# dbdexter-dev/sdrpp_radiosonde

Hardware: AMD Instinct MI355X
Metric: IQ Msamples/s through demod+FEC @ 48 kS/s/ch (higher is better)
Workload: dtype f32; 1 GPU; RS41-SG x 1024 channels/GPU x 196608 samples per step (4800 Bd GFSK, 48 kS/s, Eb/N0 14.0 dB); 5 consecutive blocks of a continuous signal resident in HBM, cycled; channels_per_gpu=1024, samples_per_channel=196608, flags=0, launch_units=1, join=one launch on the caller's stream, channel_stride_samples=262144, ingest=rank-local

## Files before the change

### include/sonde_abi.h

```cpp
#ifndef SONDE_ABI_H
#define SONDE_ABI_H

#include <stddef.h>
#include <stdint.h>
#include <time.h>

#ifdef __cplusplus
extern "C" {
#endif


typedef enum { PROCEED = 0, PARSED = 1 } ParserStatus;

#define DATA_SEQ      (1 << 0)
#define DATA_POS      (1 << 1)
#define DATA_SPEED    (1 << 2)
#define DATA_TIME     (1 << 3)
#define DATA_PTU      (1 << 4)
#define DATA_SERIAL   (1 << 5)
#define DATA_SHUTDOWN (1 << 6)
#define DATA_OZONE    (1 << 7)

typedef struct {
	int    fields;
	int    seq;
	float  lat, lon, alt;
	float  speed, heading, climb;
	time_t time;
	float  calib_percent;
	float  temp, rh, pressure;
	char   serial[32];
	int    shutdown;
	float  o3_mpa;
} SondeData;

typedef struct SondeB1Decoder RS41Decoder;
typedef struct SondeB1Decoder DFM09Decoder;
typedef struct SondeB1Decoder IMS100Decoder;
typedef struct SondeB1Decoder M10Decoder;
typedef struct SondeB1Decoder IMET4Decoder;
typedef struct SondeB1Decoder C50Decoder;
typedef struct SondeB1Decoder MRZN1Decoder;

#define SONDE_B1_DECL(T, x) \
	T *x##_decoder_init(int samplerate); \
	void x##_decoder_deinit(T *d); \
	ParserStatus x##_decode(T *d, SondeData *dst, const float *src, size_t len);

SONDE_B1_DECL(RS41Decoder,   rs41)
SONDE_B1_DECL(DFM09Decoder,  dfm09)
SONDE_B1_DECL(IMS100Decoder, ims100)
SONDE_B1_DECL(M10Decoder,    m10)
SONDE_B1_DECL(IMET4Decoder,  imet4)
SONDE_B1_DECL(C50Decoder,    c50)
SONDE_B1_DECL(MRZN1Decoder,  mrzn1)


enum { SONDE_RS41 = 0, SONDE_DFM09 = 1, SONDE_IMS100 = 2, SONDE_M10 = 3, SONDE_IMET4 = 4, SONDE_C50 = 5, SONDE_MRZN1 = 6, SONDE_NTYPES = 7 };

enum { SONDE_INPUT_IQ = 0,
       SONDE_INPUT_REAL = 1,
       SONDE_INPUT_IQ8 = 3,
       SONDE_INPUT_IQ16 = 2 };

#define SONDE_TILE       2048
#define SONDE_FRAME_MAX  528

typedef struct {
	uint32_t channel;
	uint32_t type;
	int32_t  len;
	int32_t  nerr[2];
	uint32_t flags;
	uint64_t bitpos;
	uint8_t  data[SONDE_FRAME_MAX];
} SondeFrame;

typedef struct {
	uint32_t       n_channels;
	const uint8_t *types;
	uint32_t       max_samples;
	int32_t        input_kind;
	int32_t        device;
	uint32_t       flags;
	uint32_t       launch_units;
	uint32_t       struct_size;
	uint32_t       time_slices;
} SondeBatchConfig;
#define SONDE_BATCH_CONFIG_INIT { 0, NULL, 0, 0, 0, 0, 0, (uint32_t)sizeof(SondeBatchConfig), 0 }

#define SONDE_FLAG_WIDE      1u
#define SONDE_FLAG_RS41_WIDE SONDE_FLAG_WIDE
#define SONDE_FLAG_SPLIT_FEC 2u
#define SONDE_FLAG_PIPELINE  4u
#define SONDE_FLAG_WIDE_AUTO 8u
#define SONDE_FLAG_JOIN      16u
#define SONDE_FLAG_LATE_JOIN 32u

typedef struct SondeBatch SondeBatch;

int  sonde_batch_create(const SondeBatchConfig *cfg, SondeBatch **out);
void sonde_batch_destroy(SondeBatch *b);

size_t sonde_row_stride(size_t n_samples, int input_kind);
size_t sonde_sample_bytes(int input_kind);
int  sonde_batch_submit(SondeBatch *b, const void *samples, size_t n_samples, size_t channel_stride, void *stream);
int  sonde_batch_submit_host(SondeBatch *b, const void *samples, size_t n_samples, size_t channel_stride);
int  sonde_batch_wait_input(SondeBatch *b, void *stream);
long sonde_batch_sync(SondeBatch *b);
long sonde_batch_frames(SondeBatch *b, SondeFrame *out, size_t cap);
uint64_t sonde_batch_ticket(SondeBatch *b);
long sonde_batch_frames_of(SondeBatch *b, uint64_t ticket, SondeFrame *out, size_t cap);
long sonde_batch_overflow(SondeBatch *b);
long sonde_batch_poll(SondeBatch *b, SondeData *out, uint32_t *channel, size_t cap);
int  sonde_batch_kernel_ms(SondeBatch *b, float *demod_ms, float *framer_ms);
int  sonde_batch_set_timing(SondeBatch *b, int every_n);
int  sonde_batch_launch_info(const SondeBatch *b, uint32_t *n_units, int32_t *join_mode);
int  sonde_batch_class_ms(SondeBatch *b, float out[4]);

int      sonde_batch_read_bits(SondeBatch *b, uint32_t channel, uint64_t from, size_t count, uint8_t *out );
int      sonde_batch_test_rs255(SondeBatch *b, uint8_t *cw_pairs, size_t n_pairs, int n, int32_t *status);
uint64_t sonde_batch_nbits(SondeBatch *b, uint32_t channel);
int      sonde_batch_read_state(SondeBatch *b, uint32_t channel, int64_t *t_next, int32_t *period, float *bias, float *amp,
                                float *afc_u );
int      sonde_get_taps(int type, float *out );
int      sonde_get_afsk_table(float *out );

int  sonde_parse_frame(const SondeFrame *f, SondeData *out, int cap);

typedef struct SondeParserHandle SondeParserHandle;
SondeParserHandle *sonde_parser_create(int sonde_type);
int  sonde_parser_feed(SondeParserHandle *p, const SondeFrame *f, SondeData *out, int cap);
void sonde_parser_destroy(SondeParserHandle *p);

float sonde_rs41_temp(uint32_t f, uint32_t f1, uint32_t f2, float rf1, float rf2, const float co[3], const float cal[3]);
float sonde_rs41_rh(uint32_t f, uint32_t f1, uint32_t f2, float calh0, float temp);
float sonde_dfm_temp(float f, float f1, float f2);
float sonde_rs41_pressure(uint32_t f, uint32_t f1, uint32_t f2, float tpress, const float *cfP );
float sonde_ozone_mpa(float cell_ua, float tpump_c);
float sonde_m10_temp(unsigned scale, unsigned adc);
float sonde_m10_rh(uint32_t cap_sensor, uint32_t cap_ref, float temp);
float sonde_m20_temp(unsigned adc);
float sonde_ims100_temp(uint32_t f, float c0, float c1, float c2);

typedef struct SondeChannelizer SondeChannelizer;
int         sonde_chan_create(const uint8_t *types , uint32_t blocks_per_submit ,
                              int device, SondeChannelizer **out);
int         sonde_chan_create_multi(const uint8_t *types, uint32_t blocks_per_submit, uint32_t n_streams, int device, SondeChannelizer **out);
int         sonde_chan_create_dual(const uint8_t *types, uint32_t blocks_per_submit, uint32_t n_streams, int device, SondeChannelizer **out);
uint32_t    sonde_chan_streams(const SondeChannelizer *c);
uint32_t    sonde_chan_channels(const SondeChannelizer *c);
int         sonde_chan_set_fused(SondeChannelizer *c, int on);
int         sonde_chan_set_input(SondeChannelizer *c, int input_kind);
int         sonde_chan_set_overlap(SondeChannelizer *c, int on);
void        sonde_chan_destroy(SondeChannelizer *c);
uint32_t    sonde_chan_samples_per_submit(const SondeChannelizer *c);
int         sonde_chan_submit(SondeChannelizer *c, const void *iq_dev, size_t n_samples, void *stream);
SondeBatch *sonde_chan_batch(SondeChannelizer *c);
int         sonde_chan_read(SondeChannelizer *c, float *bins, float *out48);
int         sonde_chan_kernel_ms(SondeChannelizer *c, float *pfb_ms, float *disc_resamp_ms, float *demod_ms, float *framer_ms);
int         sonde_chan_tables(float *h, float *tw, float *g);

typedef struct SondeVfo SondeVfo;
int    sonde_vfo_create(uint32_t n_channels, int rate_in, size_t max_in, int device, SondeVfo **out);
void   sonde_vfo_destroy(SondeVfo *v);
int    sonde_vfo_ratio(int rate_in, int *up, int *down);
size_t sonde_vfo_out_samples(const SondeVfo *v, size_t n_in);
int    sonde_vfo_process(SondeVfo *v, const void *iq_dev, size_t n_in, size_t channel_stride ,
                         float *out48_dev, size_t out_stride , void *stream);
int    sonde_vfo_process_host(SondeVfo *v, const void *iq_host, size_t n_in, size_t channel_stride,
                              const float **out48_dev, size_t *out_stride);
int    sonde_vfo_taps(int rate_in, float *g );

typedef struct SondeDetector SondeDetector;
typedef struct {
	int32_t  type;
	uint32_t inverted;
	double   best[SONDE_NTYPES];
	uint64_t pos[SONDE_NTYPES];
} SondeDetection;
int  sonde_detect_create(uint32_t n_channels, uint32_t max_samples, int input_kind, const uint8_t *type_mask, int device, SondeDetector **out);
void sonde_detect_destroy(SondeDetector *d);
int  sonde_detect_submit(SondeDetector *d, const void *samples, size_t n_samples, size_t channel_stride, void *stream);
int  sonde_detect_results(SondeDetector *d, SondeDetection *out, size_t cap);
int  sonde_detect_reset(SondeDetector *d);
int  sonde_detect_thresholds(float out[SONDE_NTYPES]);
int  sonde_detect_read(SondeDetector *d, uint32_t channel, int32_t *D , int32_t *a_imet , int32_t *a_c50 );
int  sonde_detect_templates(int type, int8_t *s, int cap);

typedef struct { int32_t offset_hz; uint32_t bandwidth_hz;  } SondeTunerVfo;
typedef struct SondeTuner SondeTuner;
int    sonde_tuner_ratio(uint32_t rate_in, uint32_t rate_out, int *up, int *down);
int    sonde_tuner_taps(uint32_t rate_in, uint32_t rate_out, uint32_t bandwidth_hz, float *g, size_t cap);
int    sonde_tuner_create(uint32_t rate_in, uint32_t rate_out, uint32_t n_vfos, const SondeTunerVfo *vfos,
                          size_t max_in, int input_kind, int device, SondeTuner **out);
void   sonde_tuner_destroy(SondeTuner *t);
size_t sonde_tuner_out_samples(const SondeTuner *t, size_t n_in);
int    sonde_tuner_retune(SondeTuner *t, uint32_t vfo, int32_t offset_hz);
int    sonde_tuner_process(SondeTuner *t, const void *wide_dev, size_t n_in,
                           void *out_dev , size_t out_stride , void *stream);

typedef struct SondeScanner SondeScanner;
typedef struct {
	uint32_t struct_size;
	uint32_t smooth_hz;
	uint32_t min_sep_hz;
	uint32_t centroid_hz;
	float    threshold;
} SondeScanParams;
typedef struct {
	int32_t  offset_hz;
	uint32_t bandwidth_hz;
	float    cn0_dbhz;
	float    excess_db;
	uint32_t bin;
} SondeScanCandidate;
int  sonde_scan_create(uint32_t rate_in, uint32_t fft_size , size_t max_in, int input_kind, int device, SondeScanner **out);
void sonde_scan_destroy(SondeScanner *s);
int  sonde_scan_fft_size(const SondeScanner *s);
int  sonde_scan_submit(SondeScanner *s, const void *wide_dev, size_t n_in, void *stream);
int  sonde_scan_reset(SondeScanner *s);
long long sonde_scan_segments(SondeScanner *s);
int  sonde_scan_spectrum(SondeScanner *s, float *P, size_t cap);
int  sonde_scan_candidates(SondeScanner *s, const SondeScanParams *p, SondeScanCandidate *out, size_t cap);
int  sonde_scan_search(const float *P, uint32_t n, uint32_t rate_in, const SondeScanParams *p, SondeScanCandidate *out, size_t cap);
int  sonde_scan_window(uint32_t n, float *w, size_t cap);
int  sonde_scan_auto_fft_size(uint32_t rate_in);

float sonde_dewpt(float temp, float rh);
float sonde_altitude_to_pressure(float alt);

void *sonde_gpx_open(const char *path);
void  sonde_gpx_close(void *g);
void  sonde_gpx_start_track(void *g, const char *name);
void  sonde_gpx_stop_track(void *g);
void  sonde_gpx_add_point(void *g, long t, float lat, float lon, float alt, float spd, float hdg);
void *sonde_ptu_open(const char *path);
void  sonde_ptu_close(void *p);
void  sonde_ptu_add_point(void *p, long t, float temp, float rh, float dewpt, float pressure, float lat, float lon,
                          float alt, float spd, float hdg, float climb, const char *aux);

int sonde_hbm_read_probe(const void *d_buf, size_t bytes, int reps, float *gbs_out);

const char *sonde_last_error(void);
const char *sonde_version(void);

#ifdef __cplusplus
}
#endif
#endif
```

### sdrpp_radiosonde_amd/_lib.py

```python
from __future__ import annotations

import ctypes as C
import os

import numpy as np

PKG_DIR = os.path.dirname(os.path.abspath(__file__))
LIB_PATH = os.environ.get("SONDE_MI355_LIB") or os.path.join(PKG_DIR, "libsonde_mi355.so")

TILE = 2048
FRAME_MAX = 528
(RS41, DFM09, IMS100, M10, IMET4, C50, MRZN1) = range(7)
INPUT_IQ, INPUT_REAL, INPUT_IQ16, INPUT_IQ8 = 0, 1, 2, 3
PROCEED, PARSED = 0, 1
DATA_SEQ, DATA_POS, DATA_SPEED, DATA_TIME, DATA_PTU, DATA_SERIAL, DATA_SHUTDOWN, DATA_OZONE = (1 << i for i in range(8))


class SondeFrame(C.Structure):
    _fields_ = [("channel", C.c_uint32), ("type", C.c_uint32), ("len", C.c_int32), ("nerr", C.c_int32 * 2),
                ("flags", C.c_uint32), ("bitpos", C.c_uint64), ("data", C.c_uint8 * FRAME_MAX)]


FRAME_DTYPE = np.dtype([("channel", "<u4"), ("type", "<u4"), ("len", "<i4"), ("nerr", "<i4", (2,)),
                        ("flags", "<u4"), ("bitpos", "<u8"), ("data", "u1", (FRAME_MAX,))])
assert FRAME_DTYPE.itemsize == C.sizeof(SondeFrame)


class SondeData(C.Structure):
    _fields_ = [("fields", C.c_int), ("seq", C.c_int), ("lat", C.c_float), ("lon", C.c_float), ("alt", C.c_float),
                ("speed", C.c_float), ("heading", C.c_float), ("climb", C.c_float), ("time", C.c_int64),
                ("calib_percent", C.c_float), ("temp", C.c_float), ("rh", C.c_float), ("pressure", C.c_float),
                ("serial", C.c_char * 32), ("shutdown", C.c_int), ("o3_mpa", C.c_float)]


class SondeDetection(C.Structure):
    _fields_ = [("type", C.c_int32), ("inverted", C.c_uint32), ("best", C.c_double * 7), ("pos", C.c_uint64 * 7)]


DETECTION_DTYPE = np.dtype([("type", "<i4"), ("inverted", "<u4"), ("best", "<f8", (7,)), ("pos", "<u8", (7,))])
assert DETECTION_DTYPE.itemsize == C.sizeof(SondeDetection)


class SondeTunerVfo(C.Structure):
    _fields_ = [("offset_hz", C.c_int32), ("bandwidth_hz", C.c_uint32)]


class SondeScanParams(C.Structure):
    _fields_ = [("struct_size", C.c_uint32), ("smooth_hz", C.c_uint32), ("min_sep_hz", C.c_uint32), ("centroid_hz", C.c_uint32),
                ("threshold", C.c_float)]


class SondeScanCandidate(C.Structure):
    _fields_ = [("offset_hz", C.c_int32), ("bandwidth_hz", C.c_uint32), ("cn0_dbhz", C.c_float), ("excess_db", C.c_float),
                ("bin", C.c_uint32)]


CANDIDATE_DTYPE = np.dtype([("offset_hz", "<i4"), ("bandwidth_hz", "<u4"), ("cn0_dbhz", "<f4"), ("excess_db", "<f4"), ("bin", "<u4")])
assert CANDIDATE_DTYPE.itemsize == C.sizeof(SondeScanCandidate)


class SondeBatchConfig(C.Structure):
    _fields_ = [("n_channels", C.c_uint32), ("types", C.POINTER(C.c_uint8)), ("max_samples", C.c_uint32),
                ("input_kind", C.c_int32), ("device", C.c_int32), ("flags", C.c_uint32), ("launch_units", C.c_uint32),
                ("struct_size", C.c_uint32), ("time_slices", C.c_uint32)]

    def __init__(self, *a, **k):
        super().__init__(*a, **k)
        self.struct_size = C.sizeof(SondeBatchConfig)


FLAG_WIDE = 1
FLAG_RS41_WIDE = FLAG_WIDE
FLAG_SPLIT_FEC = 2
FLAG_PIPELINE = 4
FLAG_JOIN = 16
FLAG_LATE_JOIN = 32
FLAG_WIDE_AUTO = 8


ABI_SYMBOLS = [
    "sonde_batch_create", "sonde_batch_destroy", "sonde_batch_submit", "sonde_batch_submit_host",
    "sonde_row_stride", "sonde_sample_bytes", "sonde_batch_wait_input", "sonde_batch_sync", "sonde_batch_frames", "sonde_batch_frames_of", "sonde_batch_ticket", "sonde_batch_overflow", "sonde_batch_kernel_ms", "sonde_batch_set_timing", "sonde_batch_class_ms", "sonde_batch_read_bits",
    "sonde_batch_launch_info", "sonde_batch_nbits", "sonde_batch_read_state", "sonde_batch_test_rs255", "sonde_batch_poll", "sonde_get_taps", "sonde_get_afsk_table", "sonde_parse_frame",
    "sonde_parser_create", "sonde_parser_feed", "sonde_parser_destroy", "sonde_rs41_temp", "sonde_rs41_rh", "sonde_dfm_temp", "sonde_rs41_pressure", "sonde_ozone_mpa",
    "sonde_m10_temp", "sonde_m10_rh", "sonde_m20_temp", "sonde_ims100_temp",
    "sonde_last_error", "sonde_version", "sonde_hbm_read_probe", "sonde_dewpt", "sonde_altitude_to_pressure",
    "sonde_gpx_open", "sonde_gpx_close", "sonde_gpx_start_track", "sonde_gpx_stop_track", "sonde_gpx_add_point",
    "sonde_ptu_open", "sonde_ptu_close", "sonde_ptu_add_point",
    "sonde_chan_create", "sonde_chan_create_multi", "sonde_chan_create_dual", "sonde_chan_streams", "sonde_chan_channels", "sonde_chan_set_fused", "sonde_chan_set_input", "sonde_chan_set_overlap", "sonde_chan_destroy", "sonde_chan_samples_per_submit", "sonde_chan_submit", "sonde_chan_batch",
    "sonde_chan_read", "sonde_chan_tables", "sonde_chan_kernel_ms",
    "sonde_vfo_create", "sonde_vfo_destroy", "sonde_vfo_ratio", "sonde_vfo_out_samples", "sonde_vfo_process", "sonde_vfo_process_host", "sonde_vfo_taps",
    "sonde_detect_create", "sonde_detect_destroy", "sonde_detect_submit", "sonde_detect_results", "sonde_detect_reset", "sonde_detect_thresholds",
    "sonde_detect_read", "sonde_detect_templates",
    "sonde_tuner_ratio", "sonde_tuner_taps", "sonde_tuner_create", "sonde_tuner_destroy", "sonde_tuner_out_samples", "sonde_tuner_retune",
    "sonde_tuner_process",
    "sonde_scan_create", "sonde_scan_destroy", "sonde_scan_fft_size", "sonde_scan_submit", "sonde_scan_reset", "sonde_scan_segments",
    "sonde_scan_spectrum", "sonde_scan_candidates", "sonde_scan_search", "sonde_scan_window", "sonde_scan_auto_fft_size",
] + [f"{x}_{fn}" for x in ("rs41", "dfm09", "ims100", "m10", "imet4", "c50", "mrzn1")
     for fn in ("decoder_init", "decoder_deinit", "decode")]

_lib = None


def load() -> C.CDLL:
    global _lib
    if _lib is not None:
        return _lib
    if not os.path.exists(LIB_PATH):
        import subprocess
        csrc = os.path.join(os.path.dirname(LIB_PATH), "csrc")
        try:
            subprocess.check_call(["make", "-s", "-C", csrc])
        except (OSError, subprocess.CalledProcessError) as e:
            raise RuntimeError(f"{LIB_PATH} is missing and `make -C {csrc}` failed ({e}); there is no CPU fallback") from e
    L = C.CDLL(LIB_PATH)
    vp = C.c_void_p
    L.sonde_hbm_read_probe.argtypes = [C.c_void_p, C.c_size_t, C.c_int, C.POINTER(C.c_float)]
    L.sonde_hbm_read_probe.restype = C.c_int
    L.sonde_last_error.restype = C.c_char_p
    L.sonde_version.restype = C.c_char_p
    L.sonde_batch_create.argtypes = [C.POINTER(SondeBatchConfig), C.POINTER(vp)]
    L.sonde_batch_destroy.argtypes = [vp]
    L.sonde_batch_destroy.restype = None
    L.sonde_batch_submit.argtypes = [vp, vp, C.c_size_t, C.c_size_t, vp]
    L.sonde_batch_submit_host.argtypes = [vp, vp, C.c_size_t, C.c_size_t]
    L.sonde_batch_sync.argtypes = [vp]
    L.sonde_batch_sync.restype = C.c_long
    if hasattr(L, "sonde_batch_wait_input"):
        L.sonde_batch_wait_input.argtypes = [vp, vp]
    L.sonde_batch_frames.argtypes = [vp, vp, C.c_size_t]
    L.sonde_batch_frames.restype = C.c_long
    if hasattr(L, "sonde_batch_frames_of"):
        L.sonde_batch_frames_of.argtypes = [vp, C.c_uint64, vp, C.c_size_t]
        L.sonde_batch_frames_of.restype = C.c_long
        L.sonde_batch_ticket.argtypes = [vp]
        L.sonde_batch_ticket.restype = C.c_uint64
        L.sonde_batch_overflow.argtypes = [vp]
        L.sonde_batch_overflow.restype = C.c_long
    L.sonde_batch_kernel_ms.argtypes = [vp, C.POINTER(C.c_float), C.POINTER(C.c_float)]
    if hasattr(L, "sonde_batch_set_timing"):
        L.sonde_batch_set_timing.argtypes = [vp, C.c_int]
    L.sonde_batch_read_bits.argtypes = [vp, C.c_uint32, C.c_uint64, C.c_size_t, vp]
    L.sonde_batch_nbits.argtypes = [vp, C.c_uint32]
    L.sonde_batch_nbits.restype = C.c_uint64
    L.sonde_batch_read_state.argtypes = [vp, C.c_uint32, C.POINTER(C.c_int64), C.POINTER(C.c_int32),
                                         C.POINTER(C.c_float), C.POINTER(C.c_float), C.POINTER(C.c_float)]
    if hasattr(L, "sonde_batch_test_rs255"):
        L.sonde_batch_test_rs255.argtypes = [vp, vp, C.c_size_t, C.c_int, vp]
    L.sonde_get_taps.argtypes = [C.c_int, vp]
    L.sonde_parse_frame.argtypes = [vp, C.POINTER(SondeData), C.c_int]
    L.sonde_batch_poll.argtypes = [vp, C.POINTER(SondeData), C.POINTER(C.c_uint32), C.c_size_t]
    L.sonde_batch_poll.restype = C.c_long
    L.sonde_parser_create.argtypes = [C.c_int]
    L.sonde_parser_create.restype = vp
    L.sonde_parser_feed.argtypes = [vp, vp, C.POINTER(SondeData), C.c_int]
    L.sonde_parser_feed.restype = C.c_int
    L.sonde_parser_destroy.argtypes = [vp]
    L.sonde_parser_destroy.restype = None
    L.sonde_rs41_pressure.argtypes = [C.c_uint32, C.c_uint32, C.c_uint32, C.c_float, C.POINTER(C.c_float)]
    L.sonde_rs41_pressure.restype = C.c_float
    L.sonde_ozone_mpa.argtypes = [C.c_float, C.c_float]
    L.sonde_ozone_mpa.restype = C.c_float
    L.sonde_m10_temp.argtypes = [C.c_uint, C.c_uint]
    L.sonde_m10_temp.restype = C.c_float
    L.sonde_m10_rh.argtypes = [C.c_uint32, C.c_uint32, C.c_float]
    L.sonde_m10_rh.restype = C.c_float
    L.sonde_m20_temp.argtypes = [C.c_uint]
    L.sonde_m20_temp.restype = C.c_float
    L.sonde_ims100_temp.argtypes = [C.c_uint32, C.c_float, C.c_float, C.c_float]
    L.sonde_ims100_temp.restype = C.c_float
    L.sonde_rs41_temp.argtypes = [C.c_uint32, C.c_uint32, C.c_uint32, C.c_float, C.c_float, C.POINTER(C.c_float), C.POINTER(C.c_float)]
    L.sonde_rs41_temp.restype = C.c_float
    L.sonde_rs41_rh.argtypes = [C.c_uint32, C.c_uint32, C.c_uint32, C.c_float, C.c_float]
    L.sonde_rs41_rh.restype = C.c_float
    L.sonde_dfm_temp.argtypes = [C.c_float, C.c_float, C.c_float]
    L.sonde_dfm_temp.restype = C.c_float
    L.sonde_dewpt.restype = C.c_float
    L.sonde_dewpt.argtypes = [C.c_float, C.c_float]
    L.sonde_altitude_to_pressure.restype = C.c_float
    L.sonde_altitude_to_pressure.argtypes = [C.c_float]
    L.sonde_chan_create.argtypes = [vp, C.c_uint32, C.c_int, C.POINTER(vp)]
    L.sonde_chan_create_multi.argtypes = [vp, C.c_uint32, C.c_uint32, C.c_int, C.POINTER(vp)]
    L.sonde_chan_set_fused.argtypes = [vp, C.c_int]
    L.sonde_chan_set_overlap.argtypes = [vp, C.c_int]
    L.sonde_row_stride.argtypes = [C.c_size_t, C.c_int]
    L.sonde_row_stride.restype = C.c_size_t
    L.sonde_sample_bytes.argtypes = [C.c_int]
    L.sonde_sample_bytes.restype = C.c_size_t
    L.sonde_chan_streams.argtypes = [vp]
    L.sonde_chan_streams.restype = C.c_uint32
    L.sonde_chan_destroy.argtypes = [vp]
    L.sonde_chan_destroy.restype = None
    L.sonde_chan_samples_per_submit.argtypes = [vp]
    L.sonde_chan_samples_per_submit.restype = C.c_uint32
    L.sonde_chan_submit.argtypes = [vp, vp, C.c_size_t, vp]
    L.sonde_chan_kernel_ms.argtypes = [vp] + [C.POINTER(C.c_float)] * 4
    L.sonde_chan_batch.argtypes = [vp]
    L.sonde_chan_batch.restype = vp
    L.sonde_chan_read.argtypes = [vp, vp, vp]
    L.sonde_chan_tables.argtypes = [vp, vp, vp]
    if hasattr(L, "sonde_vfo_create"):
        L.sonde_vfo_create.argtypes = [C.c_uint32, C.c_int, C.c_size_t, C.c_int, C.POINTER(vp)]
        L.sonde_vfo_destroy.argtypes = [vp]
        L.sonde_vfo_destroy.restype = None
        L.sonde_vfo_ratio.argtypes = [C.c_int, C.POINTER(C.c_int), C.POINTER(C.c_int)]
        L.sonde_vfo_out_samples.argtypes = [vp, C.c_size_t]
        L.sonde_vfo_out_samples.restype = C.c_size_t
        L.sonde_vfo_process.argtypes = [vp, vp, C.c_size_t, C.c_size_t, vp, C.c_size_t, vp]
        L.sonde_vfo_process_host.argtypes = [vp, vp, C.c_size_t, C.c_size_t, C.POINTER(vp), C.POINTER(C.c_size_t)]
        L.sonde_vfo_taps.argtypes = [C.c_int, vp]
    if hasattr(L, "sonde_detect_create"):
        L.sonde_detect_create.argtypes = [C.c_uint32, C.c_uint32, C.c_int, vp, C.c_int, C.POINTER(vp)]
        L.sonde_detect_destroy.argtypes = [vp]
        L.sonde_detect_destroy.restype = None
        L.sonde_detect_submit.argtypes = [vp, vp, C.c_size_t, C.c_size_t, vp]
        L.sonde_detect_results.argtypes = [vp, vp, C.c_size_t]
        L.sonde_detect_reset.argtypes = [vp]
        L.sonde_detect_thresholds.argtypes = [vp]
        L.sonde_detect_read.argtypes = [vp, C.c_uint32, vp, vp, vp]
        L.sonde_detect_templates.argtypes = [C.c_int, vp, C.c_int]
    if hasattr(L, "sonde_tuner_create"):
        L.sonde_tuner_ratio.argtypes = [C.c_uint32, C.c_uint32, C.POINTER(C.c_int), C.POINTER(C.c_int)]
        L.sonde_tuner_taps.argtypes = [C.c_uint32, C.c_uint32, C.c_uint32, vp, C.c_size_t]
        L.sonde_tuner_create.argtypes = [C.c_uint32, C.c_uint32, C.c_uint32, C.POINTER(SondeTunerVfo), C.c_size_t, C.c_int, C.c_int, C.POINTER(vp)]
        L.sonde_tuner_destroy.argtypes = [vp]
        L.sonde_tuner_destroy.restype = None
        L.sonde_tuner_out_samples.argtypes = [vp, C.c_size_t]
        L.sonde_tuner_out_samples.restype = C.c_size_t
        L.sonde_tuner_retune.argtypes = [vp, C.c_uint32, C.c_int32]
        L.sonde_tuner_process.argtypes = [vp, vp, C.c_size_t, vp, C.c_size_t, vp]
    if hasattr(L, "sonde_scan_create"):
        L.sonde_scan_create.argtypes = [C.c_uint32, C.c_uint32, C.c_size_t, C.c_int, C.c_int, C.POINTER(vp)]
        L.sonde_scan_destroy.argtypes = [vp]
        L.sonde_scan_destroy.restype = None
        L.sonde_scan_fft_size.argtypes = [vp]
        L.sonde_scan_submit.argtypes = [vp, vp, C.c_size_t, vp]
        L.sonde_scan_reset.argtypes = [vp]
        L.sonde_scan_segments.argtypes = [vp]
        L.sonde_scan_segments.restype = C.c_longlong
        L.sonde_scan_spectrum.argtypes = [vp, vp, C.c_size_t]
        L.sonde_scan_candidates.argtypes = [vp, C.POINTER(SondeScanParams), vp, C.c_size_t]
        L.sonde_scan_search.argtypes = [vp, C.c_uint32, C.c_uint32, C.POINTER(SondeScanParams), vp, C.c_size_t]
        L.sonde_scan_window.argtypes = [C.c_uint32, vp, C.c_size_t]
        L.sonde_scan_auto_fft_size.argtypes = [C.c_uint32]
    f = C.c_float
    L.sonde_gpx_open.restype = vp
    L.sonde_gpx_open.argtypes = [C.c_char_p]
    L.sonde_gpx_close.argtypes = [vp]
    L.sonde_gpx_start_track.argtypes = [vp, C.c_char_p]
    L.sonde_gpx_stop_track.argtypes = [vp]
    L.sonde_gpx_add_point.argtypes = [vp, C.c_long, f, f, f, f, f]
    L.sonde_ptu_open.restype = vp
    L.sonde_ptu_open.argtypes = [C.c_char_p]
    L.sonde_ptu_close.argtypes = [vp]
    L.sonde_ptu_add_point.argtypes = [vp, C.c_long, f, f, f, f, f, f, f, f, f, f, C.c_char_p]
    for x in ("rs41", "dfm09", "ims100", "m10", "imet4", "c50", "mrzn1"):
        getattr(L, f"{x}_decoder_init").argtypes = [C.c_int]
        getattr(L, f"{x}_decoder_init").restype = vp
        getattr(L, f"{x}_decoder_deinit").argtypes = [vp]
        getattr(L, f"{x}_decoder_deinit").restype = None
        getattr(L, f"{x}_decode").argtypes = [vp, C.POINTER(SondeData), vp, C.c_size_t]
        getattr(L, f"{x}_decode").restype = C.c_int
    _lib = L
    return L


def last_error() -> str:
    return load().sonde_last_error().decode()
```

### sdrpp_radiosonde_amd/batch.py

```python
from __future__ import annotations

import ctypes as C

import numpy as np

from . import _lib
from ._lib import FRAME_DTYPE, INPUT_IQ, INPUT_IQ8, INPUT_IQ16, INPUT_REAL, TILE


class SondeError(RuntimeError):
    pass


class SondeBatch:

    def __init__(self, n_channels: int, max_samples: int, *, types=None, input_kind: int = INPUT_IQ, device: int = 0, flags: int = 0, time_slices: int = 0):
        self.L = _lib.load()
        self.n_channels = int(n_channels)
        self.max_samples = int(max_samples)
        self.input_kind = input_kind
        self.device = int(device)
        cfg = _lib.SondeBatchConfig()
        cfg.n_channels = self.n_channels
        self._types = None
        if types is not None:
            self._types = np.ascontiguousarray(types, dtype=np.uint8)
            assert self._types.shape == (self.n_channels,)
            cfg.types = self._types.ctypes.data_as(C.POINTER(C.c_uint8))
        cfg.max_samples = self.max_samples
        cfg.flags = flags
        cfg.time_slices = time_slices
        cfg.input_kind = input_kind
        cfg.device = device
        h = C.c_void_p()
        if self.L.sonde_batch_create(C.byref(cfg), C.byref(h)) != 0:
            raise SondeError(_lib.last_error())
        self.h = h

    def close(self):
        if getattr(self, "h", None):
            self.L.sonde_batch_destroy(self.h)
            self.h = None

    __del__ = close

    def _chk(self, rc):
        if rc < 0:
            raise SondeError(_lib.last_error())
        return rc

    def submit(self, samples, stream: int | None = None):
        shape = tuple(samples.shape)
        n = shape[1]
        if shape[0] != self.n_channels:
            raise SondeError("first dimension must be n_channels")
        is_iq = self.input_kind in (INPUT_IQ, INPUT_IQ16, INPUT_IQ8)
        if is_iq and (len(shape) != 3 or shape[2] != 2):
            raise SondeError("IQ input must be [C, n, 2] (float32; int16 for INPUT_IQ16, int8 for INPUT_IQ8)")
        if not is_iq and len(shape) != 2:
            raise SondeError("real input must be [C, n] float32")
        dt = str(getattr(samples, "dtype", ""))
        want = {INPUT_IQ16: "int16", INPUT_IQ8: "int8"}.get(self.input_kind, "float32")
        if not dt.endswith(want) or dt.endswith("u" + want):
            raise SondeError(f"samples must be {want}, got {dt}")
        dev = getattr(samples, "device", None)
        if dev is None or getattr(dev, "type", "") != "cuda":
            raise SondeError("samples must be a device (HIP) tensor; use submit_host() for host memory")
        if dev.index is not None and dev.index != self.device:
            raise SondeError(f"samples live on device {dev.index}, the batch on device {self.device}")
        st = tuple(samples.stride())
        if (is_iq and st[1:] != (2, 1)) or (not is_iq and st[1] != 1):
            raise SondeError("samples must be contiguous inside a channel (only the channel stride may be padded)")
        stride = samples.stride(0) // (2 if is_iq else 1)
        self._keep = (samples, getattr(self, "_keep", (None, None))[0])
        self._chk(self.L.sonde_batch_submit(self.h, C.c_void_p(samples.data_ptr()), n, stride, C.c_void_p(stream or 0)))

    def submit_host(self, samples: np.ndarray):
        want = {INPUT_IQ16: np.int16, INPUT_IQ8: np.int8}.get(self.input_kind, np.float32)
        if want is not np.float32 and np.asarray(samples).dtype != want:
            raise SondeError(f"samples must be {np.dtype(want).name} for this input kind, got {np.asarray(samples).dtype} (no silent conversion)")
        samples = np.ascontiguousarray(samples, dtype=want)
        n = samples.shape[1]
        self._chk(self.L.sonde_batch_submit_host(self.h, samples.ctypes.data_as(C.c_void_p), n, n))

    def wait_input(self, stream: int | None = None):
        self._chk(self.L.sonde_batch_wait_input(self.h, C.c_void_p(stream or 0)))

    def sync(self) -> int:
        return self._chk(self.L.sonde_batch_sync(self.h))

    def frames(self) -> np.ndarray:
        n = self.sync()
        out = np.zeros(n, dtype=FRAME_DTYPE)
        if n:
            got = self._chk(self.L.sonde_batch_frames(self.h, out.ctypes.data_as(C.c_void_p), n))
            out = out[:got]
        return out

    def ticket(self) -> int:
        return int(self.L.sonde_batch_ticket(self.h))

    def frames_of(self, ticket: int) -> np.ndarray:
        n = self._chk(self.L.sonde_batch_frames_of(self.h, ticket, None, 0))
        out = np.zeros(n, dtype=FRAME_DTYPE)
        if n:
            out = out[:self._chk(self.L.sonde_batch_frames_of(self.h, ticket, out.ctypes.data_as(C.c_void_p), n))]
        return out

    def overflow(self) -> int:
        return self._chk(self.L.sonde_batch_overflow(self.h))

    def poll(self, cap: int = 4096):
        out = (_lib.SondeData * cap)()
        chan = (C.c_uint32 * cap)()
        res = []
        while True:
            n = self._chk(self.L.sonde_batch_poll(self.h, out, chan, cap))
            if n == 0:
                return res
            for i in range(n):
                d = _lib.SondeData()
                C.memmove(C.byref(d), C.byref(out[i]), C.sizeof(d))
                res.append((int(chan[i]), d))

    def kernel_ms(self):
        a, b = C.c_float(), C.c_float()
        self._chk(self.L.sonde_batch_kernel_ms(self.h, C.byref(a), C.byref(b)))
        return a.value, b.value

    def class_ms(self) -> dict:
        v = (C.c_float * 4)()
        self.L.sonde_batch_class_ms.argtypes = [C.c_void_p, C.POINTER(C.c_float)]
        n = self._chk(self.L.sonde_batch_class_ms(self.h, v))
        return {k: float(v[k]) for k in range(4) if n > 0 and v[k] >= 0.0}

    def launch_info(self) -> dict:
        u, j = C.c_uint32(), C.c_int32()
        self.L.sonde_batch_launch_info.argtypes = [C.c_void_p, C.POINTER(C.c_uint32), C.POINTER(C.c_int32)]
        self._chk(self.L.sonde_batch_launch_info(self.h, C.byref(u), C.byref(j)))
        return {"units": int(u.value), "join": int(j.value)}

    def set_timing(self, every_n: int):
        self._chk(self.L.sonde_batch_set_timing(self.h, int(every_n)))

    def nbits(self, channel: int) -> int:
        return int(self.L.sonde_batch_nbits(self.h, channel))

    def read_bits(self, channel: int, start: int, count: int) -> np.ndarray:
        out = np.zeros(count, dtype=np.uint8)
        self._chk(self.L.sonde_batch_read_bits(self.h, channel, start, count, out.ctypes.data_as(C.c_void_p)))
        return out

    def state(self, channel: int) -> dict:
        t, p = C.c_int64(), C.c_int32()
        b, a, y = C.c_float(), C.c_float(), C.c_float()
        self._chk(self.L.sonde_batch_read_state(self.h, channel, C.byref(t), C.byref(p), C.byref(b), C.byref(a), C.byref(y)))
        return dict(t_next=t.value, period=p.value, bias=b.value, amp=a.value, afc_u=y.value, yprev=y.value)


def row_stride(n_samples: int, iq: bool = True, kind: int | None = None) -> int:
    if kind is None:
        kind = INPUT_IQ if iq else INPUT_REAL
    return int(_lib.load().sonde_row_stride(int(n_samples), kind))


def strided_rows(x, stride: int | None = None):
    import torch
    n = x.shape[1]
    st = stride or row_stride(n, kind={torch.int16: INPUT_IQ16, torch.int8: INPUT_IQ8}.get(x.dtype, INPUT_IQ) if x.dim() == 3 else INPUT_REAL)
    if st == n:
        return x
    buf = torch.empty((x.shape[0], st) + tuple(x.shape[2:]), dtype=x.dtype, device=x.device)
    buf[:, :n] = x
    return buf[:, :n]


class SondeChannelizer:

    def __init__(self, types=None, blocks_per_submit: int = 1, device: int = 0, n_streams: int = 1, fused: bool | None = None, overlap: bool | None = None,
                 dual: bool = False, input_kind: int = INPUT_IQ):
        self.L = _lib.load()
        self._types = None
        self.n_streams = int(n_streams)
        self.dual = bool(dual)
        self.n_channels = (1024 if dual else 512) * self.n_streams
        tp = None
        if types is not None:
            self._types = np.ascontiguousarray(types, dtype=np.uint8)
            assert self._types.shape == (self.n_channels,)
            tp = self._types.ctypes.data_as(C.c_void_p)
        h = C.c_void_p()
        create = self.L.sonde_chan_create_dual if dual else self.L.sonde_chan_create_multi
        if create(tp, blocks_per_submit, self.n_streams, device, C.byref(h)) != 0:
            raise SondeError(_lib.last_error() or "sonde_chan_create failed")
        self.h = h
        self.fused = bool(self.L.sonde_chan_set_fused(self.h, 1 if fused else 0)) if fused is not None else bool(self.L.sonde_chan_set_fused(self.h, -1))
        self.overlap = bool(self.L.sonde_chan_set_overlap(self.h, 1)) if overlap else False
        self.input_kind = int(self.L.sonde_chan_set_input(self.h, input_kind))
        if self.input_kind != input_kind:
            raise SondeError("sonde_chan_set_input: input kind not accepted")
        self.samples_per_submit = int(self.L.sonde_chan_samples_per_submit(self.h))
        self.n_steps = self.samples_per_submit // 500
        self.batch = SondeBatch.__new__(SondeBatch)
        self.batch.L = self.L
        self.batch.h = C.c_void_p(self.L.sonde_chan_batch(self.h))
        self.batch.n_channels = self.n_channels
        self.batch.close = lambda: None

    def submit(self, iq, stream: int | None = None):
        assert tuple(iq.shape) in ((self.samples_per_submit, 2), (self.n_streams, self.samples_per_submit, 2)) and iq.is_contiguous()
        assert self.n_streams == 1 or iq.dim() == 3
        want = {INPUT_IQ16: "int16", INPUT_IQ8: "int8"}.get(self.input_kind, "float32")
        if not str(iq.dtype).endswith(want) or str(iq.dtype).endswith("u" + want):
            raise SondeError(f"wideband block must be {want}, got {iq.dtype}")
        self._keep = iq
        if self.L.sonde_chan_submit(self.h, C.c_void_p(iq.data_ptr()), self.samples_per_submit, C.c_void_p(stream or 0)) != 0:
            raise SondeError(_lib.last_error() or "sonde_chan_submit failed")

    def frames(self) -> np.ndarray:
        return SondeBatch.frames(self.batch)

    def kernel_ms(self):
        v = [C.c_float() for _ in range(4)]
        if self.L.sonde_chan_kernel_ms(self.h, *[C.byref(x) for x in v]) != 0:
            raise SondeError(_lib.last_error() or "sonde_chan_kernel_ms failed")
        return tuple(x.value for x in v)

    def read(self):
        bins = np.zeros((self.n_channels, self.n_steps), dtype=np.float32)
        out48 = None if self.fused else np.zeros((self.n_channels, self.n_steps * 12 // 5), dtype=np.float32)
        if self.L.sonde_chan_read(self.h, bins.ctypes.data_as(C.c_void_p), out48.ctypes.data_as(C.c_void_p) if out48 is not None else None) != 0:
            raise SondeError("sonde_chan_read failed")
        return bins, out48

    def close(self):
        if getattr(self, "h", None):
            self.batch.h = None
            self.L.sonde_chan_destroy(self.h)
            self.h = None

    __del__ = close


def get_taps(sonde_type: int) -> np.ndarray:
    out = np.zeros((32, 32), dtype=np.float32)
    if _lib.load().sonde_get_taps(sonde_type, out.ctypes.data_as(C.c_void_p)) != 0:
        raise SondeError(_lib.last_error())
    return out


VFO_RATE = {0: 10000, 1: 15000, 2: 20000, 3: 50000, 4: 20000, 5: 20000, 6: 20000}


class SondeVfo:

    def __init__(self, n_channels: int, rate_in: int, max_in: int, device: int = 0):
        self.L = _lib.load()
        h = C.c_void_p()
        if self.L.sonde_vfo_create(n_channels, rate_in, max_in, device, C.byref(h)) != 0:
            raise SondeError(_lib.last_error() or "sonde_vfo_create failed")
        self.h = h
        self.n_channels, self.rate_in, self.max_in = n_channels, rate_in, max_in
        up, down = C.c_int(), C.c_int()
        self.L.sonde_vfo_ratio(rate_in, C.byref(up), C.byref(down))
        self.up, self.down = up.value, down.value

    def out_samples(self, n_in: int) -> int:
        return int(self.L.sonde_vfo_out_samples(self.h, n_in))

    def process(self, iq, out=None, stream: int | None = None):
        import torch
        assert iq.is_cuda and iq.dtype == torch.float32 and iq.shape[0] == self.n_channels and iq.shape[2] == 2 and iq.stride(1) == 2
        n_in = iq.shape[1]
        n_out = self.out_samples(n_in)
        if out is None:
            out = torch.empty((self.n_channels, n_out), dtype=torch.float32, device=iq.device)
        if stream is None:
            stream = torch.cuda.current_stream(iq.device).cuda_stream
        if self.L.sonde_vfo_process(self.h, C.c_void_p(iq.data_ptr()), n_in, iq.stride(0) // 2, C.c_void_p(out.data_ptr()), out.stride(0),
                                    C.c_void_p(stream)) != 0:
            raise SondeError(_lib.last_error() or "sonde_vfo_process failed")
        return out

    def taps(self) -> np.ndarray:
        g = np.zeros((self.up, 16), dtype=np.float32)
        if self.L.sonde_vfo_taps(self.rate_in, g.ctypes.data_as(C.c_void_p)) != 0:
            raise SondeError(_lib.last_error() or "sonde_vfo_taps failed")
        return g

    def close(self):
        if getattr(self, "h", None):
            self.L.sonde_vfo_destroy(self.h)
            self.h = None

    def __del__(self):
        try:
            self.close()
        except Exception:
            pass
```

### sdrpp_radiosonde_amd/csrc/batch.hip

```cpp
#include <hip/hip_runtime.h>
#include <math.h>
#include <stdio.h>
#include <stdlib.h>
#include <string.h>
#include <algorithm>
#include <string>
#include <vector>
#include "sonde_dev.h"
#include "sd_input.h"
#include "../../include/sonde_abi.h"

#include "launch.h"
#include "parse.h"
#include <deque>
#include <memory>

#ifndef SD_EV_FLAGS
#define SD_EV_FLAGS hipEventDisableSystemFence
#endif
#define SD_EV_TIMING (SD_EV_FLAGS)
#define SD_EV_ORDER  (hipEventDisableTiming | SD_EV_FLAGS)
static thread_local std::string g_err;
static int fail(const char *what, hipError_t e = hipSuccess)
{
	g_err = what;
	if (e != hipSuccess) { g_err += ": "; g_err += hipGetErrorString(e); }
	return -1;
}
#define HIPCHK(x) do { hipError_t e_ = (x); if (e_ != hipSuccess) return fail(#x, e_); } while (0)

extern "C" const char *sonde_last_error(void) { return g_err.c_str(); }
int sd_fail(const char *what, hipError_t e) { return fail(what, e); }
extern "C" const char *sonde_version(void) { return "sonde_mi355 0.1 (gfx950)"; }

struct ModemDef { double baud; float cutoff; int decim; int pre; };
static const ModemDef k_modems[SONDE_NTYPES] = {
	{ 4800.0, 0.65f, 4, 1 },
	{ 5000.0, 0.65f, 4, 1 },
	{ 4800.0, 0.65f, 4, 1 },
	{ 9600.0, 0.65f, 2, 1 },
	{ 1200.0, 0.65f, 1, 8 },
	{ 2400.0, 0.65f, 1, 8 },
	{ 4800.0, 0.65f, 4, 1 },
};

static int modem_div(const ModemDef *md, int type) { return md[type].decim * md[type].pre; }
static int32_t modem_period0(const ModemDef *md, int type) { return (int32_t)llrint(65536.0 * ((double)SD_FS / modem_div(md, type)) / md[type].baud); }
static int modem_nt(const ModemDef *md, int type) { return SD_NT_OF(modem_period0(md, type), md[type].pre); }
static const int k_cls_decim[4] = { 1, 2, 4, 2 }, k_cls_nt[4] = { 16, 16, 8, 8 };
static int modem_class(const ModemDef *md, int type)
{
	const int d = md[type].decim, nt = modem_nt(md, type);
	for (int k = 0; k < 4; k++) if (k_cls_decim[k] == d && k_cls_nt[k] == nt) return k;
	return -1;
}

static void make_taps(const ModemDef *md, int type, float *out )
{
	const double PI = 3.14159265358979323846;
	const double fc = (double)md[type].cutoff * md[type].baud / ((double)SD_FS / modem_div(md, type));
	const int nt = modem_nt(md, type);
	memset(out, 0, sizeof(float) * SD_NPHASE * SD_NTAPS);
	for (int p = 0; p < SD_NPHASE; p++) {
		double h[SD_NTAPS], sum = 0.0;
		for (int j = 0; j < nt; j++) {
			const double t = (double)j - (double)(nt / 2) + (double)p / (double)SD_NPHASE;
			const double x = (t + (double)(nt / 2)) / (double)nt;
			const double w = 0.42 - 0.5 * cos(2.0 * PI * x) + 0.08 * cos(4.0 * PI * x);
			const double s = (t == 0.0) ? 2.0 * fc : sin(2.0 * PI * fc * t) / (PI * t);
			h[j] = s * w;
			sum += h[j];
		}
		for (int j = 0; j < nt; j++) out[p * SD_NTAPS + j] = (float)(h[j] / sum);
	}
}

void make_mixer(float *out, int cycles, int per)
{
	const double PI = 3.14159265358979323846;
	for (int k = 0; k < per; k++) {
		const double a = 2.0 * PI * (double)cycles * (double)k / (double)per;
		out[2 * k] = (float)cos(a);
		out[2 * k + 1] = (float)(-sin(a));
	}
}
extern "C" int sonde_get_afsk_table(float *out )
{
	if (!out) return fail("sonde_get_afsk_table: null argument");
	make_mixer(out, 17, SD_AF_PER);
	return 0;
}

extern "C" int sonde_get_taps(int type, float *out)
{
	if (type < 0 || type >= SONDE_NTYPES || !out) return fail("sonde_get_taps: bad argument");
	make_taps(k_modems, type, out);
	return 0;
}

struct SondeBatch {
	uint32_t n_channels = 0, max_samples = 0;
	int input_kind = 0, device = 0;
	uint32_t ring_words = 0, max_frames = 0;
	uint32_t type_frames[SONDE_NTYPES] = {};
	std::vector<uint8_t> types;
	std::vector<uint32_t> chlist[SONDE_NTYPES];
	ModemDef md[SONDE_NTYPES];

	SdChanState *d_states = nullptr;
	SdFramerState *d_fstates = nullptr;
	float *d_hist = nullptr;
	uint32_t *d_bitring = nullptr;
	SondeFrame *d_frames2[2] = {};
	uint32_t *d_counts2[2] = {};
	hipEvent_t ev_done[2] = {};
	bool ev_valid[2] = { false, false };
	bool ticketing = false;
	hipEvent_t ev_xs = nullptr;
	uint64_t tickets = 0;
	float *d_taps = nullptr;
	SdModem *d_modems = nullptr;
	uint8_t *d_gfexp = nullptr, *d_gflog = nullptr, *d_g64 = nullptr;
	uint16_t *d_m10tab = nullptr;
	uint32_t fuse_fec = 1;
	uint32_t fixed_epi = 1;
	SdFramerOut *d_fo2[2] = {};
	SdFramerOut h_fo2[2] = {};
	SdModem h_modems[SONDE_NTYPES] = {};
	uint32_t *d_gfswar = nullptr;
	void *d_descs = nullptr;
	uint32_t *d_chlist[SONDE_NTYPES] = {};
	void *d_stage = nullptr;
	size_t stage_bytes = 0;
	SdAfskState *d_astates = nullptr;
	float *d_wtab = nullptr, *d_wtab_c50 = nullptr, *d_afq = nullptr;
	uint32_t n_cls[4] = {};
	int cls_type[4] = { -1, -1, -1, -1 };
	int n_classes = 0, only_class = 0;
	struct Unit { int type, cls; uint32_t off, n; size_t row0; hipStream_t st; hipEvent_t ev_join[2]; };
	std::vector<Unit> units;
	uint32_t *d_cls[4] = {};
	int n_chunks = 1;
	hipEvent_t ev_fork = nullptr;
	int join_mode = 0;
	bool pipeline = false;
	hipStream_t done_stream = nullptr;
	uint32_t granule = SONDE_TILE;
	uint32_t *d_prog = nullptr;
	uint32_t seg_base = 0;
	uint32_t residency = 1024;
	int seg_force = 0;
	bool sliced_once = false;
	bool mixed_one = false;

	static const int kEvSlots = 128;
	hipEvent_t ev[3 * kEvSlots] = {};
	int ev_used = 0;
	hipEvent_t *evc = nullptr;
	int evc_used = 0;
	int timing_every = 8;
	unsigned long n_submits = 0;
	bool ev_has_framer[kEvSlots] = {};
	hipStream_t last_stream = nullptr;
	bool pending = false;
	bool have_counts2[2] = { false, false };
	std::vector<uint32_t> h_counts2[2];
	long n_frames2[2] = { 0, 0 }, n_overflow2[2] = { 0, 0 };
	std::vector<SondeFrame> h_slots;
	std::vector<std::unique_ptr<SondeParser>> parsers;
	std::deque<std::pair<uint32_t, SondeData>> frags;
	uint64_t polled_ticket = 0;
};

static uint32_t pow2ceil(uint32_t v) { uint32_t p = 1; while (p < v) p <<= 1; return p; }

extern "C" void sonde_batch_destroy(SondeBatch *b)
{
	if (!b) return;
	(void)hipSetDevice(b->device);
	if (b->pending) (void)hipStreamSynchronize(b->last_stream);
	(void)hipFree(b->d_states); (void)hipFree(b->d_fstates); (void)hipFree(b->d_hist); (void)hipFree(b->d_bitring);
	for (int k = 0; k < 2; k++) { (void)hipFree(b->d_frames2[k]); (void)hipFree(b->d_counts2[k]); (void)hipFree(b->d_fo2[k]); if (b->ev_done[k]) (void)hipEventDestroy(b->ev_done[k]); }
	if (b->ev_xs) (void)hipEventDestroy(b->ev_xs);
	(void)hipFree(b->d_taps); (void)hipFree(b->d_modems); (void)hipFree(b->d_prog);
	(void)hipFree(b->d_astates); (void)hipFree(b->d_wtab); (void)hipFree(b->d_wtab_c50); (void)hipFree(b->d_afq);
	for (auto &u : b->units) { if (u.st) (void)hipStreamDestroy(u.st); for (int k = 0; k < 2; k++) if (u.ev_join[k]) (void)hipEventDestroy(u.ev_join[k]); }
	for (int k = 0; k < 4; k++) (void)hipFree(b->d_cls[k]);
	if (b->done_stream) (void)hipStreamDestroy(b->done_stream);
	if (b->ev_fork) (void)hipEventDestroy(b->ev_fork);
	(void)hipFree(b->d_gfexp); (void)hipFree(b->d_gflog); (void)hipFree(b->d_gfswar); (void)hipFree(b->d_g64); (void)hipFree(b->d_m10tab); (void)hipFree(b->d_descs); (void)hipFree(b->d_stage);
	for (int t = 0; t < SONDE_NTYPES; t++) (void)hipFree(b->d_chlist[t]);
	for (int i = 0; i < 3 * SondeBatch::kEvSlots; i++) if (b->ev[i]) (void)hipEventDestroy(b->ev[i]);
	if (b->evc) { for (size_t i = 0; i < 2 * b->units.size() * SondeBatch::kEvSlots; i++) if (b->evc[i]) (void)hipEventDestroy(b->evc[i]); delete[] b->evc; }
	delete b;
}

extern "C" int sonde_batch_create(const SondeBatchConfig *cfg, SondeBatch **out)
{
	if (!cfg || !out) return fail("sonde_batch_create: null argument");
	*out = nullptr;
	if (cfg->struct_size != sizeof(SondeBatchConfig))
		return fail("sonde_batch_create: SondeBatchConfig.struct_size != sizeof(SondeBatchConfig) -- initialise with SONDE_BATCH_CONFIG_INIT (a host built against an older sonde_abi.h must be recompiled)");
	if (cfg->launch_units > 16) return fail("sonde_batch_create: launch_units must be 0 (the library's choice) or 1..16");
	if (cfg->time_slices > 16) return fail("sonde_batch_create: time_slices must be 0 (the library's choice) or 1..16");
	if (cfg->n_channels == 0) return fail("sonde_batch_create: n_channels == 0");
	if (cfg->max_samples == 0 || cfg->max_samples % SONDE_TILE) return fail("sonde_batch_create: max_samples must be a positive multiple of SONDE_TILE");
	if (!sd_input_known(cfg->input_kind)) return fail("sonde_batch_create: bad input_kind");
	int ndev = 0;
	HIPCHK(hipGetDeviceCount(&ndev));
	if (cfg->device < 0 || cfg->device >= ndev) return fail("sonde_batch_create: no such HIP device");
	HIPCHK(hipSetDevice(cfg->device));

	SondeBatch *b = new SondeBatch;
	b->n_channels = cfg->n_channels;
	b->max_samples = cfg->max_samples;
	b->input_kind = cfg->input_kind;
	b->device = cfg->device;
	for (int t = 0; t < SONDE_NTYPES; t++) b->md[t] = k_modems[t];
	if ((cfg->flags & (SONDE_FLAG_WIDE | SONDE_FLAG_WIDE_AUTO)) && cfg->input_kind != SONDE_INPUT_REAL)
		for (int t = 0; t < SONDE_NTYPES; t++) {
			const bool wide_type = (cfg->flags & SONDE_FLAG_WIDE) || t == SONDE_IMS100 || t == SONDE_MRZN1 || t == SONDE_M10;
			if (b->md[t].pre == 1 && wide_type) b->md[t].decim /= 2;
		}
	const ModemDef *md = b->md;
	b->types.assign(cfg->n_channels, SONDE_RS41);
	if (cfg->types) b->types.assign(cfg->types, cfg->types + cfg->n_channels);
	uint64_t max_bits = 0;
	for (uint32_t c = 0; c < b->n_channels; c++) {
		const int t = b->types[c];
		if (t < 0 || t >= SONDE_NTYPES) { delete b; return fail("sonde_batch_create: bad sonde type"); }
		b->chlist[t].push_back(c);
		const int32_t p = modem_period0(md, t) - (modem_period0(md, t) >> 8);
		max_bits = std::max(max_bits, ((uint64_t)(cfg->max_samples / modem_div(md, t)) << 16) / (uint64_t)p + 2);
	}
	b->ring_words = pow2ceil((uint32_t)((max_bits + 8 * SONDE_FRAME_MAX + 1024 + 31) / 32));
	b->max_frames = 2;
	{
		static const uint32_t min_frame_bits[SONDE_NTYPES] = { 320 * 8, 560, 1152, 1648, 140, 90, 768 };
		for (int t = 0; t < SONDE_NTYPES; t++) {
			if (b->chlist[t].empty()) continue;
			const int32_t p = modem_period0(md, t) - (modem_period0(md, t) >> 8);
			const uint64_t bits_t = ((uint64_t)(cfg->max_samples / modem_div(md, t)) << 16) / (uint64_t)p + 2;
			b->type_frames[t] = (uint32_t)(bits_t / min_frame_bits[t]) + 2;
			b->max_frames = std::max(b->max_frames, b->type_frames[t]);
		}
	}
	if ((size_t)b->ring_words * 4 >= 65536) { delete b; return fail("sonde_batch_create: max_samples too large for the LDS-staged bit ring (< 64 KB)"); }

	const size_t C = b->n_channels;
#define ALLOC(p, bytes) do { hipError_t e_ = hipMalloc((void **)&(p), (bytes)); if (e_ != hipSuccess) { sonde_batch_destroy(b); return fail("hipMalloc " #p, e_); } } while (0)
	ALLOC(b->d_states, C * sizeof(SdChanState));
	ALLOC(b->d_fstates, C * sizeof(SdFramerState));
	ALLOC(b->d_hist, C * SD_HIST * sizeof(float));
	ALLOC(b->d_bitring, C * (size_t)b->ring_words * sizeof(uint32_t));
	for (int k = 0; k < 2; k++) {
		ALLOC(b->d_frames2[k], C * (size_t)b->max_frames * sizeof(SondeFrame));
		ALLOC(b->d_counts2[k], C * sizeof(uint32_t));
		ALLOC(b->d_fo2[k], sizeof(SdFramerOut));
	}
	ALLOC(b->d_taps, (size_t)SONDE_NTYPES * SD_NPHASE * SD_NTAPS * sizeof(float));
	ALLOC(b->d_modems, SONDE_NTYPES * sizeof(SdModem));
	ALLOC(b->d_prog, (C + 1) * sizeof(uint32_t));
	ALLOC(b->d_gfexp, 2304);
	ALLOC(b->d_gflog, 512);
	ALLOC(b->d_gfswar, 24 * 8 * sizeof(uint32_t));
	ALLOC(b->d_g64, 192);
	ALLOC(b->d_m10tab, 99 * 8 * sizeof(uint16_t));
	ALLOC(b->d_descs, C * (size_t)b->max_frames * SD_DESC_BYTES);
	for (int t = 0; t < SONDE_NTYPES; t++)
		if (!b->chlist[t].empty()) ALLOC(b->d_chlist[t], b->chlist[t].size() * sizeof(uint32_t));
	const size_t n_afsk = b->chlist[SONDE_IMET4].size() + b->chlist[SONDE_C50].size();
	std::vector<uint32_t> cls[4];
	for (uint32_t c = 0; c < b->n_channels; c++) {
		if (b->types[c] == SONDE_IMET4 || b->types[c] == SONDE_C50) continue;
		const int k = modem_class(md, b->types[c]);
		if (k < 0) { sonde_batch_destroy(b); return fail("sonde_batch_create: no demodulator class for this sonde type"); }
		cls[k].push_back(c);
	}
	for (int k = 0; k < 4; k++) {
		b->n_cls[k] = (uint32_t)cls[k].size();
		if (b->n_cls[k]) { b->n_classes++; b->only_class = k; }
		for (uint32_t c : cls[k]) {
			if (c == cls[k][0]) b->cls_type[k] = b->types[c];
			else if (b->types[c] != b->cls_type[k]) { b->cls_type[k] = -1; break; }
		}
	}
	b->join_mode = (cfg->flags & SONDE_FLAG_PIPELINE) ? 2 : ((cfg->flags & SONDE_FLAG_LATE_JOIN) ? 1 : 0);
	int one_class_units = 1;
	if (b->join_mode != 0 && n_afsk == 0 && b->n_classes == 1) {
		int n_types = 0;
		for (int t = 0; t < SONDE_NTYPES; t++) n_types += !b->chlist[t].empty();
		hipDeviceProp_t prop0;
		const uint32_t residency = hipGetDeviceProperties(&prop0, cfg->device) == hipSuccess ? 4u * (uint32_t)prop0.multiProcessorCount : 1024u;
		one_class_units = (n_types == 1 && b->n_channels >= 512 && b->n_channels % residency != 0) ? 2 : 1;
		if (cfg->launch_units) one_class_units = std::max(1, std::min(16, (int)cfg->launch_units));
	}
	const bool need_lists = n_afsk != 0 || b->n_classes > 1 || one_class_units > 1;
	if (n_afsk) {
		if (cfg->max_samples % (SONDE_TILE * SD_AF_DEC)) { sonde_batch_destroy(b); return fail("sonde_batch_create: with iMet channels max_samples must be a multiple of 16384"); }
		b->granule = SONDE_TILE * SD_AF_DEC;
		ALLOC(b->d_astates, C * sizeof(SdAfskState));
		ALLOC(b->d_wtab, SD_AF_PER * 2 * sizeof(float));
		ALLOC(b->d_wtab_c50, SD_C50_PER * 2 * sizeof(float));
		ALLOC(b->d_afq, n_afsk * (size_t)(cfg->max_samples / SD_AF_DEC) * sizeof(float));
	}
#undef ALLOC
#define CHK(x) do { hipError_t e_ = (x); if (e_ != hipSuccess) { sonde_batch_destroy(b); return fail(#x, e_); } } while (0)
	std::vector<float> taps((size_t)SONDE_NTYPES * SD_NPHASE * SD_NTAPS);
	SdModem modems[SONDE_NTYPES];
	for (int t = 0; t < SONDE_NTYPES; t++) {
		make_taps(md, t, &taps[(size_t)t * SD_NPHASE * SD_NTAPS]);
		const int32_t p0 = modem_period0(md, t);
		modems[t].period0 = p0;
		modems[t].kp = (float)p0 * 0.159154943f;
		modems[t].ki = modems[t].kp * (1.0f / 4096.0f);
		modems[t].pmin = p0 - (p0 >> 8);
		modems[t].pmax = p0 + (p0 >> 8);
		modems[t].decim = md[t].decim;
		modems[t].itile = SD_TILE / md[t].decim;
		modems[t].nt = modem_nt(md, t);
		const int rmax = SD_ROUND_MAX * SD_ROUND_SPL(modems[t].decim, modems[t].nt);
		modems[t].rounds = (int32_t)(((((int64_t)modems[t].itile << 16) / modems[t].pmin) + 2 + rmax - 1) / rmax);
	}
	CHK(hipMemcpy(b->d_taps, taps.data(), taps.size() * sizeof(float), hipMemcpyHostToDevice));
	CHK(hipMemcpy(b->d_modems, modems, sizeof(modems), hipMemcpyHostToDevice));
	memcpy(b->h_modems, modems, sizeof(modems));
	uint8_t gexp[512], glog[256];
	{
		int x = 1;
		memset(glog, 0, sizeof(glog));
		for (int i = 0; i < 255; i++) { gexp[i] = (uint8_t)x; glog[x] = (uint8_t)i; x <<= 1; if (x & 0x100) x ^= 0x11D; }
		for (int i = 255; i < 512; i++) gexp[i] = gexp[i - 255];
	}
	{
		std::vector<uint8_t> e2(2304, 0);
		for (int i = 0; i < 768; i++) e2[i] = gexp[i % 255];
		uint16_t l2[256];
		for (int v = 0; v < 256; v++) l2[v] = v ? (uint16_t)glog[v] : (uint16_t)768;
		CHK(hipMemcpy(b->d_gfexp, e2.data(), e2.size(), hipMemcpyHostToDevice));
		CHK(hipMemcpy(b->d_gflog, l2, sizeof(l2), hipMemcpyHostToDevice));
	}
	{
		uint32_t sw[24 * 8];
		memset(sw, 0, sizeof(sw));
		auto mul = [&](int c, int v) -> uint32_t { return (c && v) ? gexp[glog[c] + glog[v]] : 0u; };
		for (int j = 0; j < 24; j++) {
			const int c = gexp[(4 * j) % 255];
			for (int x = 0; x < 8; x++) {
				sw[8 * j + 0 + x / 4] |= mul(c, x) << (8 * (x % 4));
				sw[8 * j + 2 + x / 4] |= mul(c, x << 3) << (8 * (x % 4));
				if (x < 4) sw[8 * j + 4] |= mul(c, x << 6) << (8 * x);
			}
		}
		CHK(hipMemcpy(b->d_gfswar, sw, sizeof(sw), hipMemcpyHostToDevice));
	}
	{
		uint8_t g64[192];
		memset(g64, 0, sizeof(g64));
		int x = 1;
		for (int i = 0; i < 63; i++) { g64[i] = (uint8_t)x; g64[128 + x] = (uint8_t)i; x <<= 1; if (x & 0x40) x ^= 0x43; }
		for (int i = 63; i < 128; i++) g64[i] = g64[i - 63];
		CHK(hipMemcpy(b->d_g64, g64, sizeof(g64), hipMemcpyHostToDevice));
	}
	{
		auto step = [](unsigned c, unsigned bb) {
			const unsigned c1 = c & 0xFF;
			bb = ((bb >> 1) | ((bb & 1) << 7)) & 0xFF;
			bb ^= (bb >> 2) & 0xFF;
			const unsigned t6 = (c & 1) ^ ((c >> 2) & 1) ^ ((c >> 4) & 1);
			const unsigned t7 = ((c >> 1) & 1) ^ ((c >> 3) & 1) ^ ((c >> 5) & 1);
			const unsigned t = (c & 0x3F) | (t6 << 6) | (t7 << 7);
			unsigned sft = (c >> 7) & 0xFF;
			sft ^= (sft >> 2) & 0xFF;
			return ((c1 << 8) | (bb ^ t ^ sft)) & 0xFFFFu;
		};
		uint16_t tab[99 * 8];
		for (int j = 0; j < 8; j++) {
			unsigned c = step(0, 1u << j);
			for (int k = 0; k < 99; k++) { tab[8 * k + j] = (uint16_t)c; c = step(c, 0); }
		}
		CHK(hipMemcpy(b->d_m10tab, tab, sizeof(tab), hipMemcpyHostToDevice));
	}
	{
		b->fuse_fec = (cfg->flags & SONDE_FLAG_SPLIT_FEC) ? 0u : 1u;
		for (int k = 0; k < 2; k++) {
			hipDeviceProp_t prop;
			CHK(hipGetDeviceProperties(&prop, cfg->device));
			const uint32_t loop_wg = 4u * (uint32_t)prop.multiProcessorCount;
			if (!b->fuse_fec) b->fixed_epi = 0;
			const SdFramerOut fo = { b->d_fstates, b->d_descs, b->d_counts2[k], b->max_frames, b->fuse_fec, loop_wg, b->d_gfexp, b->d_gflog, b->d_gfswar, b->d_g64, b->d_frames2[k],
			                         b->d_m10tab, b->fixed_epi };
			CHK(hipMemcpy(b->d_fo2[k], &fo, sizeof(fo), hipMemcpyHostToDevice));
			b->h_fo2[k] = fo;
			CHK(hipEventCreateWithFlags(&b->ev_done[k], hipEventDisableTiming));
		}
		CHK(hipEventCreateWithFlags(&b->ev_xs, SD_EV_ORDER));
	}
	std::vector<SdChanState> st(C);
	for (size_t c = 0; c < C; c++) {
		memset(&st[c], 0, sizeof(SdChanState));
		const int t = b->types[c];
		st[c].type = t;
		st[c].period = modems[t].period0;
		st[c].t_next = ((int64_t)SD_NTAPS << 16) + modems[t].period0;
		st[c].amp = 0.25f;
	}
	CHK(hipMemcpy(b->d_states, st.data(), C * sizeof(SdChanState), hipMemcpyHostToDevice));
	CHK(hipMemset(b->d_fstates, 0, C * sizeof(SdFramerState)));
	CHK(hipMemset(b->d_prog, 0, (C + 1) * sizeof(uint32_t)));
	{
		hipDeviceProp_t pr;
		if (hipGetDeviceProperties(&pr, cfg->device) == hipSuccess && pr.multiProcessorCount > 0) b->residency = 4u * (uint32_t)pr.multiProcessorCount;
		b->seg_force = (int)cfg->time_slices;
	}
	CHK(hipMemset(b->d_hist, 0, C * SD_HIST * sizeof(float)));
	CHK(hipMemset(b->d_bitring, 0, C * (size_t)b->ring_words * sizeof(uint32_t)));
	for (int k = 0; k < 2; k++) CHK(hipMemset(b->d_counts2[k], 0, C * sizeof(uint32_t)));
	if (n_afsk) {
		float wtab[2 * SD_AF_PER];
		sonde_get_afsk_table(wtab);
		CHK(hipMemcpy(b->d_wtab, wtab, sizeof(wtab), hipMemcpyHostToDevice));
		float wc[2 * SD_C50_PER];
		make_mixer(wc, 19, SD_C50_PER);
		CHK(hipMemcpy(b->d_wtab_c50, wc, sizeof(wc), hipMemcpyHostToDevice));
		CHK(hipMemset(b->d_astates, 0, C * sizeof(SdAfskState)));
	}
	for (int t = 0; t < SONDE_NTYPES; t++)
		if (!b->chlist[t].empty())
			CHK(hipMemcpy(b->d_chlist[t], b->chlist[t].data(), b->chlist[t].size() * sizeof(uint32_t), hipMemcpyHostToDevice));
	for (int i = 0; i < 3 * SondeBatch::kEvSlots; i++) CHK(hipEventCreateWithFlags(&b->ev[i], SD_EV_TIMING));
	if (need_lists) {
		CHK(hipEventCreateWithFlags(&b->ev_fork, SD_EV_ORDER));
		const bool pipelined = b->join_mode != 0;
		int R = 1;
		if (one_class_units > 1) R = one_class_units;
		b->n_chunks = pipelined ? R : 1;
		static const int order[] = { SONDE_M10, SONDE_RS41, SONDE_DFM09, SONDE_IMS100, SONDE_MRZN1 };
		if (pipelined) {
			for (int j = 0; j < R; j++)
				for (int t : order) {
					const size_t nt = b->chlist[t].size();
					const size_t lo = nt * (size_t)j / (size_t)R, hi = nt * (size_t)(j + 1) / (size_t)R;
					if (hi > lo) b->units.push_back({ t, modem_class(md, t), (uint32_t)lo, (uint32_t)(hi - lo), 0, nullptr, { nullptr, nullptr } });
				}
		} else {
			for (int k : { 3, 0, 2, 1 }) {
				if (!b->n_cls[k]) continue;
				hipError_t e_ = hipMalloc((void **)&b->d_cls[k], cls[k].size() * sizeof(uint32_t));
				if (e_ == hipSuccess) e_ = hipMemcpy(b->d_cls[k], cls[k].data(), cls[k].size() * sizeof(uint32_t), hipMemcpyHostToDevice);
				if (e_ != hipSuccess) { sonde_batch_destroy(b); return fail("hipMalloc d_cls", e_); }
				b->units.push_back({ -1, k, 0, b->n_cls[k], 0, nullptr, { nullptr, nullptr } });
			}
		}
		size_t row0 = 0;
		for (int t : { SONDE_IMET4, SONDE_C50 }) {
			if (b->chlist[t].empty()) continue;
			b->units.push_back({ t, 0, 0, (uint32_t)b->chlist[t].size(), row0, nullptr, { nullptr, nullptr } });
			row0 += b->chlist[t].size();
		}
		{
			if (b->join_mode == 0 && n_afsk == 0 && b->n_classes == 2 && b->n_cls[2] && b->n_cls[3] && b->fuse_fec && b->fixed_epi) {
				b->mixed_one = true;
				b->units.clear();
			}
		}
		for (auto &u : b->units) {
			CHK(hipStreamCreateWithFlags(&u.st, hipStreamNonBlocking));
			for (int k = 0; k < 2; k++) CHK(hipEventCreateWithFlags(&u.ev_join[k], SD_EV_ORDER));
		}
		const size_t nev = 2 * b->units.size() * SondeBatch::kEvSlots;
		b->evc = new hipEvent_t[nev]();
		for (size_t i = 0; i < nev; i++) CHK(hipEventCreateWithFlags(&b->evc[i], SD_EV_TIMING));
		if (b->join_mode != 0) {
			b->pipeline = true;
			CHK(hipStreamCreateWithFlags(&b->done_stream, hipStreamNonBlocking));
		}
	}
#undef CHK
	for (int k = 0; k < 2; k++) b->h_counts2[k].assign(C, 0);
	*out = b;
	return 0;
}

static int submit_impl(SondeBatch *b, const void *samples, size_t n_samples, size_t channel_stride, void *stream_, const SdBinsArgs *bins_in);

extern "C" int sonde_batch_submit(SondeBatch *b, const void *samples, size_t n_samples, size_t channel_stride, void *stream_)
{
	if (!b || !samples) return fail("sonde_batch_submit: null argument");
	if (n_samples == 0 || n_samples % b->granule || n_samples > b->max_samples) return fail("sonde_batch_submit: n_samples must be a multiple of SONDE_TILE (16384 with iMet channels) and <= max_samples");
	if (channel_stride < n_samples) return fail("sonde_batch_submit: channel_stride < n_samples");
	if (((uintptr_t)samples & 15u) || channel_stride % (16 / sd_sample_bytes(b->input_kind)))
		return fail("sonde_batch_submit: samples must be 16-byte aligned and channel_stride a multiple of 2 (IQ) / 4 (real, 16-bit IQ) / 8 (8-bit IQ) samples");
	return submit_impl(b, samples, n_samples, channel_stride, stream_, nullptr);
}

int sd_batch_bins_capable(const SondeBatch *b)
{
	if (!b || b->input_kind != SONDE_INPUT_REAL) return 0;
	for (int t = 0; t < SONDE_NTYPES; t++) {
		if (b->chlist[t].empty()) continue;
		if (t == SONDE_IMET4 || t == SONDE_C50) return 0;
		const int k = modem_class(b->md, t);
		if (!(k_cls_nt[k] == 8 && k_cls_decim[k] == 4)) return 0;
	}
	return 1;
}
int sd_batch_submit_bins(SondeBatch *b, const SdBinsArgs *ba, size_t n_steps, void *stream_)
{
	if (!b || !ba || !ba->phases || !ba->carry_rows || !ba->g_comp || !sd_batch_bins_capable(b)) return fail("sd_batch_submit_bins: bad argument");
	if (!b->units.empty()) return fail("sd_batch_submit_bins: the decoder batch behind a channelizer must be one plain launch (no launch units)");
	const size_t n_out = n_steps / 5 * 12;
	if (n_steps == 0 || n_steps % 2560 || n_out > b->max_samples || ba->row_stride < n_steps + 16)
		return fail("sd_batch_submit_bins: n_steps must be a multiple of 2560 within max_samples");
	if ((ba->row_stride & 7) || (ba->carry_stride & 7) || ((uintptr_t)ba->phases & 15u) || ((uintptr_t)ba->carry_rows & 15u))
		return fail("sd_batch_submit_bins: phase rows and carry rows must be 16-byte aligned with strides that are multiples of 8 phases");
	return submit_impl(b, ba->phases, n_out, ba->row_stride, stream_, ba);
}

static int choose_segments(const SondeBatch *b, uint32_t n_wg, uint32_t total_wg, int n_tiles)
{
	(void)n_wg;
	if (b->seg_force > 0) return (b->seg_force <= n_tiles && total_wg > 0) ? b->seg_force : 1;
	if (b->join_mode != 0 || total_wg <= b->residency) return 1;
	static const int cand[] = { 1, 2, 4, 8 };
	int best = 1;
	double best_cost = 1e30;
	for (int S : cand) {
		const int st = (n_tiles + S - 1) / S;
		if (S > 1 && (st < 12 || n_tiles % S)) continue;
		double cost = 0.0;
		for (uint64_t left = (uint64_t)total_wg * (uint64_t)S; left > 0;) {
			const uint64_t g = left < b->residency ? left : b->residency;
			const double occ = (double)g / (double)b->residency;
			cost += (double)st * (occ < 0.67 ? 0.67 : occ) + 2.6;
			left -= g;
		}
		if (cost < best_cost * 0.98) { best_cost = cost; best = S; }
	}
	return best;
}

static int submit_impl(SondeBatch *b, const void *samples, size_t n_samples, size_t channel_stride, void *stream_, const SdBinsArgs *bins_in)
{
	HIPCHK(hipSetDevice(b->device));
	hipStream_t stream = (hipStream_t)stream_;
	const int n_tiles = (int)(n_samples / SONDE_TILE);
	const bool timed = b->timing_every > 0 && (b->n_submits % (unsigned long)b->timing_every == (unsigned long)b->timing_every - 1 || b->tickets == 0);
	b->n_submits++;
	hipEvent_t *ev = b->ev + 3 * (b->ev_used % SondeBatch::kEvSlots);
	if (timed) HIPCHK(hipEventRecord(ev[0], stream));
	const int slot = (int)(b->tickets & 1);
	SondeFrame *const d_frames = b->d_frames2[slot];
	uint32_t *const d_counts = b->d_counts2[slot];
	const SdFramerOut *fo = b->d_fo2[slot];
	const bool pipe = b->pipeline;
	if (!pipe && b->tickets && stream != b->last_stream) {
		HIPCHK(hipEventRecord(b->ev_xs, b->last_stream));
		HIPCHK(hipStreamWaitEvent(stream, b->ev_xs, 0));
	}
	bool framer_launched = false;
	auto launch_framers = [&](int t, hipStream_t sk, uint32_t off = 0, uint32_t nch = 0) -> int {
		if (b->chlist[t].empty()) return 0;
		if (!nch) nch = (uint32_t)b->chlist[t].size();
		const uint32_t *list = b->d_chlist[t] + off;
		if (t == SONDE_RS41) {
			if (b->fuse_fec) return 0;
			sd_launch_framer_rs41(nch, sk, b->d_bitring, b->ring_words, b->d_gfexp, b->d_gflog, b->d_gfswar, b->d_descs,
				d_frames, d_counts, b->max_frames, b->type_frames[SONDE_RS41], list);
		} else if (t == SONDE_C50) {
			sd_launch_framer_c50(nch, sk, b->d_states, b->d_fstates, b->d_bitring, b->ring_words, d_frames, d_counts, b->max_frames, list);
		} else if (t == SONDE_IMET4) {
			sd_launch_framer_imet(nch, sk, b->d_states, b->d_fstates, b->d_bitring, b->ring_words, d_frames, d_counts, b->max_frames, list);
		} else {
			if (b->fixed_epi && !bins_in) return 0;
			sd_launch_framer_other(t, nch, sk, b->d_states, b->d_fstates, b->d_bitring, b->ring_words,
				t == SONDE_M10 ? (const uint8_t *)b->d_m10tab : b->d_g64, b->d_descs, d_frames, d_counts, b->max_frames, b->type_frames[t], list,
				 !b->fuse_fec);
		}
		HIPCHK(hipGetLastError());
		framer_launched = true;
		return 0;
	};
	const bool one_launch = b->units.empty();
	uint32_t total_wg = b->n_channels;
	if (!one_launch) { total_wg = 0; for (const SondeBatch::Unit &u : b->units) total_wg += u.n; }
	int max_seg = 1;
	auto slice_of = [&](uint32_t n_wg, int tiles, SdSlice &sl, int decim, int nt) -> const SdSlice * {
		if (!sd_slices_supported(b->input_kind, decim, nt)) return nullptr;
		if (!one_launch && b->seg_force <= 0) return nullptr;
		const int S = choose_segments(b, n_wg, total_wg, tiles);
		if (S <= 1) return nullptr;
		sl.seg_tiles = (tiles + S - 1) / S; sl.n_wg = n_wg; sl.seg_base = b->seg_base; sl.prog = b->d_prog; sl.err_index = b->n_channels;
		sl.n_seg = (tiles + sl.seg_tiles - 1) / sl.seg_tiles;
		max_seg = std::max(max_seg, (int)sl.n_seg);
		b->sliced_once = true;
		return &sl;
	};
	if (b->mixed_one && !bins_in) {
		sd_launch_demod_mixed(b->input_kind, b->n_cls[2], b->d_cls[2], b->cls_type[2], b->n_cls[3], b->d_cls[3], b->cls_type[3], stream, (const float *)samples, channel_stride,
			n_tiles, b->d_states, b->d_hist, b->d_bitring, b->ring_words, b->d_taps, b->d_modems, fo);
		HIPCHK(hipGetLastError());
		if (timed) HIPCHK(hipEventRecord(ev[1], stream));
	} else if (one_launch) {
		if (bins_in)
			sd_launch_bins(b->n_channels, stream, bins_in->phases, bins_in->row_stride, n_tiles / 3, bins_in->carry_rows, bins_in->carry_stride,
				b->d_states, b->d_hist, b->d_bitring, b->ring_words, b->d_taps, b->h_modems, &b->h_fo2[slot], bins_in->g_comp, b->cls_type[b->only_class]);
		else {
			SdSlice sl;
			sd_launch_demod(b->input_kind, k_cls_decim[b->only_class], k_cls_nt[b->only_class], b->n_channels, stream, (const float *)samples, channel_stride, n_tiles,
				b->d_states, b->d_hist, b->d_bitring, b->ring_words, b->d_taps, b->d_modems, nullptr, false, fo, b->cls_type[b->only_class],
				slice_of(b->n_channels, n_tiles, sl, k_cls_decim[b->only_class], k_cls_nt[b->only_class]));
		}
		HIPCHK(hipGetLastError());
		if (timed) HIPCHK(hipEventRecord(ev[1], stream));
		for (int t = 0; t < SONDE_NTYPES; t++) if (launch_framers(t, stream)) return -1;
	} else {
		HIPCHK(hipEventRecord(b->ev_fork, stream));
		const size_t nq = n_samples / SD_AF_DEC;
		hipStream_t join_to = pipe ? b->done_stream : stream;
		for (size_t ui = 0; ui < b->units.size(); ui++) {
			const SondeBatch::Unit &u = b->units[ui];
			HIPCHK(hipStreamWaitEvent(u.st, b->ev_fork, 0));
			hipEvent_t *ec = b->evc + 2 * (b->units.size() * (size_t)(b->evc_used % SondeBatch::kEvSlots) + ui);
			if (timed) HIPCHK(hipEventRecord(ec[0], u.st));
			if (u.type == SONDE_IMET4 || u.type == SONDE_C50) {
				float *rows = b->d_afq + u.row0 * (size_t)(b->max_samples / SD_AF_DEC);
				sd_launch_afsk(u.type, b->input_kind, u.n, u.st, (const float *)samples, channel_stride, n_tiles,
					b->d_chlist[u.type], b->d_astates, u.type == SONDE_C50 ? b->d_wtab_c50 : b->d_wtab, rows, nq);
				sd_launch_demod(SONDE_INPUT_REAL, 1, 16, u.n, u.st, rows, nq, (int)(nq / SONDE_TILE),
					b->d_states, b->d_hist, b->d_bitring, b->ring_words, b->d_taps, b->d_modems, b->d_chlist[u.type], true, fo, u.type);
			} else {
				SdSlice sl;
				sd_launch_demod(b->input_kind, k_cls_decim[u.cls], k_cls_nt[u.cls], u.n, u.st, (const float *)samples, channel_stride, n_tiles,
					b->d_states, b->d_hist, b->d_bitring, b->ring_words, b->d_taps, b->d_modems,
					u.type < 0 ? b->d_cls[u.cls] : b->d_chlist[u.type] + u.off, false, fo, u.type < 0 ? b->cls_type[u.cls] : u.type,
					slice_of(u.n, n_tiles, sl, k_cls_decim[u.cls], k_cls_nt[u.cls]));
			}
			HIPCHK(hipGetLastError());
			if (timed) HIPCHK(hipEventRecord(ec[1], u.st));
			if (u.type >= 0) {
				if (launch_framers(u.type, u.st, u.off, u.n)) return -1;
			} else {
				for (int t = 0; t < SONDE_NTYPES; t++)
					if (t != SONDE_IMET4 && t != SONDE_C50 && modem_class(b->md, t) == u.cls && launch_framers(t, u.st)) return -1;
			}
			HIPCHK(hipEventRecord(u.ev_join[slot], u.st));
			HIPCHK(hipStreamWaitEvent(join_to, u.ev_join[slot], 0));
		}
		if (b->join_mode == 1 && b->tickets)
			for (const SondeBatch::Unit &u : b->units) HIPCHK(hipStreamWaitEvent((hipStream_t)stream_, u.ev_join[slot ^ 1], 0));
		if (timed) b->evc_used++;
		if (pipe) stream = b->done_stream;
		if (timed) HIPCHK(hipEventRecord(ev[1], stream));
		framer_launched = false;
	}
	if (timed) {
		if (framer_launched) HIPCHK(hipEventRecord(ev[2], stream));
		b->ev_has_framer[b->ev_used % SondeBatch::kEvSlots] = framer_launched;
		b->ev_used++;
	}
	if (max_seg > 1) b->seg_base += (uint32_t)max_seg;
	b->ev_valid[slot] = b->ticketing;
	if (b->ticketing) HIPCHK(hipEventRecord(b->ev_done[slot], stream));
	b->tickets++;
	b->last_stream = stream;
	b->pending = true;
	b->have_counts2[slot] = false;
	return 0;
}

extern "C" int sonde_batch_wait_input(SondeBatch *b, void *stream_)
{
	if (!b) return fail("sonde_batch_wait_input: null argument");
	if (b->tickets == 0) return 0;
	HIPCHK(hipSetDevice(b->device));
	hipStream_t stream = (hipStream_t)stream_;
	if (!b->units.empty()) {
		const int slot = (int)((b->tickets - 1) & 1);
		for (const SondeBatch::Unit &u : b->units) HIPCHK(hipStreamWaitEvent(stream, u.ev_join[slot], 0));
		return 0;
	}
	if (stream == b->last_stream) return 0;
	HIPCHK(hipEventRecord(b->ev_xs, b->last_stream));
	HIPCHK(hipStreamWaitEvent(stream, b->ev_xs, 0));
	return 0;
}

extern "C" int sonde_batch_launch_info(const SondeBatch *b, uint32_t *n_units, int32_t *join_mode)
{
	if (!b) return fail("sonde_batch_launch_info: null argument");
	if (n_units) *n_units = b->units.empty() ? 1u : (uint32_t)b->units.size();
	if (join_mode) *join_mode = b->join_mode;
	return 0;
}

extern "C" size_t sonde_sample_bytes(int input_kind)
{
	return sd_sample_bytes(input_kind);
}

extern "C" size_t sonde_row_stride(size_t n_samples, int input_kind)
{
	const size_t elem = sonde_sample_bytes(input_kind);
	const size_t bytes = n_samples * elem;
	if (bytes < 64 * 1024) return n_samples;
	size_t p = 64 * 1024;
	while (p < bytes) p <<= 1;
	if (3 * p <= 4 * bytes) return p / elem;
	size_t units = (bytes + 65535) / 65536;
	units |= 1;
	return std::min(units * 65536, p) / elem;
}

extern "C" int sonde_batch_submit_host(SondeBatch *b, const void *samples, size_t n_samples, size_t channel_stride)
{
	if (!b || !samples) return fail("sonde_batch_submit_host: null argument");
	if (n_samples == 0 || n_samples % b->granule || n_samples > b->max_samples) return fail("sonde_batch_submit_host: bad n_samples");
	HIPCHK(hipSetDevice(b->device));
	const size_t elem = sonde_sample_bytes(b->input_kind);
	const size_t dstride = sonde_row_stride(n_samples, b->input_kind);
	const size_t need = (size_t)b->n_channels * sonde_row_stride(b->max_samples, b->input_kind) * elem;
	if (b->stage_bytes < need) {
		(void)hipFree(b->d_stage);
		b->d_stage = nullptr;
		b->stage_bytes = 0;
		HIPCHK(hipMalloc(&b->d_stage, need));
		b->stage_bytes = need;
	}
	if (b->pending) HIPCHK(hipStreamSynchronize(b->last_stream));
	HIPCHK(hipMemcpy2D(b->d_stage, dstride * elem, samples, channel_stride * elem, n_samples * elem, b->n_channels, hipMemcpyHostToDevice));
	return sonde_batch_submit(b, b->d_stage, n_samples, dstride, nullptr);
}

static long sync_ticket(SondeBatch *b, uint64_t ticket)
{
	if (ticket == 0 || ticket > b->tickets) return fail("sonde_batch: no such submit");
	if (b->tickets - ticket >= 2) return fail("sonde_batch: the frames of that submit have been overwritten (two newer submits)");
	if (hipSetDevice(b->device) != hipSuccess) return fail("hipSetDevice");
	const int slot = (int)((ticket - 1) & 1);
	if (!b->have_counts2[slot]) {
		hipError_t e = b->ev_valid[slot] ? hipEventSynchronize(b->ev_done[slot]) : hipStreamSynchronize(b->last_stream);
		if (e != hipSuccess) return fail("hipEventSynchronize", e);
		if (ticket == b->tickets || !b->ev_valid[slot]) b->pending = false;
		e = hipMemcpy(b->h_counts2[slot].data(), b->d_counts2[slot], b->n_channels * sizeof(uint32_t), hipMemcpyDeviceToHost);
		if (e != hipSuccess) return fail("hipMemcpy counts", e);
		if (b->sliced_once) {
			uint32_t gave_up = 0;
			e = hipMemcpy(&gave_up, b->d_prog + b->n_channels, sizeof(uint32_t), hipMemcpyDeviceToHost);
			if (e != hipSuccess) return fail("hipMemcpy prog", e);
			if (gave_up) return fail("sonde_batch: a time-sliced demod launch found a segment whose predecessor never finished (workgroup dispatch out of order?); the batch's state is undefined -- recreate it");
		}
		long n = 0, over = 0;
		for (uint32_t c = 0; c < b->n_channels; c++) {
			n += std::min(b->h_counts2[slot][c], b->max_frames);
			if (b->h_counts2[slot][c] > b->max_frames) over += b->h_counts2[slot][c] - b->max_frames;
		}
		b->n_frames2[slot] = n;
		b->n_overflow2[slot] = over;
		b->have_counts2[slot] = true;
	}
	return b->n_frames2[slot];
}

extern "C" long sonde_batch_sync(SondeBatch *b)
{
	if (!b) return fail("sonde_batch_sync: null argument");
	if (b->tickets == 0) return 0;
	return sync_ticket(b, b->tickets);
}

extern "C" uint64_t sonde_batch_ticket(SondeBatch *b)
{
	if (!b) return 0;
	b->ticketing = true;
	return b->tickets;
}

extern "C" long sonde_batch_overflow(SondeBatch *b)
{
	if (!b) return fail("sonde_batch_overflow: null argument");
	if (b->tickets == 0) return 0;
	if (sync_ticket(b, b->tickets) < 0) return -1;
	return b->n_overflow2[(b->tickets - 1) & 1];
}

extern "C" long sonde_batch_frames_of(SondeBatch *b, uint64_t ticket, SondeFrame *out, size_t cap)
{
	if (!b) return fail("sonde_batch_frames_of: null argument");
	const long n = sync_ticket(b, ticket);
	if (n < 0) return n;
	if (!out || cap == 0) return n;
	if (n == 0) return 0;
	const int slot = (int)((ticket - 1) & 1);
	const std::vector<uint32_t> &h_counts = b->h_counts2[slot];
	const SondeFrame *d_frames = b->d_frames2[slot];
	size_t k = 0;
	const size_t all = (size_t)b->n_channels * b->max_frames;
	if (all * sizeof(SondeFrame) <= (64u << 20)) {
		b->h_slots.resize(all);
		hipError_t e = hipMemcpy(b->h_slots.data(), d_frames, all * sizeof(SondeFrame), hipMemcpyDeviceToHost);
		if (e != hipSuccess) return fail("hipMemcpy frames", e);
		for (uint32_t c = 0; c < b->n_channels && k < cap; c++) {
			const uint32_t cnt = std::min(h_counts[c], b->max_frames);
			const size_t take = std::min((size_t)cnt, cap - k);
			if (take) memcpy(out + k, b->h_slots.data() + (size_t)c * b->max_frames, take * sizeof(SondeFrame));
			k += take;
		}
		return (long)k;
	}
	for (uint32_t c = 0; c < b->n_channels && k < cap; c++) {
		const uint32_t cnt = std::min(h_counts[c], b->max_frames);
		if (!cnt) continue;
		const size_t take = std::min((size_t)cnt, cap - k);
		hipError_t e = hipMemcpy(out + k, d_frames + (size_t)c * b->max_frames, take * sizeof(SondeFrame), hipMemcpyDeviceToHost);
		if (e != hipSuccess) return fail("hipMemcpy frames", e);
		k += take;
	}
	return (long)k;
}

extern "C" long sonde_batch_frames(SondeBatch *b, SondeFrame *out, size_t cap)
{
	if (!b) return fail("sonde_batch_frames: null argument");
	if (b->tickets == 0) return 0;
	return sonde_batch_frames_of(b, b->tickets, out, cap);
}

extern "C" long sonde_batch_poll(SondeBatch *b, SondeData *out, uint32_t *channel, size_t cap)
{
	if (!b || !out || !channel) return fail("sonde_batch_poll: null argument");
	while (b->polled_ticket < b->tickets) {
		const uint64_t t = b->polled_ticket + 1;
		if (b->tickets - t >= 2) {
			b->polled_ticket = b->tickets - 2;
			return fail("sonde_batch_poll: the frames of an unpolled submit have been overwritten (poll at least every second submit)");
		}
		const long n = sync_ticket(b, t);
		if (n < 0) return n;
		std::vector<SondeFrame> fr((size_t)n);
		const long got = n ? sonde_batch_frames_of(b, t, fr.data(), (size_t)n) : 0;
		if (got < 0) return got;
		if (b->parsers.empty()) b->parsers.resize(b->n_channels);
		std::vector<SondeData> v;
		for (long i = 0; i < got; i++) {
			const uint32_t c = fr[(size_t)i].channel;
			if (c >= b->n_channels) continue;
			if (!b->parsers[c]) b->parsers[c].reset(new SondeParser((int)b->types[c]));
			v.clear();
			b->parsers[c]->feed(fr[(size_t)i], v);
			for (const SondeData &d : v) b->frags.emplace_back(c, d);
		}
		b->polled_ticket = t;
	}
	size_t k = 0;
	while (k < cap && !b->frags.empty()) {
		channel[k] = b->frags.front().first;
		out[k] = b->frags.front().second;
		b->frags.pop_front();
		k++;
	}
	return (long)k;
}

extern "C" int sonde_batch_kernel_ms(SondeBatch *b, float *demod_ms, float *framer_ms)
{
	if (!b) return fail("sonde_batch_kernel_ms: null argument");
	if (sonde_batch_sync(b) < 0) return -1;
	float a = 0.0f, c = 0.0f;
	const int n = std::min(b->ev_used, (int)SondeBatch::kEvSlots);
	if (n == 0) return fail("sonde_batch_kernel_ms: no timed submit since the last query (sonde_batch_set_timing)");
	for (int i = 0; i < n; i++) {
		float x = 0.0f, y = 0.0f;
		HIPCHK(hipEventElapsedTime(&x, b->ev[3 * i], b->ev[3 * i + 1]));
		if (b->ev_has_framer[i]) HIPCHK(hipEventElapsedTime(&y, b->ev[3 * i + 1], b->ev[3 * i + 2]));
		a += x; c += y;
	}
	a /= (float)n; c /= (float)n;
	b->ev_used = 0;
	if (demod_ms) *demod_ms = a;
	if (framer_ms) *framer_ms = c;
	return 0;
}

extern "C" int sonde_batch_set_timing(SondeBatch *b, int every_n)
{
	if (!b || every_n < 0) return fail("sonde_batch_set_timing: bad argument");
	if (sonde_batch_sync(b) < 0) return -1;
	b->timing_every = every_n;
	b->n_submits = 0;
	b->ev_used = 0;
	b->evc_used = 0;
	return 0;
}

extern "C" int sonde_batch_class_ms(SondeBatch *b, float out[4])
{
	if (!b || !out) return fail("sonde_batch_class_ms: null argument");
	for (int k = 0; k < 4; k++) out[k] = -1.0f;
	if (!b->evc) return 0;
	if (sonde_batch_sync(b) < 0) return -1;
	const int n = std::min(b->evc_used, (int)SondeBatch::kEvSlots);
	const size_t nu = b->units.size();
	for (int k = 0; k < 4 && n > 0; k++) {
		float acc = 0.0f;
		int cnt = 0;
		for (size_t ui = 0; ui < nu; ui++) {
			const SondeBatch::Unit &u = b->units[ui];
			if (u.type == SONDE_IMET4 || u.type == SONDE_C50 || u.cls != k) continue;
			for (int i = 0; i < n; i++) {
				float x = 0.0f;
				HIPCHK(hipEventElapsedTime(&x, b->evc[2 * (nu * (size_t)i + ui)], b->evc[2 * (nu * (size_t)i + ui) + 1]));
				acc += x;
				cnt++;
			}
		}
		if (cnt) out[k] = acc / (float)cnt;
	}
	b->evc_used = 0;
	return n;
}

extern "C" int sonde_batch_test_rs255(SondeBatch *b, uint8_t *cw_pairs, size_t n_pairs, int n, int32_t *status)
{
	if (!b || !cw_pairs || !status || !n_pairs || n < 25 || n > 255) return fail("sonde_batch_test_rs255: bad argument");
	HIPCHK(hipSetDevice(b->device));
	uint8_t *d_cw = nullptr;
	int32_t *d_st = nullptr;
	HIPCHK(hipMalloc((void **)&d_cw, n_pairs * 512));
	if (hipMalloc((void **)&d_st, n_pairs * 2 * sizeof(int32_t)) != hipSuccess) { (void)hipFree(d_cw); return fail("hipMalloc"); }
	hipError_t e = hipMemcpy(d_cw, cw_pairs, n_pairs * 512, hipMemcpyHostToDevice);
	if (e == hipSuccess) {
		sd_launch_rs255_unit(d_cw, (uint32_t)n_pairs, n, d_st, b->d_gfexp, (const uint8_t *)b->d_gflog, b->d_gfswar, nullptr);
		e = hipGetLastError();
	}
	if (e == hipSuccess) e = hipMemcpy(cw_pairs, d_cw, n_pairs * 512, hipMemcpyDeviceToHost);
	if (e == hipSuccess) e = hipMemcpy(status, d_st, n_pairs * 2 * sizeof(int32_t), hipMemcpyDeviceToHost);
	(void)hipFree(d_cw); (void)hipFree(d_st);
	return e == hipSuccess ? 0 : fail("sonde_batch_test_rs255", e);
}

extern "C" uint64_t sonde_batch_nbits(SondeBatch *b, uint32_t channel)
{
	if (!b || channel >= b->n_channels) { fail("sonde_batch_nbits: bad argument"); return 0; }
	if (sonde_batch_sync(b) < 0) return 0;
	SdChanState st;
	if (hipMemcpy(&st, b->d_states + channel, sizeof(st), hipMemcpyDeviceToHost) != hipSuccess) { fail("hipMemcpy state"); return 0; }
	return st.wpos;
}

extern "C" int sonde_batch_read_bits(SondeBatch *b, uint32_t channel, uint64_t from, size_t count, uint8_t *out)
{
	if (!b || channel >= b->n_channels || !out) return fail("sonde_batch_read_bits: bad argument");
	if (sonde_batch_sync(b) < 0) return -1;
	SdChanState st;
	HIPCHK(hipMemcpy(&st, b->d_states + channel, sizeof(st), hipMemcpyDeviceToHost));
	const uint64_t ring_bits = (uint64_t)b->ring_words * 32;
	if (from + count > st.wpos || st.wpos - from > ring_bits) return fail("sonde_batch_read_bits: range not in the ring");
	std::vector<uint32_t> ring(b->ring_words);
	HIPCHK(hipMemcpy(ring.data(), b->d_bitring + (size_t)channel * b->ring_words, (size_t)b->ring_words * 4, hipMemcpyDeviceToHost));
	for (size_t i = 0; i < count; i++) {
		const uint64_t p = from + i;
		out[i] = (ring[(p >> 5) & (b->ring_words - 1)] >> (p & 31)) & 1u;
	}
	return 0;
}

extern "C" int sonde_batch_read_state(SondeBatch *b, uint32_t channel, int64_t *t_next, int32_t *period, float *bias, float *amp, float *afc_u)
{
	if (!b || channel >= b->n_channels) return fail("sonde_batch_read_state: bad argument");
	if (sonde_batch_sync(b) < 0) return -1;
	SdChanState st;
	HIPCHK(hipMemcpy(&st, b->d_states + channel, sizeof(st), hipMemcpyDeviceToHost));
	if (t_next) *t_next = st.t_next;
	if (period) *period = st.period;
	if (bias) *bias = st.bias;
	if (amp) *amp = st.amp;
	if (afc_u) *afc_u = st.afc[2];
	return 0;
}

typedef uint32_t sd_u32x4 __attribute__((ext_vector_type(4)));
__global__ __launch_bounds__(256) void sd_read_probe_kernel(const sd_u32x4 *__restrict__ src, size_t n16, uint32_t *sink)
{
	const size_t stride = (size_t)gridDim.x * 256;
	size_t i = (size_t)blockIdx.x * 256 + threadIdx.x;
	uint32_t acc = 0;
	for (; i + 7 * stride < n16; i += 8 * stride) {
		sd_u32x4 v[8];
#pragma unroll
		for (int k = 0; k < 8; k++) v[k] = __builtin_nontemporal_load(src + i + k * stride);
#pragma unroll
		for (int k = 0; k < 8; k++) acc ^= v[k].x ^ v[k].y ^ v[k].z ^ v[k].w;
	}
	for (; i < n16; i += stride) {
		const sd_u32x4 v = src[i];
		acc ^= v.x ^ v.y ^ v.z ^ v.w;
	}
	if (acc == 0x5EEDBEEFu) sink[0] = acc;
}

extern "C" int sonde_hbm_read_probe(const void *d_buf, size_t bytes, int reps, float *gbs_out)
{
	if (!d_buf || bytes < 16 || reps < 1 || !gbs_out) return fail("sonde_hbm_read_probe: bad argument");
	uint32_t *sink = nullptr;
	HIPCHK(hipMalloc(&sink, 4));
	hipEvent_t e0, e1;
	HIPCHK(hipEventCreate(&e0));
	HIPCHK(hipEventCreate(&e1));
	const size_t n16 = bytes / 16;
	float best = 1e30f;
	for (int grid = 256 * 4; grid <= 256 * 32; grid *= 2) {
		sd_read_probe_kernel<<<grid, 256>>>((const sd_u32x4 *)d_buf, n16, sink);
		for (int r = 0; r < reps; r++) {
			(void)hipEventRecord(e0, 0);
			sd_read_probe_kernel<<<grid, 256>>>((const sd_u32x4 *)d_buf, n16, sink);
			(void)hipEventRecord(e1, 0);
			(void)hipEventSynchronize(e1);
			float ms = 0.f;
			(void)hipEventElapsedTime(&ms, e0, e1);
			if (ms < best) best = ms;
		}
	}
	const hipError_t err = hipGetLastError();
	(void)hipEventDestroy(e0);
	(void)hipEventDestroy(e1);
	(void)hipFree(sink);
	if (err != hipSuccess) return fail("sonde_hbm_read_probe", err);
	*gbs_out = (float)((double)(n16 * 16) / ((double)best * 1e-3) / 1e9);
	return 0;
}
```

### sdrpp_radiosonde_amd/csrc/bins_kernel.hip

```cpp
#include <hip/hip_runtime.h>
#include <atomic>
#include "sonde_dev.h"
#include "sd_input.h"
#include "sd_math.h"
#include "sd_wave.h"
#include "sd_rs41.h"
#include "sd_rsdec.h"
#include "sd_fixed.h"
#include "launch.h"

#define BK_WAVES 8
#define BK_IT    (SD_TILE / 4)
#define BK_SPILL 128
#define BK_A     (SD_LH + BK_IT + BK_SPILL + 4)
#define BK_PASS_PH 336
#define BK_NT    8
#define BK_SLOTS 4

struct BinsWaveLds {
	float A[BK_A];
	alignas(16) float d[BK_PASS_PH + 8];
	uint32_t chunk[10];
	uint32_t mirror[SD_MIRROR_WORDS];
	SdFrameDesc k4list[SD_K4_LIST];
};
struct BinsLds {
	BinsWaveLds w[BK_WAVES];
	alignas(16) float taps[BK_SLOTS][SD_NPHASE * SD_TAPS_LD];
	EpiTabs et;
};
static_assert(sizeof(FramerLds) <= sizeof(float) * BK_A, "the FEC work area aliases the tile buffer");
static_assert(sizeof(BinsLds) <= 80 * 1024, "two workgroups per CU: 16 bins in flight per CU, 4096 bins in one generation");

__device__ __forceinline__ int bk_slot(int type) { return type == SONDE_RS41 ? 0 : type == SONDE_DFM09 ? 1 : type == SONDE_IMS100 ? 2 : 3; }

#ifdef BK_TS
__device__ unsigned long long g_bk_ts[64];
extern "C" int sonde_debug_bins_ts(unsigned long long *out) { return hipMemcpyFromSymbol(out, HIP_SYMBOL(g_bk_ts), sizeof(g_bk_ts)) == hipSuccess ? 0 : -1; }
#define BK_STAMP(i) do { if (ch == 1000u && lane == 0) g_bk_ts[i] = __builtin_readcyclecounter(); } while (0)
#else
#define BK_STAMP(i) do { } while (0)
#endif

struct SdBinsParams {
	SdFramerOut fo;
	SdModem modems[SONDE_NTYPES];
	int utype;
};

__global__ __launch_bounds__(64 * BK_WAVES, 4) void sd_bins_kernel(
	const int16_t *__restrict__ phases, size_t row_stride , int n_blocks,
	int16_t *__restrict__ carry_rows, size_t carry_stride ,
	SdChanState *__restrict__ states, float *__restrict__ hist, uint32_t *__restrict__ bitring, uint32_t ring_words,
	const float *__restrict__ taps_all, const float *__restrict__ g_comp , uint32_t n_channels, const SdBinsParams P)
{
	__shared__ __attribute__((aligned(16))) BinsLds s;
	const int tid = threadIdx.x, lane = tid & 63;
	const int wave = __builtin_amdgcn_readfirstlane(tid >> 6);
	const uint32_t ch = blockIdx.x * (blockDim.x >> 6) + (uint32_t)wave;
	if (ch >= n_channels) return;
	BinsWaveLds &w = s.w[wave];
	BK_STAMP(0);

	const uint32_t *row32 = reinterpret_cast<const uint32_t *>(phases + (size_t)ch * row_stride);
	const uint4 *row128 = reinterpret_cast<const uint4 *>(row32);
	uint4 ph[4];
	const int n_pass = 8 * n_blocks;
	auto load_pass = [&](int gp, uint4 &p) {
		p = lane < 42 ? row128[40 * (size_t)gp + lane] : make_uint4(0u, 0u, 0u, 0u);
	};
	load_pass(0, ph[0]); load_pass(1, ph[1]); load_pass(2, ph[2]);
	const uint32_t sv = lane < 16 ? reinterpret_cast<const uint32_t *>(states + ch)[lane] : (lane < 24 ? reinterpret_cast<const uint32_t *>(P.fo.fstates + ch)[lane - 16] : 0u);
	const float hv = lane >= SD_HIST - 16 ? hist[(size_t)ch * SD_HIST + lane] : 0.0f;
	auto svw = [&](int i) { return (uint32_t)__builtin_amdgcn_readlane((int)sv, i); };
	auto sv64 = [&](int i) { return (uint64_t)svw(i) | ((uint64_t)svw(i + 1) << 32); };
	SdChanState st;
	st.t_next = (int64_t)sv64(0); st.n0 = (int64_t)sv64(2); st.wpos = sv64(4); st.period = (int32_t)svw(6); st.nstat = (int32_t)svw(7);
	st.bias = __uint_as_float(svw(8)); st.amp = __uint_as_float(svw(9)); st.iq_last[0] = __uint_as_float(svw(10)); st.iq_last[1] = __uint_as_float(svw(11));
	st.type = (int32_t)svw(12); st.afc[0] = __uint_as_float(svw(13)); st.afc[1] = __uint_as_float(svw(14)); st.afc[2] = __uint_as_float(svw(15));
	SdFramerState f0;
	f0.rpos = sv64(16); f0.fstart = sv64(18); f0.collecting = (int32_t)svw(20); f0.inv = (int32_t)svw(21); f0.flen = (int32_t)svw(22); f0.pad = 0;
	const int stype = P.utype >= 0 ? P.utype : st.type;
	const SdModem md = P.modems[stype];
	const bool is_rs41 = stype == SONDE_RS41, is_dfm = stype == SONDE_DFM09, is_ims = stype == SONDE_IMS100, is_mrz = stype == SONDE_MRZN1;
	const bool fuse = P.fo.fuse_fec != 0;
	const bool framing = is_rs41 || (fuse && (is_dfm || is_ims || is_mrz));
	const bool fec_here = is_rs41 && fuse;
	uint32_t *ring_g = bitring + (size_t)ch * ring_words;
	const uint32_t ring_mask = ring_words - 1;
	const uint32_t wi = (uint32_t)(st.wpos >> 5) - (uint32_t)(63 - lane);
	const uint32_t xw = __hip_atomic_load(ring_g + (wi & ring_mask), __ATOMIC_RELAXED, __HIP_MEMORY_SCOPE_AGENT);
	float *const taps = s.taps[bk_slot(stype)];
	{
		const float4 *taps_g = reinterpret_cast<const float4 *>(taps_all + (size_t)stype * SD_NPHASE * SD_NTAPS);
#pragma unroll
		for (int q = 0; q < 4; q++) {
			const int i = lane + 64 * q, rowi = i >> 3, c4 = i & 7;
			const float4 tv = taps_g[i];
			*reinterpret_cast<float4 *>(&taps[rowi * SD_TAPS_LD + 4 * c4]) = make_float4(tv.y, tv.x, tv.w, tv.z);
		}
	}
	if (lane < 10) w.chunk[lane] = 0u;
	WAVE_SYNC();
	BK_STAMP(1);

	auto pass = [&](const uint4 p, int out0 ) {
		{
			typedef unsigned short u16x2 __attribute__((ext_vector_type(2)));
			const uint32_t below = (uint32_t)__builtin_amdgcn_update_dpp(0, (int)p.w, 0x138, 0xF, 0xF, false);
			const uint32_t x0 = __builtin_amdgcn_alignbit(p.x, below, 16), x1 = __builtin_amdgcn_alignbit(p.y, p.x, 16),
			               x2 = __builtin_amdgcn_alignbit(p.z, p.y, 16), x3 = __builtin_amdgcn_alignbit(p.w, p.z, 16);
			const uint32_t e0 = __builtin_bit_cast(uint32_t, __builtin_bit_cast(u16x2, p.x) - __builtin_bit_cast(u16x2, x0));
			const uint32_t e1 = __builtin_bit_cast(uint32_t, __builtin_bit_cast(u16x2, p.y) - __builtin_bit_cast(u16x2, x1));
			const uint32_t e2 = __builtin_bit_cast(uint32_t, __builtin_bit_cast(u16x2, p.z) - __builtin_bit_cast(u16x2, x2));
			const uint32_t e3 = __builtin_bit_cast(uint32_t, __builtin_bit_cast(u16x2, p.w) - __builtin_bit_cast(u16x2, x3));
			if (lane < 42) {
				float4 *dst = reinterpret_cast<float4 *>(&w.d[8 * lane]);
				dst[0] = sd_cs16_f4(make_uint2(e0, e1));
				dst[1] = sd_cs16_f4(make_uint2(e2, e3));
			}
		}
		WAVE_SYNC();
		typedef const __attribute__((address_space(4))) float *CTab;
		unsigned long long g_addr = (unsigned long long)g_comp;
		asm volatile("" : "+s"(g_addr));
		const CTab g_pass = (CTab)g_addr;
		float dv[20];
		const float *dp = &w.d[5 * lane + 1];
#pragma unroll
		for (int k = 0; k < 20; k++) dv[k] = dp[k];
#pragma unroll
		for (int c = 0; c < 3; c++) {
			constexpr int BO[3] = {1, 2, 4};
			const int bo = BO[c] + 15;
			const CTab gt = g_pass + SD_RS_KT_LD * c;
			float acc = 0.0f;
#pragma unroll
			for (int t = 0; t < SD_RS_KT; t++) acc = __builtin_fmaf(gt[t], dv[bo - t], acc);
			w.A[out0 + 3 * lane + c] = acc;
		}
		WAVE_SYNC();
	};

	int64_t n0 = st.n0;
	uint64_t wpos = st.wpos;
	uint32_t partial = 0;
	SdSyncRun k4;
	auto tile_rounds = [&]() {
		n0 += BK_IT;
		const int64_t limit = (((n0 - 1 - BK_NT / 2 - SD_MARGIN) << 16) | 0xFFFF);
		int K = (st.t_next <= limit) ? (int)((uint32_t)(limit - st.t_next) / (uint32_t)st.period) + 1 : 0;
		if (K > SD_ROUND_MAX) K = SD_ROUND_MAX;
		const int64_t base = (n0 - BK_IT - SD_LH) << 16;
		const uint32_t rel0 = (uint32_t)(st.t_next - base);
		const float bias = st.bias;
		int Ei = 0, S1i = 0, S0i = 0, C1 = 0;
#pragma unroll
		for (int hh = 0; hh < 4; hh += 2) {
			float y[2], m[2];
#pragma unroll
			for (int h = 0; h < 2; h++) {
				const uint32_t rel = rel0 + __umul24((unsigned)(sd_hw_symbol(lane) + 64 * (hh + h)), (unsigned)st.period);
				y[h] = interp<BK_NT>(w.A, taps, rel);
				m[h] = interp<BK_NT>(w.A, taps, rel - ((uint32_t)st.period >> 1));
			}
#pragma unroll
			for (int h = 0; h < 2; h++) {
				const bool act = sd_hw_symbol(lane) + 64 * (hh + h) < K;
				const float yy = act ? y[h] : 0.0f;
				const float yprev = sd_hw_prev(yy, lane);
				float e = (yprev - yy) * (m[h] - bias);
				e = sd_clamp(e * 1024.0f, -1.0e6f, 1.0e6f);
				Ei += (act && lane != 0) ? __float2int_rn(e) : 0;
				const bool bit = act && (yy > bias);
				const int Y = __float2int_rn(sd_clamp(yy, -8.0f, 8.0f) * 4096.0f);
				S1i += bit ? Y : 0;
				S0i += (act && !bit) ? Y : 0;
				const unsigned long long bal = __ballot(sd_hw_unpermute(bit ? 1 : 0, lane) != 0);
				C1 += __popcll(bal);
				if (lane == 0) { w.chunk[1 + 2 * (hh + h)] = (uint32_t)bal; w.chunk[2 + 2 * (hh + h)] = (uint32_t)(bal >> 32); }
			}
		}
		const int E = wave_sum(Ei), S1 = wave_sum(S1i), S0 = wave_sum(S0i);
		WAVE_SYNC();
		if (K <= 0) return;
		if (lane < 9) {
			const uint32_t sh = (uint32_t)wpos & 31u, w0 = (uint32_t)(wpos >> 5);
			uint32_t vv = 0;
			if ((uint32_t)(32 * lane) < sh + (uint32_t)K) {
				const uint32_t lo = w.chunk[lane + 1], pvw = w.chunk[lane];
				vv = sh ? ((lo << sh) | (pvw >> (32u - sh))) : lo;
				if (lane == 0 && sh) vv |= partial & ((1u << sh) - 1u);
				const uint32_t idx = (w0 + (uint32_t)lane) & ring_mask;
				ring_g[idx] = vv;
				w.mirror[idx & (SD_MIRROR_WORDS - 1)] = vv;
			}
			partial = vv;
		}
		partial = (uint32_t)__builtin_amdgcn_readlane((int)partial, (int)((((uint32_t)wpos & 31u) + (uint32_t)K) >> 5));
		wpos += (uint64_t)K;
		const int C0 = K - C1;
		if (C1 > 0 && C0 > 0) {
			const f32x2 cnt = {(float)C1, (float)C0};
			const f32x2 rc = sd_recip2(cnt);
			const float hi = ((float)S1 * rc.x) * (1.0f / 4096.0f);
			const float lo = ((float)S0 * rc.y) * (1.0f / 4096.0f);
			const float c = 0.5f * (hi + lo), a = 0.5f * (hi - lo);
			if (st.nstat == 0) { st.bias = c; st.amp = a; }
			else { st.bias = st.bias + 0.5f * (c - st.bias); st.amp = st.amp + 0.5f * (a - st.amp); }
			if (!(st.amp >= 1.0e-3f)) st.amp = 1.0e-3f;
			st.nstat = 1;
		} else {
			st.bias = ((float)(S1 + S0) * sd_recip((float)K)) * (1.0f / 4096.0f);
		}
		if (n0 <= 3 * (int64_t)BK_IT) st.bias = ((float)(S1 + S0) * sd_recip((float)K)) * (1.0f / 4096.0f);
		const f32x2 den = {(float)K, st.amp * st.amp};
		const f32x2 rd = sd_recip2(den);
		float err = ((float)E * rd.x) * (1.0f / 1024.0f);
		err = err * rd.y;
		err = sd_clamp(err, -1.0f, 1.0f);
		const int dphase = __float2int_rn(err * md.kp), dper = __float2int_rn(err * md.ki);
		st.t_next += (int64_t)K * st.period + dphase;
		st.period += dper;
		if (st.period < md.pmin) st.period = md.pmin;
		if (st.period > md.pmax) st.period = md.pmax;
	};
	auto k4_block = [&]() {
		if (!framing) return;
		WAVE_SYNC();
		SdFrameDesc *dch = (SdFrameDesc *)P.fo.descs + (size_t)ch * P.fo.max_frames;
		const uint32_t mf = P.fo.max_frames;
		if (is_rs41) sd_rs41_sync_step<true>(k4, wpos, w.mirror, lane, dch, mf, w.k4list);
		else if (is_dfm) sd_fixed_sync_step<SONDE_DFM09, true>(k4, wpos, w.mirror, lane, dch, mf, w.k4list);
		else if (is_ims) sd_fixed_sync_step<SONDE_IMS100, true>(k4, wpos, w.mirror, lane, dch, mf, w.k4list);
		else sd_fixed_sync_step<SONDE_MRZN1, true>(k4, wpos, w.mirror, lane, dch, mf, w.k4list);
	};
	auto roll = [&]() {
		const float h0 = w.A[BK_IT + lane], h1 = w.A[BK_IT + 64 + lane], h2 = w.A[BK_IT + 128 + lane];
		WAVE_SYNC();
		w.A[lane] = h0; w.A[64 + lane] = h1; w.A[128 + lane] = h2;
		WAVE_SYNC();
	};

	for (int b = 0; b < n_blocks; b++) {
		const int gp = 8 * b;
		load_pass(gp + 3, ph[3]);                         pass(ph[0], SD_LH + 0);     
		load_pass(gp + 4, ph[0]);                         pass(ph[1], SD_LH + 192);   
		load_pass(gp + 5, ph[1]);                         pass(ph[2], SD_LH + 384);   BK_STAMP(5);
		if (b == 0) {
			w.A[lane] = hv;
			w.mirror[wi & (SD_MIRROR_WORDS - 1)] = xw;
			partial = ((uint32_t)st.wpos & 31u) ? (uint32_t)__builtin_amdgcn_readlane((int)xw, 63) : 0u;
			k4.rpos = f0.rpos; k4.fstart = f0.fstart; k4.collecting = f0.collecting; k4.inv = f0.inv; k4.flen = f0.flen; k4.nout = 0; k4.wp_seen = 0;
			WAVE_SYNC();
			BK_STAMP(2);
		}
		tile_rounds(); BK_STAMP(6); roll(); 
		load_pass(gp + 6, ph[2]);                         pass(ph[3], SD_LH + 64);    
		load_pass(gp + 7, ph[3]);                         pass(ph[0], SD_LH + 256);   
		if (gp + 8 < n_pass) load_pass(gp + 8, ph[0]);    pass(ph[1], SD_LH + 448);   BK_STAMP(10);
		tile_rounds(); BK_STAMP(11); roll();
		if (gp + 9 < n_pass) load_pass(gp + 9, ph[1]);    pass(ph[2], SD_LH + 128);   
		if (gp + 10 < n_pass) load_pass(gp + 10, ph[2]);  pass(ph[3], SD_LH + 320);   BK_STAMP(13);
		tile_rounds(); BK_STAMP(14); roll();
		k4_block();
	}

	if (lane >= SD_HIST - 16) hist[(size_t)ch * SD_HIST + lane] = w.A[lane];
	if (lane < 8) {
		const size_t n_ph = 2560 * (size_t)n_blocks;
		reinterpret_cast<uint32_t *>(carry_rows + (size_t)ch * carry_stride)[lane] = row32[n_ph / 2 + lane];
	}
	if (lane == 0) {
		st.n0 = n0;
		st.wpos = wpos;
		states[ch] = st;
		if (framing) {
			SdFramerState f1;
			f1.rpos = k4.rpos; f1.fstart = k4.fstart; f1.collecting = k4.collecting; f1.inv = k4.inv; f1.flen = k4.flen; f1.pad = 0;
			P.fo.fstates[ch] = f1;
			P.fo.counts[ch] = k4.nout;
		}
	}
	BK_STAMP(15);
	if (fec_here) {
		const uint32_t max_frames = P.fo.max_frames;
		const uint32_t nfr = min((uint32_t)__builtin_amdgcn_readfirstlane((int)k4.nout), max_frames);
		if (nfr) {
			for (int i = lane; i < GF_EXP2 / 16 + 512 / 16 + RS_R * 8 * 4 / 16; i += 64) {
				if (i < GF_EXP2 / 16) reinterpret_cast<uint4 *>(s.et.tabs.exp2)[i] = reinterpret_cast<const uint4 *>(P.fo.gf_exp)[i];
				else if (i < GF_EXP2 / 16 + 512 / 16) reinterpret_cast<uint4 *>(s.et.tabs.log2)[i - GF_EXP2 / 16] = reinterpret_cast<const uint4 *>(P.fo.gf_log)[i - GF_EXP2 / 16];
				else reinterpret_cast<uint4 *>(s.et.swar)[i - (GF_EXP2 / 16 + 512 / 16)] = reinterpret_cast<const uint4 *>(P.fo.gf_swar)[i - (GF_EXP2 / 16 + 512 / 16)];
			}
			WAVE_SYNC();
			FramerLds &wl = *reinterpret_cast<FramerLds *>(&w.A[0]);
			GfSwar swar;
			const uint32_t *sw = s.et.swar + 8 * (lane % RS_R);
			swar.a_lo = sw[0]; swar.a_hi = sw[1]; swar.b_lo = sw[2]; swar.b_hi = sw[3]; swar.c = sw[4];
			const unsigned long long *dg = reinterpret_cast<const unsigned long long *>((const SdFrameDesc *)P.fo.descs + (size_t)ch * max_frames);
			SondeFrame *fout = P.fo.frames + (size_t)ch * max_frames;
			for (uint32_t k = 0; k < nfr; k++) {
				unsigned long long d0, d1;
				if (k < SD_K4_LIST) {
					const unsigned long long *dl = reinterpret_cast<const unsigned long long *>(&w.k4list[k]);
					d0 = dl[0]; d1 = dl[1];
				} else {
					d0 = __hip_atomic_load(dg + 2 * k, __ATOMIC_RELAXED, __HIP_MEMORY_SCOPE_AGENT);
					d1 = __hip_atomic_load(dg + 2 * k + 1, __ATOMIC_RELAXED, __HIP_MEMORY_SCOPE_AGENT);
				}
				SdFrameDesc d;
				d.fstart = sd_uniform64(d0);
				d.flen = __builtin_amdgcn_readfirstlane((int)(uint32_t)d1);
				d.inv = __builtin_amdgcn_readfirstlane((int)(d1 >> 32));
				sd_rs41_decode_frame<true>(s.et.tabs, wl, swar, ring_g, ring_mask, d, fout + k, ch, lane);
			}
		}
	}
	BK_STAMP(16);
}

void sd_launch_bins(uint32_t n_channels, hipStream_t stream, const int16_t *phases, size_t row_stride, int n_blocks,
	int16_t *carry_rows, size_t carry_stride, SdChanState *states, float *hist, uint32_t *bitring, uint32_t ring_words,
	const float *taps_all, const SdModem *modems_host, const SdFramerOut *fo_host, const float *g_comp, int utype)
{
	int wpw = BK_WAVES;
	{
		static std::atomic<int> cus_of[64];
		int dev = 0, cus = 256;
		if (hipGetDevice(&dev) == hipSuccess && dev >= 0 && dev < 64) {
			int known = cus_of[dev].load(std::memory_order_relaxed);
			if (!known && hipDeviceGetAttribute(&known, hipDeviceAttributeMultiprocessorCount, dev) == hipSuccess && known > 0) cus_of[dev].store(known, std::memory_order_relaxed);
			if (known > 0) cus = known;
		}
		while (wpw > 1 && (n_channels + wpw - 1) / wpw < (uint32_t)cus) wpw >>= 1;
	}
	const dim3 g((n_channels + wpw - 1) / wpw), blk(64 * wpw);
	SdBinsParams P;
	P.fo = *fo_host;
	for (int t = 0; t < SONDE_NTYPES; t++) P.modems[t] = modems_host[t];
	P.utype = utype;
	hipLaunchKernelGGL(sd_bins_kernel, g, blk, 0, stream, phases, row_stride, n_blocks, carry_rows, carry_stride, states, hist, bitring,
	                   ring_words, taps_all, g_comp, n_channels, P);
}
```

### sdrpp_radiosonde_amd/csrc/channelizer.hip

```cpp
#include <hip/hip_runtime.h>
#include <math.h>
#include <stdlib.h>
#include <string.h>
#include <type_traits>
#include <string>
#include <vector>
#include "sd_math.h"
#include "sonde_dev.h"
#include "sd_input.h"
#include "../../include/sonde_abi.h"
#include "launch.h"

#define CH_M 512
#define CH_D 500
#define CH_T 16
#define CH_L (CH_M * CH_T)
#define CH_H (CH_L - CH_D)
#define RS_UP 12
#define RS_DN 5
#define RS_TAPS 16
#define PH_HEAD 16

#define P_S    8
#define P_NT   (64 * P_S)
#define P_NS   (CH_T + P_S - 1)
#define P_WIN  (CH_L + (P_S - 1) * CH_D)
#define P_NOWRAP ((CH_M - (P_S - 1) * (CH_M - CH_D)) / 64)
#define PFB_FB (CH_M + CH_M / 8)
#define P_OT   (P_S + 1)
static_assert(P_NT == CH_M, "fold: one thread per window column; FFT: one wave per step");
static_assert(CH_M * P_OT <= 2 * P_S * PFB_FB, "the phase tile aliases the FFT buffers");
static_assert(3 * ((CH_L / 2 + 128) * sizeof(float) + P_S * PFB_FB * sizeof(float2)) <= 160 * 1024, "three workgroups per CU");

#ifdef P_TS
__device__ unsigned long long g_pfb_ts[128];
extern "C" int sonde_debug_pfb_ts(unsigned long long *out) { return hipMemcpyFromSymbol(out, HIP_SYMBOL(g_pfb_ts), sizeof(g_pfb_ts)) == hipSuccess ? 0 : -1; }
#define P_STAMP(i) do { if (blockIdx.x == P_TS_WG && blockIdx.y == 0 && (threadIdx.x & 63) == 0) g_pfb_ts[8 * (i) + (threadIdx.x >> 6)] = __builtin_readcyclecounter(); } while (0)
#ifndef P_TS_WG
#define P_TS_WG 100
#endif
#else
#define P_STAMP(i) do { } while (0)
#endif

__device__ __forceinline__ void pfb_bfly(float2 &a, float2 &b, const float2 w)
{
	const float tr = __builtin_fmaf(-b.y, w.y, b.x * w.x);
	const float ti = __builtin_fmaf(b.x, w.y, b.y * w.x);
	const float2 a0 = a;
	a = make_float2(a0.x + tr, a0.y + ti);
	b = make_float2(a0.x - tr, a0.y - ti);
}

__device__ __forceinline__ void pfb_bfly_one(float2 &a, float2 &b)
{
	const float2 a0 = a, b0 = b;
	a = make_float2(a0.x + b0.x, a0.y + b0.y);
	b = make_float2(a0.x - b0.x, a0.y - b0.y);
}
__device__ __forceinline__ void pfb_bfly_mj(float2 &a, float2 &b)
{
	const float2 a0 = a, b0 = b;
	a = make_float2(a0.x + b0.y, a0.y - b0.x);
	b = make_float2(a0.x - b0.y, a0.y + b0.x);
}
struct PfbTw { float2 a2, b2[2], c2[4], a3, b3[2], c3[4]; };
__device__ __forceinline__ PfbTw pfb_load_tw(const float2 *__restrict__ tw, int lane)
{
	PfbTw t;
	const int lo = lane >> 3;
	t.a2 = tw[lo * 32];
#pragma unroll
	for (int k = 0; k < 2; k++) t.b2[k] = tw[(lo + 8 * k) * 16];
#pragma unroll
	for (int k = 0; k < 4; k++) t.c2[k] = tw[(lo + 8 * k) * 8];
	t.a3 = tw[lane * 4];
#pragma unroll
	for (int k = 0; k < 2; k++) t.b3[k] = tw[(lane + 64 * k) * 2];
#pragma unroll
	for (int k = 0; k < 4; k++) t.c3[k] = tw[lane + 64 * k];
	return t;
}
#define PFB_WSYNC() do { __builtin_amdgcn_fence(__ATOMIC_SEQ_CST, "wavefront"); __builtin_amdgcn_wave_barrier(); } while (0)
__device__ __forceinline__ void pfb_fft512n(float2 *fb, const float2 w64 , const float2 w128 , const float2 w192 ,
                                            const PfbTw &t, int lane, float2 (&e)[8])
{
	constexpr int BR3[8] = {0, 4, 2, 6, 1, 5, 3, 7};
	(void)w128;
#pragma unroll
	for (int j = 0; j < 8; j++) e[j] = fb[lane + 64 * BR3[j]];
#pragma unroll
	for (int j = 0; j < 8; j += 2) pfb_bfly_one(e[j], e[j + 1]);
#pragma unroll
	for (int j = 0; j < 8; j++) if ((j & 2) == 0) { if (j & 1) pfb_bfly_mj(e[j], e[j + 2]); else pfb_bfly_one(e[j], e[j + 2]); }
	pfb_bfly_one(e[0], e[4]); pfb_bfly(e[1], e[5], w64); pfb_bfly_mj(e[2], e[6]); pfb_bfly(e[3], e[7], w192);
	PFB_WSYNC();
#pragma unroll
	for (int j = 0; j < 8; j++) fb[72 * j + lane] = e[j];
	PFB_WSYNC();
	{
		const int lo = lane >> 3, hp = lane & 7;
#pragma unroll
		for (int j = 0; j < 8; j++) e[j] = fb[72 * lo + 8 * BR3[j] + hp];
#pragma unroll
		for (int j = 0; j < 8; j += 2) pfb_bfly(e[j], e[j + 1], t.a2);
#pragma unroll
		for (int j = 0; j < 8; j++) if ((j & 2) == 0) pfb_bfly(e[j], e[j + 2], t.b2[j & 1]);
#pragma unroll
		for (int j = 0; j < 4; j++) pfb_bfly(e[j], e[j + 4], t.c2[j]);
		PFB_WSYNC();
#pragma unroll
		for (int j = 0; j < 8; j++) fb[9 * (lo + 8 * j) + hp] = e[j];
	}
	PFB_WSYNC();
#pragma unroll
	for (int j = 0; j < 8; j++) e[j] = fb[9 * lane + BR3[j]];
#pragma unroll
	for (int j = 0; j < 8; j += 2) pfb_bfly(e[j], e[j + 1], t.a3);
#pragma unroll
	for (int j = 0; j < 8; j++) if ((j & 2) == 0) pfb_bfly(e[j], e[j + 2], t.b3[j & 1]);
#pragma unroll
	for (int j = 0; j < 4; j++) pfb_bfly(e[j], e[j + 4], t.c3[j]);
}

template <int IK>
__global__ __launch_bounds__(P_NT, 6) void sd_pfb_kernel(const void *__restrict__ iq_all_, size_t stream_stride,
                                                           const void *__restrict__ hist_in_all_, void *__restrict__ hist_out_all_,
                                                           const float *__restrict__ h_even, const float2 *__restrict__ tw,
                                                           int16_t *__restrict__ phi_all, uint32_t n_steps, uint32_t xcd_map,
                                                           uint32_t dual, const float *__restrict__ h_odd, const float2 *__restrict__ twist)
{
	__shared__ __attribute__((aligned(16))) float s_h_[CH_L / 2 + 128];
	float *const s_h = s_h_ + 128;
	__shared__ __attribute__((aligned(16))) float2 s_x[P_S * PFB_FB];
	const int tid = threadIdx.x, lane = tid & 63, wave = __builtin_amdgcn_readfirstlane(tid >> 6);
	uint32_t grp, sidx;
	if (xcd_map == 2u) {
		const uint32_t lin = blockIdx.x + gridDim.x * blockIdx.y, j = lin >> 3;
		sidx = (lin & 7u) + 8u * (j / gridDim.x);
		grp = j % gridDim.x;
	} else {
		grp = xcd_map ? (blockIdx.x & 7u) * (gridDim.x >> 3) + (blockIdx.x >> 3) : blockIdx.x;
		sidx = blockIdx.y;
	}
	const uint32_t m0 = grp * P_S;
	const bool odd = dual && (sidx & 1u);
	const uint32_t phys = dual ? sidx >> 1 : sidx;
	const float *h = odd ? h_odd : h_even;
	using ET = sd_iq_t<IK>;
	using PT = typename std::conditional<IK == SONDE_INPUT_IQ8, uint32_t, typename std::conditional<IK == SONDE_INPUT_IQ16, uint2, float4>::type>::type;
	const ET *iq = reinterpret_cast<const ET *>(iq_all_) + (size_t)phys * stream_stride;
	const ET *hist_in = reinterpret_cast<const ET *>(hist_in_all_) + (size_t)phys * CH_H;
	ET *hist_out_all = reinterpret_cast<ET *>(hist_out_all_);
	const size_t prow = (size_t)n_steps + PH_HEAD;
	int16_t *phi = phi_all + (size_t)sidx * CH_M * prow + PH_HEAD;
	const long p0 = (long)m0 * CH_D - CH_H;
	const int c = tid;
	P_STAMP(0);
	ET xr[P_NS];
	auto stage = [&](auto get) {
#pragma unroll
		for (int k = 0; k < 8; k++) { xr[k] = get(k); __builtin_amdgcn_sched_barrier(0); }
		float hreg[CH_T / 2];
#pragma unroll
		for (int t = 0; t < CH_T / 2; t++) hreg[t] = h[c + t * CH_M];
		__builtin_amdgcn_sched_barrier(0);
#pragma unroll
		for (int k = 8; k < P_NS; k++) { xr[k] = get(k); __builtin_amdgcn_sched_barrier(0); }
#pragma unroll
		for (int t = 0; t < CH_T / 2; t++) s_h[c + t * CH_M] = hreg[t];
	};
	if (p0 >= 0) {
		const ET *src = iq + p0 + c;
		stage([&](int k) -> ET { return (k < P_NS - 1 || c + CH_M * k < P_WIN) ? src[CH_M * k] : ET{}; });
	} else {
		stage([&](int k) -> ET {
			const long pos = p0 + c + CH_M * k;
			return (k < P_NS - 1 || c + CH_M * k < P_WIN) ? (pos < 0 ? hist_in[CH_H + pos] : iq[pos]) : ET{};
		});
	}
	P_STAMP(1);
	if (grp == gridDim.x - 1 && !odd) {
		const PT *tail = reinterpret_cast<const PT *>(iq + (size_t)n_steps * CH_D - CH_H);
		PT *ho = reinterpret_cast<PT *>(hist_out_all + (size_t)phys * CH_H);
		for (int i = tid; i < CH_H / 2; i += P_NT) ho[i] = tail[i];
	}
	__syncthreads();
	P_STAMP(2);
	float2 v[P_S];
#pragma unroll
	for (int q = 0; q < P_S; q++) v[q] = make_float2(0.0f, 0.0f);
	auto fold = [&](auto edge_c, auto odd_c) {
		constexpr bool edge = decltype(edge_c)::value, ODD = decltype(odd_c)::value;
		const float *hq = s_h + c;
		const float *hm = s_h + (CH_L - 1) - c;
		float hk[P_S], he = 0.0f;
		auto mir = [&](int off) -> float { const float m = hm[-off]; return ODD ? -m : m; };
		auto taps_of = [&](int k, float (&hh)[P_S], float &hm1) {
#pragma unroll
			for (int q = 0; q < P_S; q++) {
				const int d = k - q, off = (CH_M - CH_D) * q + CH_M * d;
				if (d >= 0 && d < CH_T / 2 - 1) hh[q] = hq[off];
				else if (d == CH_T / 2 - 1) {
					if (edge) { const float a = hq[off], b = mir(off); hh[q] = c + (CH_M - CH_D) * q < CH_M ? a : b; }
					else hh[q] = hq[off];
				} else if (d >= CH_T / 2 && d < CH_T) hh[q] = mir(off);
				else hh[q] = 0.0f;
			}
			hm1 = 0.0f;
			if (edge && k + 1 < P_S) hm1 = hq[(CH_M - CH_D) * (k + 1) - CH_M];
		};
#pragma unroll
		for (int k = 0; k < P_NS; k++) {
			taps_of(k, hk, he);
			const float2 xv = sd_iq_f2<IK>(xr[k]);
			if (edge && k + 1 < P_S) {
				const int q = k + 1;
				const bool ok = c + (CH_M - CH_D) * q >= CH_M;
				const float nx = __builtin_fmaf(he, xv.x, v[q].x), ny = __builtin_fmaf(he, xv.y, v[q].y);
				v[q].x = ok ? nx : v[q].x;
				v[q].y = ok ? ny : v[q].y;
			}
#pragma unroll
			for (int q = 0; q < P_S; q++) {
				const int d = k - q;
				if (d >= 0 && d < CH_T - 1) {
					v[q].x = __builtin_fmaf(hk[q], xv.x, v[q].x);
					v[q].y = __builtin_fmaf(hk[q], xv.y, v[q].y);
				} else if (d == CH_T - 1) {
					const float nx = __builtin_fmaf(hk[q], xv.x, v[q].x), ny = __builtin_fmaf(hk[q], xv.y, v[q].y);
					const bool ok = !edge || c + (CH_M - CH_D) * q < CH_M;
					v[q].x = ok ? nx : v[q].x;
					v[q].y = ok ? ny : v[q].y;
				}
			}
#ifndef P_NOSB
			__builtin_amdgcn_sched_barrier(0);
#endif
		}
	};
	if (wave < P_NOWRAP) { if (odd) fold(std::false_type{}, std::true_type{}); else fold(std::false_type{}, std::false_type{}); }
	else { if (odd) fold(std::true_type{}, std::true_type{}); else fold(std::true_type{}, std::false_type{}); }
	P_STAMP(3);
	const float2 w64 = tw[64], w128 = tw[128], w192 = tw[192];
	const PfbTw twr = pfb_load_tw(tw, lane);
	if (odd) {
#pragma unroll
		for (int q = 0; q < P_S; q++) {
			const float2 w = twist[(c + (CH_M - CH_D) * q) & (CH_M - 1)];
			const float tr = __builtin_fmaf(-v[q].y, w.y, v[q].x * w.x), ti = __builtin_fmaf(v[q].x, w.y, v[q].y * w.x);
			v[q] = make_float2(tr, ti);
		}
	}
	{
		const uint32_t pos = ((uint32_t)c + m0 * (uint32_t)CH_D) & (CH_M - 1);
#pragma unroll
		for (int q = 0; q < P_S; q++) s_x[q * PFB_FB + pos] = v[q];
	}
	__syncthreads();
	P_STAMP(4);
	float2 e0[8];
	pfb_fft512n(s_x + wave * PFB_FB, w64, w128, w192, twr, lane, e0);
	P_STAMP(5);
	float ph[8];
#pragma unroll
	for (int j = 0; j < 8; j++) ph[j] = sd_atan2q(e0[j].y, e0[j].x);
	P_STAMP(6);
	__syncthreads();
	P_STAMP(7);
	float *const s_t = reinterpret_cast<float *>(s_x);
#pragma unroll
	for (int j = 0; j < 8; j++) s_t[(lane + 64 * j) * P_OT + wave] = ph[j];
	__syncthreads();
	P_STAMP(8);
	{
		const float *row = s_t + tid * P_OT;
		uint32_t q[P_S];
#pragma unroll
		for (int j = 0; j < P_S; j++) {
			q[j] = (uint32_t)__float2int_rn(row[j] * 16384.0f);
			if (odd) q[j] -= 32000u * (m0 + (uint32_t)j);
			q[j] &= 0xffffu;
		}
		*reinterpret_cast<uint4 *>(phi + (size_t)tid * prow + m0) = make_uint4(q[0] | (q[1] << 16), q[2] | (q[3] << 16), q[4] | (q[5] << 16), q[6] | (q[7] << 16));
	}
	P_STAMP(9);
}

__global__ __launch_bounds__(256) void sd_phase_resamp_kernel(const int16_t *__restrict__ phi, uint32_t n_steps,
                                                               const float *__restrict__ g, int32_t *__restrict__ phi_last,
                                                               float *__restrict__ dhist, float *__restrict__ out48)
{
	extern __shared__ float s_d[];
	__shared__ float s_g[RS_UP * RS_TAPS];
	const uint32_t k = blockIdx.x;
	const int tid = threadIdx.x;
	const int16_t *x = phi + (size_t)k * (n_steps + PH_HEAD) + PH_HEAD;
	if (tid < RS_UP * RS_TAPS) s_g[tid] = g[tid];
	if (tid < RS_TAPS) s_d[tid] = dhist[(size_t)k * RS_TAPS + tid];
	const int first_prev = phi_last[k];
	for (uint32_t i = tid; i < n_steps; i += 256) s_d[RS_TAPS + i] = (float)(int16_t)(uint16_t)((int)x[i] - (i ? (int)x[i - 1] : first_prev)) * (1.0f / 16384.0f);
	__syncthreads();
	const uint32_t n_out = n_steps * RS_UP / RS_DN;
	for (uint32_t j = tid; j < n_out; j += 256) {
		const uint32_t i0 = (j * RS_DN) / RS_UP, p = (j * RS_DN) % RS_UP;
		float acc = 0.0f;
#pragma unroll
		for (int t = 0; t < RS_TAPS; t++) acc = __builtin_fmaf(s_g[p * RS_TAPS + t], s_d[RS_TAPS + i0 - t], acc);
		out48[(size_t)k * n_out + j] = acc;
	}
	if (tid < RS_TAPS) dhist[(size_t)k * RS_TAPS + tid] = s_d[n_steps + tid];
	if (tid == 0) phi_last[k] = x[n_steps - 1];
}

static thread_local std::string g_cerr;
extern "C" const char *sonde_last_error(void);

struct SondeChannelizer {
	int device = 0;
	uint32_t n_steps = 0, n_streams = 1;
	int input_kind = SONDE_INPUT_IQ;
	uint32_t n_phys = 1, dual = 0;
	float *d_h_odd = nullptr; float2 *d_twist = nullptr;
	bool fused = false;
	hipStream_t last_stream = nullptr;
	hipEvent_t ev_xs = nullptr;
	uint32_t xcd_map = 0;
	bool overlap = false;
	hipStream_t s_pfb = nullptr, s_dec = nullptr;
	hipEvent_t ev_in = nullptr, ev_pfb[2] = {}, ev_dec[2] = {};
	int16_t *d_bins_b = nullptr;
	int16_t *d_bins_last = nullptr;
	SondeBatch *batch = nullptr;
	float2 *d_hist[2] = {}, *d_tw = nullptr;
	int16_t *d_bins = nullptr;
	int32_t *d_philast = nullptr;
	float *d_h = nullptr, *d_g = nullptr, *d_gc = nullptr, *d_dhist = nullptr, *d_out48 = nullptr;
	hipEvent_t ev[3] = {};
	unsigned long n_submits = 0, n_blocks = 0;
	double acc_ms[2] = { 0.0, 0.0 };
	int n_timed = 0;
	bool ev_pending = false;
};

static void composite_rows(const std::vector<float> &g, int dec, float *G )
{
	for (int phi = 0; phi < 3; phi++) {
		const int newest = (RS_DN * (dec * phi + dec - 1)) / RS_UP;
		for (int k = 0; k < SD_RS_KT_LD; k++) {
			double acc = 0.0;
			for (int j = dec * phi; j < dec * phi + dec; j++) {
				const int t = k - (newest - (RS_DN * j) / RS_UP);
				if (t >= 0 && t < RS_TAPS) acc += (double)g[((RS_DN * j) % RS_UP) * RS_TAPS + t];
			}
			G[phi * SD_RS_KT_LD + k] = (float)(acc / (double)dec);
		}
	}
}

static void make_tables(std::vector<float> &h, std::vector<float> &tw, std::vector<float> &g)
{
	const double PI = 3.14159265358979323846;
	h.resize(CH_L); tw.resize(CH_M); g.resize(RS_UP * RS_TAPS);
	{
		const double fc = 8000.0 / 10000000.0;
		std::vector<double> tmp(CH_L);
		double sum = 0.0;
		for (int i = 0; i < CH_L; i++) {
			const double t = (double)i - 0.5 * (double)(CH_L - 1);
			const double x = (double)i / (double)(CH_L - 1);
			const double w = 0.42 - 0.5 * cos(2.0 * PI * x) + 0.08 * cos(4.0 * PI * x);
			const double s = (t == 0.0) ? 2.0 * fc : sin(2.0 * PI * fc * t) / (PI * t);
			tmp[i] = s * w;
			sum += tmp[i];
		}
		for (int i = 0; i < CH_L; i++) h[i] = (float)(tmp[i] / sum);
	}
	for (int k = 0; k < CH_M / 2; k++) {
		tw[2 * k] = (float)cos(2.0 * PI * (double)k / (double)CH_M);
		tw[2 * k + 1] = (float)(-sin(2.0 * PI * (double)k / (double)CH_M));
	}
	tw[2 * 128] = 0.0f;
	{
		const int N = RS_UP * RS_TAPS;
		const double fc = 9000.0 / 240000.0;
		std::vector<double> tmp(N);
		for (int i = 0; i < N; i++) {
			const double t = (double)i - 0.5 * (double)(N - 1);
			const double x = (double)i / (double)(N - 1);
			const double w = 0.42 - 0.5 * cos(2.0 * PI * x) + 0.08 * cos(4.0 * PI * x);
			const double s = (t == 0.0) ? 2.0 * fc : sin(2.0 * PI * fc * t) / (PI * t);
			tmp[i] = s * w;
		}
		for (int p = 0; p < RS_UP; p++) {
			double sum = 0.0;
			for (int t = 0; t < RS_TAPS; t++) sum += tmp[t * RS_UP + p];
			for (int t = 0; t < RS_TAPS; t++) g[p * RS_TAPS + t] = (float)(tmp[t * RS_UP + p] / sum);
		}
	}
}

extern "C" void sonde_chan_destroy(SondeChannelizer *c)
{
	if (!c) return;
	(void)hipSetDevice(c->device);
	sonde_batch_destroy(c->batch);
	for (int i = 0; i < 3; i++) if (c->ev[i]) (void)hipEventDestroy(c->ev[i]);
	if (c->ev_xs) (void)hipEventDestroy(c->ev_xs);
	if (c->ev_in) (void)hipEventDestroy(c->ev_in);
	for (int i = 0; i < 2; i++) { if (c->ev_pfb[i]) (void)hipEventDestroy(c->ev_pfb[i]); if (c->ev_dec[i]) (void)hipEventDestroy(c->ev_dec[i]); }
	if (c->s_pfb) (void)hipStreamDestroy(c->s_pfb);
	if (c->s_dec) (void)hipStreamDestroy(c->s_dec);
	(void)hipFree(c->d_bins_b);
	(void)hipFree(c->d_hist[0]); (void)hipFree(c->d_hist[1]); (void)hipFree(c->d_bins); (void)hipFree(c->d_tw); (void)hipFree(c->d_philast);
	(void)hipFree(c->d_h); (void)hipFree(c->d_g); (void)hipFree(c->d_dhist); (void)hipFree(c->d_out48); (void)hipFree(c->d_gc); (void)hipFree(c->d_h_odd); (void)hipFree(c->d_twist);
	delete c;
}

static int chan_create(const uint8_t *types, uint32_t blocks_per_submit, uint32_t n_phys, uint32_t dual, int device, SondeChannelizer **out);
extern "C" int sonde_chan_create_multi(const uint8_t *types, uint32_t blocks_per_submit, uint32_t n_streams, int device, SondeChannelizer **out)
{
	return chan_create(types, blocks_per_submit, n_streams, 0, device, out);
}
extern "C" int sonde_chan_create_dual(const uint8_t *types, uint32_t blocks_per_submit, uint32_t n_streams, int device, SondeChannelizer **out)
{
	return chan_create(types, blocks_per_submit, n_streams, 1, device, out);
}
static int chan_create(const uint8_t *types, uint32_t blocks_per_submit, uint32_t n_phys, uint32_t dual, int device, SondeChannelizer **out)
{
	const uint32_t n_streams = n_phys * (dual ? 2u : 1u);
	if (!out || blocks_per_submit == 0 || blocks_per_submit > 8 || n_streams == 0 || n_streams > 64) return -1;
	*out = nullptr;
	for (size_t i = 0; types && i < (size_t)n_streams * CH_M; i++)
		if (types[i] == SONDE_M10) return sd_fail("sonde_chan_create: an M10 / M20 channel (50 kHz) does not fit a 19.5 kHz channelizer bin; use sonde_vfo_* at 50 kS/s", hipSuccess);
	SondeChannelizer *c = new SondeChannelizer;
	c->device = device;
	c->n_streams = n_streams;
	c->n_phys = n_phys;
	c->dual = dual;
	c->n_steps = 2560u * blocks_per_submit;
	c->xcd_map = (c->n_steps / P_S) % 8 == 0 && (size_t)(c->n_steps / P_S) * n_streams > 1024;
	if (c->xcd_map && !dual && n_streams % 8 == 0) c->xcd_map = 2;
	const uint32_t n_out = c->n_steps * RS_UP / RS_DN;
	const size_t nb = (size_t)n_streams * CH_M;
	SondeBatchConfig cfg = SONDE_BATCH_CONFIG_INIT;
	cfg.n_channels = (uint32_t)nb;
	cfg.types = types;
	cfg.max_samples = n_out;
	cfg.input_kind = SONDE_INPUT_REAL;
	cfg.device = device;
	cfg.flags = 0;
	if (sonde_batch_create(&cfg, &c->batch) != 0) { delete c; return -1; }
	std::vector<float> h, tw, g;
	make_tables(h, tw, g);
	const size_t hist_bytes = (size_t)n_phys * CH_H * sizeof(float2);
	bool ok = hipMalloc((void **)&c->d_hist[0], hist_bytes) == hipSuccess && hipMalloc((void **)&c->d_hist[1], hist_bytes) == hipSuccess &&
	          hipMalloc((void **)&c->d_bins, nb * ((size_t)c->n_steps + PH_HEAD) * sizeof(int16_t)) == hipSuccess &&
	          (blocks_per_submit > 2 || hipMalloc((void **)&c->d_out48, nb * n_out * sizeof(float)) == hipSuccess) &&
	          hipMalloc((void **)&c->d_h, CH_L * sizeof(float)) == hipSuccess &&
	          hipMalloc((void **)&c->d_tw, CH_M * sizeof(float)) == hipSuccess &&
	          hipMalloc((void **)&c->d_g, RS_UP * RS_TAPS * sizeof(float)) == hipSuccess &&
	          hipMalloc((void **)&c->d_philast, nb * sizeof(int32_t)) == hipSuccess &&
	          hipMalloc((void **)&c->d_dhist, nb * RS_TAPS * sizeof(float)) == hipSuccess;
	ok = ok && hipMemset(c->d_hist[0], 0, hist_bytes) == hipSuccess && hipMemset(c->d_hist[1], 0, hist_bytes) == hipSuccess && hipMemset(c->d_philast, 0, nb * sizeof(int32_t)) == hipSuccess && hipMemset(c->d_bins, 0, nb * ((size_t)c->n_steps + PH_HEAD) * sizeof(int16_t)) == hipSuccess &&
	     hipMemset(c->d_dhist, 0, nb * RS_TAPS * sizeof(float)) == hipSuccess &&
	     [&] { for (int i = 0; i < CH_L / 2; i++) if (memcmp(&h[i], &h[CH_L - 1 - i], sizeof(float))) return false; return true; }() &&
	     hipMemcpy(c->d_h, h.data(), CH_L * sizeof(float), hipMemcpyHostToDevice) == hipSuccess &&
	     hipMemcpy(c->d_tw, tw.data(), CH_M * sizeof(float), hipMemcpyHostToDevice) == hipSuccess &&
	     hipMemcpy(c->d_g, g.data(), RS_UP * RS_TAPS * sizeof(float), hipMemcpyHostToDevice) == hipSuccess;
	for (int i = 0; i < 3 && ok; i++) ok = hipEventCreateWithFlags(&c->ev[i], hipEventDisableSystemFence) == hipSuccess;
	ok = ok && hipEventCreateWithFlags(&c->ev_xs, hipEventDisableTiming | hipEventDisableSystemFence) == hipSuccess;
	if (ok) {
		float gc[3 * SD_RS_KT_LD];
		composite_rows(g, 4, gc);
		for (float &v : gc) v *= 1.0f / 16384.0f;
		ok = hipMalloc((void **)&c->d_gc, sizeof(gc)) == hipSuccess && hipMemcpy(c->d_gc, gc, sizeof(gc), hipMemcpyHostToDevice) == hipSuccess;
		if (ok && dual) {
			const double PI = 3.14159265358979323846;
			std::vector<float> ho(h), wt(2 * CH_M);
			for (int i = 0; i < CH_L; i++) if ((i / CH_M) & 1) ho[i] = -ho[i];
			for (int r = 0; r < CH_M; r++) { wt[2 * r] = (float)cos(PI * (double)r / (double)CH_M); wt[2 * r + 1] = (float)(-sin(PI * (double)r / (double)CH_M)); }
			ok = hipMalloc((void **)&c->d_h_odd, CH_L * sizeof(float)) == hipSuccess && hipMalloc((void **)&c->d_twist, CH_M * sizeof(float2)) == hipSuccess &&
			     hipMemcpy(c->d_h_odd, ho.data(), CH_L * sizeof(float), hipMemcpyHostToDevice) == hipSuccess &&
			     hipMemcpy(c->d_twist, wt.data(), CH_M * sizeof(float2), hipMemcpyHostToDevice) == hipSuccess;
		}
		c->fused = sd_batch_bins_capable(c->batch);
		if (!c->fused && blocks_per_submit > 2) ok = false;
		c->overlap = false;
	}
	if (!ok) { sonde_chan_destroy(c); return -1; }
	*out = c;
	return 0;
}

extern "C" int sonde_chan_create(const uint8_t *types, uint32_t blocks_per_submit, int device, SondeChannelizer **out)
{
	return sonde_chan_create_multi(types, blocks_per_submit, 1, device, out);
}
extern "C" uint32_t sonde_chan_streams(const SondeChannelizer *c) { return c ? c->n_phys : 0; }
extern "C" uint32_t sonde_chan_channels(const SondeChannelizer *c) { return c ? c->n_streams * CH_M : 0; }
extern "C" int sonde_chan_set_fused(SondeChannelizer *c, int on)
{
	if (!c) return -1;
	if (on < 0) return c->fused ? 1 : 0;
	if (c->n_blocks == 0 && (on || c->d_out48)) c->fused = on && sd_batch_bins_capable(c->batch);
	return c->fused ? 1 : 0;
}

extern "C" int sonde_chan_set_overlap(SondeChannelizer *c, int on)
{
	if (!c) return -1;
	if (c->n_blocks == 0) c->overlap = on && c->fused;
	return c->overlap ? 1 : 0;
}

static bool chan_overlap_setup(SondeChannelizer *c)
{
	if (c->s_pfb) return true;
	const size_t nb = (size_t)c->n_streams * CH_M;
	bool ok = hipStreamCreateWithFlags(&c->s_pfb, hipStreamNonBlocking) == hipSuccess && hipStreamCreateWithFlags(&c->s_dec, hipStreamNonBlocking) == hipSuccess &&
	          hipEventCreateWithFlags(&c->ev_in, hipEventDisableTiming | hipEventDisableSystemFence) == hipSuccess &&
	          hipMalloc((void **)&c->d_bins_b, nb * ((size_t)c->n_steps + PH_HEAD) * sizeof(int16_t)) == hipSuccess &&
	          hipMemset(c->d_bins_b, 0, nb * ((size_t)c->n_steps + PH_HEAD) * sizeof(int16_t)) == hipSuccess;
	for (int i = 0; i < 2 && ok; i++)
		ok = hipEventCreateWithFlags(&c->ev_pfb[i], hipEventDisableTiming | hipEventDisableSystemFence) == hipSuccess &&
		     hipEventCreateWithFlags(&c->ev_dec[i], hipEventDisableTiming | hipEventDisableSystemFence) == hipSuccess;
	return ok;
}

extern "C" int sonde_chan_set_input(SondeChannelizer *c, int input_kind)
{
	if (!c) return -1;
	if (c->n_blocks == 0 && sd_input_known(input_kind) && input_kind != SONDE_INPUT_REAL) c->input_kind = input_kind;
	return c->input_kind;
}

static void launch_pfb(SondeChannelizer *c, hipStream_t st, const void *iq_dev, size_t n_samples, int16_t *bins)
{
	const dim3 g(c->n_steps / P_S, c->n_streams), blk(P_NT);
	const void *hin = c->d_hist[c->n_blocks & 1];
	void *hout = c->d_hist[(c->n_blocks + 1) & 1];
	sd_input_dispatch(c->input_kind, [&](auto k) {
		if constexpr (decltype(k)::value != SONDE_INPUT_REAL)
			hipLaunchKernelGGL(sd_pfb_kernel<decltype(k)::value>, g, blk, 0, st, iq_dev, n_samples, hin, hout, c->d_h, c->d_tw, bins, c->n_steps, c->xcd_map, c->dual,
				c->d_h_odd, c->d_twist);
	});
}

extern "C" uint32_t sonde_chan_samples_per_submit(const SondeChannelizer *c) { return c ? c->n_steps * CH_D : 0; }
extern "C" SondeBatch *sonde_chan_batch(SondeChannelizer *c) { return c ? c->batch : nullptr; }

extern "C" int sonde_chan_submit(SondeChannelizer *c, const void *iq_dev, size_t n_samples, void *stream_)
{
	if (!c || !iq_dev || n_samples != (size_t)c->n_steps * CH_D) return -1;
	hipStream_t stream = (hipStream_t)stream_;
	if (hipSetDevice(c->device) != hipSuccess) return -1;
	const uint32_t n_out = c->n_steps * RS_UP / RS_DN;
	if (c->ev_pending && hipEventQuery(c->ev[2]) == hipSuccess) {
		float a = 0.f, b = 0.f;
		if (hipEventElapsedTime(&a, c->ev[0], c->ev[1]) == hipSuccess && hipEventElapsedTime(&b, c->ev[1], c->ev[2]) == hipSuccess) {
			c->acc_ms[0] += a; c->acc_ms[1] += b; c->n_timed++;
		}
		c->ev_pending = false;
	}
	const bool timed = !c->ev_pending && ((c->n_submits % 8) == 7 || c->n_blocks == 0);
	c->n_submits++;
	if ((uintptr_t)iq_dev & 15u) return -1;
	c->overlap = c->overlap && c->fused;
	if (c->overlap) {
		if (!chan_overlap_setup(c)) return -1;
		const int b = (int)(c->n_blocks & 1);
		int16_t *bins = b ? c->d_bins_b : c->d_bins;
		int16_t *bins_next = b ? c->d_bins : c->d_bins_b;
		if (hipEventRecord(c->ev_in, stream) != hipSuccess || hipStreamWaitEvent(c->s_pfb, c->ev_in, 0) != hipSuccess) return -1;
		if (c->n_blocks >= 2 && hipStreamWaitEvent(c->s_pfb, c->ev_dec[b], 0) != hipSuccess) return -1;
		if (timed) (void)hipEventRecord(c->ev[0], c->s_pfb);
		launch_pfb(c, c->s_pfb, iq_dev, n_samples, bins);
		c->n_blocks++;
		c->d_bins_last = bins;
		if (timed) { (void)hipEventRecord(c->ev[1], c->s_pfb); (void)hipEventRecord(c->ev[2], c->s_pfb); c->ev_pending = true; }
		if (hipEventRecord(c->ev_pfb[b], c->s_pfb) != hipSuccess) return -1;
		if (hipStreamWaitEvent(stream, c->ev_pfb[b], 0) != hipSuccess || hipStreamWaitEvent(c->s_dec, c->ev_pfb[b], 0) != hipSuccess) return -1;
		if (hipGetLastError() != hipSuccess) return -1;
		c->last_stream = stream;
		const SdBinsArgs ba = { bins, (size_t)c->n_steps + PH_HEAD, bins_next, (size_t)c->n_steps + PH_HEAD, c->d_gc };
		if (sd_batch_submit_bins(c->batch, &ba, c->n_steps, (void *)c->s_dec) != 0) return -1;
		return hipEventRecord(c->ev_dec[b], c->s_dec) == hipSuccess ? 0 : -1;
	}
	if (c->n_blocks && stream != c->last_stream) {
		if (hipEventRecord(c->ev_xs, c->last_stream) != hipSuccess || hipStreamWaitEvent(stream, c->ev_xs, 0) != hipSuccess) return -1;
	}
	c->last_stream = stream;
	if (timed) (void)hipEventRecord(c->ev[0], stream);
	launch_pfb(c, stream, iq_dev, n_samples, c->d_bins);
	c->n_blocks++;
	c->d_bins_last = c->d_bins;
	if (timed) (void)hipEventRecord(c->ev[1], stream);
	if (!c->fused)
		hipLaunchKernelGGL(sd_phase_resamp_kernel, dim3(CH_M * c->n_streams), dim3(256), (RS_TAPS + c->n_steps) * sizeof(float), stream,
		                   c->d_bins, c->n_steps, c->d_g, c->d_philast, c->d_dhist, c->d_out48);
	if (timed) { (void)hipEventRecord(c->ev[2], stream); c->ev_pending = true; }
	if (hipGetLastError() != hipSuccess) return -1;
	if (c->fused) {
		const SdBinsArgs ba = { c->d_bins, (size_t)c->n_steps + PH_HEAD, c->d_bins, (size_t)c->n_steps + PH_HEAD, c->d_gc };
		return sd_batch_submit_bins(c->batch, &ba, c->n_steps, stream_);
	}
	return sonde_batch_submit(c->batch, c->d_out48, n_out, n_out, stream_);
}

extern "C" int sonde_chan_kernel_ms(SondeChannelizer *c, float *pfb_ms, float *disc_resamp_ms, float *demod_ms, float *framer_ms)
{
	if (!c) return -1;
	if (hipSetDevice(c->device) != hipSuccess || hipDeviceSynchronize() != hipSuccess) return -1;
	if (c->ev_pending) {
		float a = 0.f, b = 0.f;
		if (hipEventElapsedTime(&a, c->ev[0], c->ev[1]) == hipSuccess && hipEventElapsedTime(&b, c->ev[1], c->ev[2]) == hipSuccess) {
			c->acc_ms[0] += a; c->acc_ms[1] += b; c->n_timed++;
		}
		c->ev_pending = false;
	}
	if (c->n_timed == 0) return -1;
	if (pfb_ms) *pfb_ms = (float)(c->acc_ms[0] / c->n_timed);
	if (disc_resamp_ms) *disc_resamp_ms = (float)(c->acc_ms[1] / c->n_timed);
	c->acc_ms[0] = c->acc_ms[1] = 0.0;
	c->n_timed = 0;
	c->n_submits = 0;
	return sonde_batch_kernel_ms(c->batch, demod_ms, framer_ms);
}

extern "C" int sonde_chan_read(SondeChannelizer *c, float *bins , float *out48 )
{
	if (!c) return -1;
	if (hipSetDevice(c->device) != hipSuccess || hipDeviceSynchronize() != hipSuccess) return -1;
	const uint32_t n_out = c->n_steps * RS_UP / RS_DN;
	const size_t nb = (size_t)c->n_streams * CH_M;
	if (bins) {
		const size_t prow = (size_t)c->n_steps + PH_HEAD;
		std::vector<int16_t> tmp(nb * prow);
		if (hipMemcpy(tmp.data(), c->d_bins_last ? c->d_bins_last : c->d_bins, tmp.size() * sizeof(int16_t), hipMemcpyDeviceToHost) != hipSuccess) return -1;
		for (size_t k = 0; k < nb; k++)
			for (size_t m = 0; m < c->n_steps; m++) bins[k * c->n_steps + m] = (float)tmp[k * prow + PH_HEAD + m] * (1.0f / 16384.0f);
	}
	if (out48 && c->fused) return -1;
	if (out48 && hipMemcpy(out48, c->d_out48, nb * n_out * sizeof(float), hipMemcpyDeviceToHost) != hipSuccess) return -1;
	return 0;
}

extern "C" int sonde_chan_tables(float *h , float *tw , float *g )
{
	std::vector<float> vh, vt, vg;
	make_tables(vh, vt, vg);
	if (h) memcpy(h, vh.data(), vh.size() * sizeof(float));
	if (tw) memcpy(tw, vt.data(), vt.size() * sizeof(float));
	if (g) memcpy(g, vg.data(), vg.size() * sizeof(float));
	return 0;
}
```

### sdrpp_radiosonde_amd/csrc/launch.h

```cpp
#pragma once
#include <hip/hip_runtime.h>
#include "sonde_dev.h"
#include "../../include/sonde_abi.h"

struct SdFramerOut {
	SdFramerState *fstates; void *descs; uint32_t *counts; uint32_t max_frames;
	uint32_t fuse_fec;
	uint32_t loop_fec_max_wg;
	const uint8_t *gf_exp, *gf_log; const uint32_t *gf_swar;
	const uint8_t *gf64;
	SondeFrame *frames;
	const uint16_t *m10tab;
	uint32_t fixed_epi;
};
struct SdSlice {
	int32_t   n_seg;
	int32_t   seg_tiles;
	uint32_t  n_wg;
	uint32_t  seg_base;
	uint32_t *prog;
	uint32_t  err_index;
};
bool sd_slices_supported(int in_kind, int decim, int nt);
void sd_launch_demod(int in_kind, int decim, int nt, uint32_t n_channels, hipStream_t stream,
	const float *in, size_t ch_stride, int n_tiles, SdChanState *states, float *hist,
	uint32_t *bitring, uint32_t ring_words, const float *taps_all, const SdModem *modems,
	const uint32_t *chlist, bool compact_in, const SdFramerOut *fo ,
	int utype ,
	const SdSlice *slice = nullptr );
void sd_launch_demod_mixed(int in_kind, uint32_t n_a, const uint32_t *list_a, int utype_a, uint32_t n_b, const uint32_t *list_b, int utype_b, hipStream_t stream,
	const float *in, size_t ch_stride, int n_tiles, SdChanState *states, float *hist, uint32_t *bitring, uint32_t ring_words,
	const float *taps_all, const SdModem *modems, const SdFramerOut *fo );
struct SdBinsArgs { const int16_t *phases; size_t row_stride; int16_t *carry_rows; size_t carry_stride; const float *g_comp ; };
void sd_launch_bins(uint32_t n_channels, hipStream_t stream, const int16_t *phases, size_t row_stride, int n_blocks,
	int16_t *carry_rows, size_t carry_stride, SdChanState *states, float *hist, uint32_t *bitring, uint32_t ring_words,
	const float *taps_all, const SdModem *modems_host , const SdFramerOut *fo_host ,
	const float *g_comp, int utype );
int sd_batch_submit_bins(SondeBatch *b, const SdBinsArgs *ba, size_t n_steps, void *stream);
int sd_batch_bins_capable(const SondeBatch *b);

void sd_launch_afsk(int type , int kind , uint32_t n_list, hipStream_t stream, const float *in, size_t ch_stride, int n_tiles,
	const uint32_t *chlist, SdAfskState *astates, const float *wtab, float *out, size_t out_stride);
void sd_launch_framer_imet(uint32_t n_list, hipStream_t stream, const SdChanState *states, SdFramerState *fstates,
	const uint32_t *bitring, uint32_t ring_words, SondeFrame *frames, uint32_t *counts, uint32_t max_frames, const uint32_t *chlist);
void sd_launch_framer_c50(uint32_t n_list, hipStream_t stream, const SdChanState *states, SdFramerState *fstates,
	const uint32_t *bitring, uint32_t ring_words, SondeFrame *frames, uint32_t *counts, uint32_t max_frames, const uint32_t *chlist);

#define SD_DESC_BYTES 16
void sd_launch_framer_rs41(uint32_t n_list, hipStream_t stream, const uint32_t *bitring, uint32_t ring_words,
	const uint8_t *gf_exp, const uint8_t *gf_log, const uint32_t *gf_swar, const void *descs,
	SondeFrame *frames, const uint32_t *counts, uint32_t max_frames, uint32_t grid_frames, const uint32_t *chlist);

void sd_launch_framer_other(int type, uint32_t n_list, hipStream_t stream,
	const SdChanState *states, SdFramerState *fstates, const uint32_t *bitring, uint32_t ring_words,
	const uint8_t *g64, void *descs, SondeFrame *frames, uint32_t *counts, uint32_t max_frames, uint32_t grid_frames, const uint32_t *chlist,
	bool with_sync );

void sd_launch_rs255_unit(uint8_t *cw_io, uint32_t n_pairs, int n, int32_t *status, const uint8_t *gf_exp, const uint8_t *gf_log,
	const uint32_t *gf_swar, hipStream_t stream);

void make_mixer(float *out, int cycles, int per);

int sd_fail(const char *what, hipError_t e = hipSuccess);
```

### sdrpp_radiosonde_amd/csrc/sd_rs41.h

```cpp
#pragma once
#include <hip/hip_runtime.h>
#include "sonde_dev.h"

#define SD_K4_LIST 8
#define RS41_SYNC_THR 6
#define RS41_LEN_STD  320
#define RS41_LEN_EXT  518
#define RS41_TYPE_POS 56
#define RS41_TYPE_MASK 0x78u

#define RS41_SYNC_LO 0x11CAB610u
#define RS41_SYNC_HI 0xF8129622u

struct SdSyncRun {
	uint64_t rpos, fstart;
	int32_t collecting, inv, flen;
	uint32_t nout;
	uint64_t wp_seen;
	SdFrameDesc list[SD_K4_LIST];
};

__device__ __forceinline__ uint64_t sd_uniform64(unsigned long long v)
{
	return ((uint64_t)(uint32_t)__builtin_amdgcn_readfirstlane((int)(v >> 32)) << 32) |
	       (uint32_t)__builtin_amdgcn_readfirstlane((int)(uint32_t)v);
}

template <bool REG = false, int NCHUNK = (REG ? 4 : 1)>
__device__ __forceinline__ void sd_rs41_sync_step(SdSyncRun &lds_state, uint64_t wp, const uint32_t *mirror, int lane,
	SdFrameDesc *__restrict__ descs_ch, uint32_t max_frames, SdFrameDesc *list = nullptr)
{
	if (!REG) list = lds_state.list;
	SdSyncRun fs;
	fs.rpos = sd_uniform64(lds_state.rpos); fs.fstart = sd_uniform64(lds_state.fstart);
	fs.collecting = __builtin_amdgcn_readfirstlane(lds_state.collecting);
	fs.inv = __builtin_amdgcn_readfirstlane(lds_state.inv);
	fs.flen = __builtin_amdgcn_readfirstlane(lds_state.flen);
	fs.nout = (uint32_t)__builtin_amdgcn_readfirstlane((int)lds_state.nout);
	if (fs.collecting && fs.flen && wp < fs.fstart + 8 * (uint64_t)fs.flen) return;
	if (REG && !fs.collecting) {
		const uint32_t avail = (uint32_t)(wp - fs.rpos);
		if (wp >= fs.rpos && avail < 64u) return;
		if (wp >= fs.rpos && avail <= 64u * NCHUNK + 63u) {
			const uint32_t b0 = (uint32_t)fs.rpos;
			unsigned long long any = 0;
#pragma unroll
			for (int j = 0; j < NCHUNK; j++) {
				const uint32_t pb = b0 + (uint32_t)(64 * j + lane);
				const uint32_t wi = (uint32_t)((fs.rpos + (uint64_t)(64 * j)) >> 5) + ((((uint32_t)fs.rpos & 31u) + (uint32_t)lane) >> 5), sh = pb & 31u;
				const uint32_t w0 = mirror[wi & (SD_MIRROR_WORDS - 1)], w1 = mirror[(wi + 1) & (SD_MIRROR_WORDS - 1)],
				               w2 = mirror[(wi + 2) & (SD_MIRROR_WORDS - 1)];
				const uint32_t lo = __builtin_amdgcn_alignbit(w1, w0, sh), hi = __builtin_amdgcn_alignbit(w2, w1, sh);
				const int hd = __popc(lo ^ RS41_SYNC_LO) + __popc(hi ^ RS41_SYNC_HI);
				const bool hit = (uint32_t)(64 * j + lane) + 64u <= avail && (hd <= RS41_SYNC_THR || hd >= 64 - RS41_SYNC_THR);
				any |= __ballot(hit);
			}
			if (!any) { lds_state.rpos = wp - 63; return; }
		}
	}
	for (;;) {
		if (!fs.collecting) {
			bool found = false;
			while (fs.rpos + 64 <= wp) {
				constexpr int NCH = NCHUNK;
				unsigned long long hm[NCH];
				int hdv[NCH];
#pragma unroll
				for (int j = 0; j < NCH; j++) {
					const uint64_t pos = fs.rpos + (uint64_t)(64 * j + lane);
					const uint32_t wi = (uint32_t)(pos >> 5), sh = (uint32_t)pos & 31u;
					const uint32_t w0 = mirror[wi & (SD_MIRROR_WORDS - 1)], w1 = mirror[(wi + 1) & (SD_MIRROR_WORDS - 1)],
					               w2 = mirror[(wi + 2) & (SD_MIRROR_WORDS - 1)];
					const uint32_t lo = __builtin_amdgcn_alignbit(w1, w0, sh), hi = __builtin_amdgcn_alignbit(w2, w1, sh);
					const int hd = __popc(lo ^ RS41_SYNC_LO) + __popc(hi ^ RS41_SYNC_HI);
					const bool hit = pos + 64 <= wp && (hd <= RS41_SYNC_THR || hd >= 64 - RS41_SYNC_THR);
					hm[j] = __ballot(hit);
					hdv[j] = hd;
				}
#pragma unroll
				for (int j = 0; j < NCH; j++) {
					if (!found && hm[j]) {
						const int fl = __ffsll((long long)hm[j]) - 1;
						fs.fstart = fs.rpos + (uint64_t)(64 * j + fl);
						fs.inv = __builtin_amdgcn_readlane(hdv[j], fl) >= 64 - RS41_SYNC_THR;
						fs.collecting = 1;
						fs.flen = 0;
						found = true;
					}
				}
				if (found) break;
				uint64_t next = fs.rpos + 64 * NCH;
				if (next > wp - 63) next = wp - 63;
				fs.rpos = next;
			}
			if (!found) break;
		}
		if (!fs.flen) {
			if (wp < fs.fstart + 8 * (RS41_TYPE_POS + 1)) break;
			const uint64_t p = fs.fstart + 8 * RS41_TYPE_POS;
			const uint32_t wi = (uint32_t)(p >> 5), sh = (uint32_t)p & 31u;
			const uint32_t raw = __builtin_amdgcn_alignbit(mirror[(wi + 1) & (SD_MIRROR_WORDS - 1)], mirror[wi & (SD_MIRROR_WORDS - 1)], sh);
			const uint32_t tb = (raw ^ (fs.inv ? 0xFFu : 0u) ^ RS41_TYPE_MASK) & 0xFFu;
			fs.flen = (__popc(tb ^ 0xF0u) < __popc(tb ^ 0x0Fu)) ? RS41_LEN_EXT : RS41_LEN_STD;
		}
		if (wp < fs.fstart + 8 * (uint64_t)fs.flen) break;
		if (fs.nout < max_frames && lane == 0) {
			SdFrameDesc d;
			d.fstart = fs.fstart; d.flen = fs.flen; d.inv = fs.inv;
			descs_ch[fs.nout] = d;
			if (fs.nout < SD_K4_LIST) list[fs.nout] = d;
		}
		fs.nout++;
		fs.rpos = fs.fstart + 8 * (uint64_t)fs.flen;
		fs.collecting = 0;
		fs.flen = 0;
	}
	if (REG) {
		lds_state.rpos = fs.rpos; lds_state.fstart = fs.fstart;
		lds_state.collecting = fs.collecting; lds_state.inv = fs.inv; lds_state.flen = fs.flen; lds_state.nout = fs.nout;
		return;
	}
	if (lane == 0) {
		lds_state.rpos = fs.rpos; lds_state.fstart = fs.fstart;
		lds_state.collecting = fs.collecting; lds_state.inv = fs.inv; lds_state.flen = fs.flen;
		__hip_atomic_store(&lds_state.nout, fs.nout, __ATOMIC_RELEASE, __HIP_MEMORY_SCOPE_WORKGROUP);
	}
	__builtin_amdgcn_fence(__ATOMIC_SEQ_CST, "wavefront");
	__builtin_amdgcn_wave_barrier();
}
```

Before: 768,400 Msamples/s.

## Add multi-wave per-channel bins decoder kernel with automatic wave selection

Adds a templated bins decoder kernel that spreads one channel's polyphase passes and framing over 2 or 4 wavefronts per workgroup, with a union-shared LDS layout. When the channel count is small relative to the CU count, the launcher picks the 4-wave variant by default, aiming to raise occupancy and per-channel parallelism. A register-reuse variant of the RS41 sync prescan loads the mirror words once for several chunks. A raw state readback API and a setter for the wave count are also added; the risks are extra intra-block synchronisation and larger LDS use per block.

```diff
diff --git a/include/sonde_abi.h b/include/sonde_abi.h
--- a/include/sonde_abi.h
+++ b/include/sonde_abi.h
@@ -123,6 +123,7 @@
 uint64_t sonde_batch_nbits(SondeBatch *b, uint32_t channel);
 int      sonde_batch_read_state(SondeBatch *b, uint32_t channel, int64_t *t_next, int32_t *period, float *bias, float *amp,
                                 float *afc_u );
+long     sonde_batch_read_raw(SondeBatch *b, int what, void *out, size_t cap);
 int      sonde_get_taps(int type, float *out );
 int      sonde_get_afsk_table(float *out );
 
@@ -153,6 +154,7 @@
 int         sonde_chan_set_fused(SondeChannelizer *c, int on);
 int         sonde_chan_set_input(SondeChannelizer *c, int input_kind);
 int         sonde_chan_set_overlap(SondeChannelizer *c, int on);
+int         sonde_chan_set_bins_waves(SondeChannelizer *c, int waves);
 void        sonde_chan_destroy(SondeChannelizer *c);
 uint32_t    sonde_chan_samples_per_submit(const SondeChannelizer *c);
 int         sonde_chan_submit(SondeChannelizer *c, const void *iq_dev, size_t n_samples, void *stream);
diff --git a/sdrpp_radiosonde_amd/_lib.py b/sdrpp_radiosonde_amd/_lib.py
--- a/sdrpp_radiosonde_amd/_lib.py
+++ b/sdrpp_radiosonde_amd/_lib.py
@@ -81,13 +81,13 @@
 ABI_SYMBOLS = [
     "sonde_batch_create", "sonde_batch_destroy", "sonde_batch_submit", "sonde_batch_submit_host",
     "sonde_row_stride", "sonde_sample_bytes", "sonde_batch_wait_input", "sonde_batch_sync", "sonde_batch_frames", "sonde_batch_frames_of", "sonde_batch_ticket", "sonde_batch_overflow", "sonde_batch_kernel_ms", "sonde_batch_set_timing", "sonde_batch_class_ms", "sonde_batch_read_bits",
-    "sonde_batch_launch_info", "sonde_batch_nbits", "sonde_batch_read_state", "sonde_batch_test_rs255", "sonde_batch_poll", "sonde_get_taps", "sonde_get_afsk_table", "sonde_parse_frame",
+    "sonde_batch_launch_info", "sonde_batch_nbits", "sonde_batch_read_raw", "sonde_batch_read_state", "sonde_batch_test_rs255", "sonde_batch_poll", "sonde_get_taps", "sonde_get_afsk_table", "sonde_parse_frame",
     "sonde_parser_create", "sonde_parser_feed", "sonde_parser_destroy", "sonde_rs41_temp", "sonde_rs41_rh", "sonde_dfm_temp", "sonde_rs41_pressure", "sonde_ozone_mpa",
     "sonde_m10_temp", "sonde_m10_rh", "sonde_m20_temp", "sonde_ims100_temp",
     "sonde_last_error", "sonde_version", "sonde_hbm_read_probe", "sonde_dewpt", "sonde_altitude_to_pressure",
     "sonde_gpx_open", "sonde_gpx_close", "sonde_gpx_start_track", "sonde_gpx_stop_track", "sonde_gpx_add_point",
     "sonde_ptu_open", "sonde_ptu_close", "sonde_ptu_add_point",
-    "sonde_chan_create", "sonde_chan_create_multi", "sonde_chan_create_dual", "sonde_chan_streams", "sonde_chan_channels", "sonde_chan_set_fused", "sonde_chan_set_input", "sonde_chan_set_overlap", "sonde_chan_destroy", "sonde_chan_samples_per_submit", "sonde_chan_submit", "sonde_chan_batch",
+    "sonde_chan_create", "sonde_chan_create_multi", "sonde_chan_create_dual", "sonde_chan_streams", "sonde_chan_channels", "sonde_chan_set_fused", "sonde_chan_set_input", "sonde_chan_set_overlap", "sonde_chan_set_bins_waves", "sonde_chan_destroy", "sonde_chan_samples_per_submit", "sonde_chan_submit", "sonde_chan_batch",
     "sonde_chan_read", "sonde_chan_tables", "sonde_chan_kernel_ms",
     "sonde_vfo_create", "sonde_vfo_destroy", "sonde_vfo_ratio", "sonde_vfo_out_samples", "sonde_vfo_process", "sonde_vfo_process_host", "sonde_vfo_taps",
     "sonde_detect_create", "sonde_detect_destroy", "sonde_detect_submit", "sonde_detect_results", "sonde_detect_reset", "sonde_detect_thresholds",
@@ -143,6 +143,8 @@
     L.sonde_batch_read_bits.argtypes = [vp, C.c_uint32, C.c_uint64, C.c_size_t, vp]
     L.sonde_batch_nbits.argtypes = [vp, C.c_uint32]
     L.sonde_batch_nbits.restype = C.c_uint64
+    L.sonde_batch_read_raw.argtypes = [vp, C.c_int, vp, C.c_size_t]
+    L.sonde_batch_read_raw.restype = C.c_long
     L.sonde_batch_read_state.argtypes = [vp, C.c_uint32, C.POINTER(C.c_int64), C.POINTER(C.c_int32),
                                          C.POINTER(C.c_float), C.POINTER(C.c_float), C.POINTER(C.c_float)]
     if hasattr(L, "sonde_batch_test_rs255"):
@@ -183,6 +185,7 @@
     L.sonde_chan_create_multi.argtypes = [vp, C.c_uint32, C.c_uint32, C.c_int, C.POINTER(vp)]
     L.sonde_chan_set_fused.argtypes = [vp, C.c_int]
     L.sonde_chan_set_overlap.argtypes = [vp, C.c_int]
+    L.sonde_chan_set_bins_waves.argtypes = [vp, C.c_int]
     L.sonde_row_stride.argtypes = [C.c_size_t, C.c_int]
     L.sonde_row_stride.restype = C.c_size_t
     L.sonde_sample_bytes.argtypes = [C.c_int]
diff --git a/sdrpp_radiosonde_amd/batch.py b/sdrpp_radiosonde_amd/batch.py
--- a/sdrpp_radiosonde_amd/batch.py
+++ b/sdrpp_radiosonde_amd/batch.py
@@ -151,6 +151,14 @@
         self._chk(self.L.sonde_batch_read_bits(self.h, channel, start, count, out.ctypes.data_as(C.c_void_p)))
         return out
 
+    def read_raw(self, what: int) -> np.ndarray:
+        n = int(self.L.sonde_batch_read_raw(self.h, what, None, 0))
+        if n < 0:
+            raise SondeError(_lib.last_error() or "sonde_batch_read_raw failed")
+        out = np.zeros(n, dtype=np.uint8)
+        self._chk(-1 if self.L.sonde_batch_read_raw(self.h, what, out.ctypes.data_as(C.c_void_p), n) != n else 0)
+        return out
+
     def state(self, channel: int) -> dict:
         t, p = C.c_int64(), C.c_int32()
         b, a, y = C.c_float(), C.c_float(), C.c_float()
@@ -178,7 +186,7 @@
 class SondeChannelizer:
 
     def __init__(self, types=None, blocks_per_submit: int = 1, device: int = 0, n_streams: int = 1, fused: bool | None = None, overlap: bool | None = None,
-                 dual: bool = False, input_kind: int = INPUT_IQ):
+                 dual: bool = False, input_kind: int = INPUT_IQ, bins_waves: int = 0):
         self.L = _lib.load()
         self._types = None
         self.n_streams = int(n_streams)
@@ -199,6 +207,8 @@
         self.input_kind = int(self.L.sonde_chan_set_input(self.h, input_kind))
         if self.input_kind != input_kind:
             raise SondeError("sonde_chan_set_input: input kind not accepted")
+        if bins_waves:
+            self.set_bins_waves(bins_waves)
         self.samples_per_submit = int(self.L.sonde_chan_samples_per_submit(self.h))
         self.n_steps = self.samples_per_submit // 500
         self.batch = SondeBatch.__new__(SondeBatch)
@@ -217,6 +227,11 @@
         if self.L.sonde_chan_submit(self.h, C.c_void_p(iq.data_ptr()), self.samples_per_submit, C.c_void_p(stream or 0)) != 0:
             raise SondeError(_lib.last_error() or "sonde_chan_submit failed")
 
+    def set_bins_waves(self, waves: int) -> int:
+        if self.L.sonde_chan_set_bins_waves(self.h, int(waves)) != int(waves):
+            raise SondeError(_lib.last_error() or "sonde_chan_set_bins_waves refused")
+        return int(waves)
+
     def frames(self) -> np.ndarray:
         return SondeBatch.frames(self.batch)
 
@@ -235,7 +250,8 @@
 
     def close(self):
         if getattr(self, "h", None):
-            self.batch.h = None
+            if getattr(self, "batch", None) is not None:
+                self.batch.h = None
             self.L.sonde_chan_destroy(self.h)
             self.h = None
 
diff --git a/sdrpp_radiosonde_amd/csrc/batch.hip b/sdrpp_radiosonde_amd/csrc/batch.hip
--- a/sdrpp_radiosonde_amd/csrc/batch.hip
+++ b/sdrpp_radiosonde_amd/csrc/batch.hip
@@ -507,7 +507,7 @@
 }
 int sd_batch_submit_bins(SondeBatch *b, const SdBinsArgs *ba, size_t n_steps, void *stream_)
 {
-	if (!b || !ba || !ba->phases || !ba->carry_rows || !ba->g_comp || !sd_batch_bins_capable(b)) return fail("sd_batch_submit_bins: bad argument");
+	if (!b || !ba || !ba->phases || !ba->carry_rows || !ba->g_comp || !sd_bins_waves_known(ba->waves) || !sd_batch_bins_capable(b)) return fail("sd_batch_submit_bins: bad argument");
 	if (!b->units.empty()) return fail("sd_batch_submit_bins: the decoder batch behind a channelizer must be one plain launch (no launch units)");
 	const size_t n_out = n_steps / 5 * 12;
 	if (n_steps == 0 || n_steps % 2560 || n_out > b->max_samples || ba->row_stride < n_steps + 16)
@@ -604,7 +604,7 @@
 	} else if (one_launch) {
 		if (bins_in)
 			sd_launch_bins(b->n_channels, stream, bins_in->phases, bins_in->row_stride, n_tiles / 3, bins_in->carry_rows, bins_in->carry_stride,
-				b->d_states, b->d_hist, b->d_bitring, b->ring_words, b->d_taps, b->h_modems, &b->h_fo2[slot], bins_in->g_comp, b->cls_type[b->only_class]);
+				b->d_states, b->d_hist, b->d_bitring, b->ring_words, b->d_taps, b->h_modems, &b->h_fo2[slot], bins_in->g_comp, b->cls_type[b->only_class], bins_in->waves);
 		else {
 			SdSlice sl;
 			sd_launch_demod(b->input_kind, k_cls_decim[b->only_class], k_cls_nt[b->only_class], b->n_channels, stream, (const float *)samples, channel_stride, n_tiles,
@@ -979,6 +979,18 @@
 	return 0;
 }
 
+extern "C" long sonde_batch_read_raw(SondeBatch *b, int what, void *out, size_t cap)
+{
+	if (!b || what < 0 || what > 2) return fail("sonde_batch_read_raw: bad argument");
+	const void *src = what == 0 ? (const void *)b->d_states : what == 1 ? (const void *)b->d_fstates : (const void *)b->d_bitring;
+	const size_t bytes = (size_t)b->n_channels * (what == 0 ? sizeof(SdChanState) : what == 1 ? sizeof(SdFramerState) : (size_t)b->ring_words * 4);
+	if (!out) return (long)bytes;
+	if (cap < bytes) return fail("sonde_batch_read_raw: buffer too small");
+	if (sonde_batch_sync(b) < 0) return -1;
+	HIPCHK(hipMemcpy(out, src, bytes, hipMemcpyDeviceToHost));
+	return (long)bytes;
+}
+
 typedef uint32_t sd_u32x4 __attribute__((ext_vector_type(4)));
 __global__ __launch_bounds__(256) void sd_read_probe_kernel(const sd_u32x4 *__restrict__ src, size_t n16, uint32_t *sink)
 {
diff --git a/sdrpp_radiosonde_amd/csrc/bins_kernel.hip b/sdrpp_radiosonde_amd/csrc/bins_kernel.hip
--- a/sdrpp_radiosonde_amd/csrc/bins_kernel.hip
+++ b/sdrpp_radiosonde_amd/csrc/bins_kernel.hip
@@ -1,5 +1,6 @@
 #include <hip/hip_runtime.h>
 #include <atomic>
+#include <type_traits>
 #include "sonde_dev.h"
 #include "sd_input.h"
 #include "sd_math.h"
@@ -37,9 +38,14 @@
 #ifdef BK_TS
 __device__ unsigned long long g_bk_ts[64];
 extern "C" int sonde_debug_bins_ts(unsigned long long *out) { return hipMemcpyFromSymbol(out, HIP_SYMBOL(g_bk_ts), sizeof(g_bk_ts)) == hipSuccess ? 0 : -1; }
-#define BK_STAMP(i) do { if (ch == 1000u && lane == 0) g_bk_ts[i] = __builtin_readcyclecounter(); } while (0)
+#ifndef BK_TS_BIN
+#define BK_TS_BIN 1000u
+#endif
+#define BK_STAMP(i) do { if (ch == BK_TS_BIN && lane == 0) g_bk_ts[i] = __builtin_readcyclecounter(); } while (0)
+#define BK_STAMP_W(i) do { if (ch == BK_TS_BIN && lane == 0) g_bk_ts[16 * wave + (i)] = __builtin_readcyclecounter(); } while (0)
 #else
 #define BK_STAMP(i) do { } while (0)
+#define BK_STAMP_W(i) do { } while (0)
 #endif
 
 struct SdBinsParams {
@@ -319,14 +325,330 @@
 	BK_STAMP(16);
 }
 
+template <int W> struct BinsWideLds {
+	union {
+		struct {
+			float A[2][BK_A];
+			alignas(16) float d[W][BK_PASS_PH + 8];
+		} t;
+		FramerLds fl[W];
+	} u;
+	int part[W][4];
+	uint32_t chunk[10];
+	uint32_t mirror[SD_MIRROR_WORDS];
+	SdFrameDesc k4list[SD_K4_LIST];
+	uint32_t nout;
+	alignas(16) float taps[SD_NPHASE * SD_TAPS_LD];
+	EpiTabs et;
+};
+
+template <int W>
+__global__ __launch_bounds__(64 * W) void sd_bins_wide_kernel(
+	const int16_t *__restrict__ phases, size_t row_stride, int n_blocks, int16_t *__restrict__ carry_rows, size_t carry_stride,
+	SdChanState *__restrict__ states, float *__restrict__ hist, uint32_t *__restrict__ bitring, uint32_t ring_words,
+	const float *__restrict__ taps_all, const float *__restrict__ g_comp, uint32_t n_channels, const SdBinsParams P)
+{
+	static_assert(W == 2 || W == 4, "the 64-symbol groups of a round are four");
+	constexpr int G = 4 / W;
+	constexpr int PPW = (3 + W - 1) / W;
+	__shared__ __attribute__((aligned(16))) BinsWideLds<W> s;
+	const int tid = threadIdx.x, lane = tid & 63;
+	const int wave = __builtin_amdgcn_readfirstlane(tid >> 6);
+	const uint32_t ch = blockIdx.x;
+	if (ch >= n_channels) return;
+	BK_STAMP_W(0);
+
+	const uint32_t *row32 = reinterpret_cast<const uint32_t *>(phases + (size_t)ch * row_stride);
+	const uint4 *row128 = reinterpret_cast<const uint4 *>(row32);
+	uint4 ph[3][PPW] = {};
+	auto load_tile = [&](int b, int t, uint4 (&p)[PPW]) {
+#pragma unroll
+		for (int k = 0; k < PPW; k++) {
+			const int pi = (W - 1 - wave) + W * k;
+			if (pi < (t == 2 ? 2 : 3)) p[k] = lane < 42 ? row128[40 * (size_t)(8 * b + 3 * t + pi) + lane] : make_uint4(0u, 0u, 0u, 0u);
+		}
+	};
+	load_tile(0, 0, ph[0]); load_tile(0, 1, ph[1]); load_tile(0, 2, ph[2]);
+	const uint32_t sv = lane < 16 ? reinterpret_cast<const uint32_t *>(states + ch)[lane] : (lane < 24 ? reinterpret_cast<const uint32_t *>(P.fo.fstates + ch)[lane - 16] : 0u);
+	const float hv = lane >= SD_HIST - 16 ? hist[(size_t)ch * SD_HIST + lane] : 0.0f;
+	auto svw = [&](int i) { return (uint32_t)__builtin_amdgcn_readlane((int)sv, i); };
+	auto sv64 = [&](int i) { return (uint64_t)svw(i) | ((uint64_t)svw(i + 1) << 32); };
+	SdChanState st;
+	st.t_next = (int64_t)sv64(0); st.n0 = (int64_t)sv64(2); st.wpos = sv64(4); st.period = (int32_t)svw(6); st.nstat = (int32_t)svw(7);
+	st.bias = __uint_as_float(svw(8)); st.amp = __uint_as_float(svw(9)); st.iq_last[0] = __uint_as_float(svw(10)); st.iq_last[1] = __uint_as_float(svw(11));
+	st.type = (int32_t)svw(12); st.afc[0] = __uint_as_float(svw(13)); st.afc[1] = __uint_as_float(svw(14)); st.afc[2] = __uint_as_float(svw(15));
+	SdFramerState f0;
+	f0.rpos = sv64(16); f0.fstart = sv64(18); f0.collecting = (int32_t)svw(20); f0.inv = (int32_t)svw(21); f0.flen = (int32_t)svw(22); f0.pad = 0;
+	const int stype = P.utype >= 0 ? P.utype : st.type;
+	const SdModem md = P.modems[stype];
+	const bool is_rs41 = stype == SONDE_RS41, is_dfm = stype == SONDE_DFM09, is_ims = stype == SONDE_IMS100, is_mrz = stype == SONDE_MRZN1;
+	const bool fuse = P.fo.fuse_fec != 0;
+	const bool framing = is_rs41 || (fuse && (is_dfm || is_ims || is_mrz));
+	const bool fec_here = is_rs41 && fuse;
+	uint32_t *ring_g = bitring + (size_t)ch * ring_words;
+	const uint32_t ring_mask = ring_words - 1;
+	const uint32_t wi = (uint32_t)(st.wpos >> 5) - (uint32_t)(63 - lane);
+	const uint32_t xw = __hip_atomic_load(ring_g + (wi & ring_mask), __ATOMIC_RELAXED, __HIP_MEMORY_SCOPE_AGENT);
+	{
+		const float4 *taps_g = reinterpret_cast<const float4 *>(taps_all + (size_t)stype * SD_NPHASE * SD_NTAPS);
+#pragma unroll
+		for (int i = tid; i < 256; i += 64 * W) {
+			const int rowi = i >> 3, c4 = i & 7;
+			const float4 tv = taps_g[i];
+			*reinterpret_cast<float4 *>(&s.taps[rowi * SD_TAPS_LD + 4 * c4]) = make_float4(tv.y, tv.x, tv.w, tv.z);
+		}
+	}
+	if (tid < 10) s.chunk[tid] = 0u;
+	BK_STAMP_W(1);
+
+	float *const dw = s.u.t.d[wave];
+	auto pass = [&](const uint4 p, float *Aout ) {
+		{
+			typedef unsigned short u16x2 __attribute__((ext_vector_type(2)));
+			const uint32_t below = (uint32_t)__builtin_amdgcn_update_dpp(0, (int)p.w, 0x138, 0xF, 0xF, false);
+			const uint32_t x0 = __builtin_amdgcn_alignbit(p.x, below, 16), x1 = __builtin_amdgcn_alignbit(p.y, p.x, 16),
+			               x2 = __builtin_amdgcn_alignbit(p.z, p.y, 16), x3 = __builtin_amdgcn_alignbit(p.w, p.z, 16);
+			const uint32_t e0 = __builtin_bit_cast(uint32_t, __builtin_bit_cast(u16x2, p.x) - __builtin_bit_cast(u16x2, x0));
+			const uint32_t e1 = __builtin_bit_cast(uint32_t, __builtin_bit_cast(u16x2, p.y) - __builtin_bit_cast(u16x2, x1));
+			const uint32_t e2 = __builtin_bit_cast(uint32_t, __builtin_bit_cast(u16x2, p.z) - __builtin_bit_cast(u16x2, x2));
+			const uint32_t e3 = __builtin_bit_cast(uint32_t, __builtin_bit_cast(u16x2, p.w) - __builtin_bit_cast(u16x2, x3));
+			if (lane < 42) {
+				float4 *dst = reinterpret_cast<float4 *>(&dw[8 * lane]);
+				dst[0] = sd_cs16_f4(make_uint2(e0, e1));
+				dst[1] = sd_cs16_f4(make_uint2(e2, e3));
+			}
+		}
+		WAVE_SYNC();
+		typedef const __attribute__((address_space(4))) float *CTab;
+		unsigned long long g_addr = (unsigned long long)g_comp;
+		asm volatile("" : "+s"(g_addr));
+		const CTab g_pass = (CTab)g_addr;
+		float dv[20];
+		const float *dp = &dw[5 * lane + 1];
+#pragma unroll
+		for (int k = 0; k < 20; k++) dv[k] = dp[k];
+#pragma unroll
+		for (int c = 0; c < 3; c++) {
+			constexpr int BO[3] = {1, 2, 4};
+			const int bo = BO[c] + 15;
+			const CTab gt = g_pass + SD_RS_KT_LD * c;
+			float acc = 0.0f;
+#pragma unroll
+			for (int t = 0; t < SD_RS_KT; t++) acc = __builtin_fmaf(gt[t], dv[bo - t], acc);
+			Aout[3 * lane + c] = acc;
+		}
+		WAVE_SYNC();
+	};
+	auto tile_passes = [&](int b, int t, uint4 (&p)[PPW], float *An) {
+#pragma unroll
+		for (int k = 0; k < PPW; k++) {
+			const int pi = (W - 1 - wave) + W * k;
+			if (pi < (t == 2 ? 2 : 3)) pass(p[k], An + SD_LH + 64 * t + 192 * pi);
+		}
+		if (b + 1 < n_blocks) load_tile(b + 1, t, p);
+	};
+
+	int64_t n0 = st.n0;
+	uint64_t wpos = st.wpos;
+	uint32_t partial = 0;
+	SdSyncRun k4;
+	int cur = 0;
+	tile_passes(0, 0, ph[0], s.u.t.A[0]);
+	if (wave == 0) {
+		s.u.t.A[0][lane] = hv;
+		s.mirror[wi & (SD_MIRROR_WORDS - 1)] = xw;
+		partial = ((uint32_t)st.wpos & 31u) ? (uint32_t)__builtin_amdgcn_readlane((int)xw, 63) : 0u;
+		k4.rpos = f0.rpos; k4.fstart = f0.fstart; k4.collecting = f0.collecting; k4.inv = f0.inv; k4.flen = f0.flen; k4.nout = 0; k4.wp_seen = 0;
+	}
+	BK_STAMP_W(2);
+
+	auto tile_step = [&](int b, auto tc) {
+		constexpr int t = decltype(tc)::value;
+		float *const A = s.u.t.A[cur], *const An = s.u.t.A[cur ^ 1];
+		n0 += BK_IT;
+		const int64_t limit = (((n0 - 1 - BK_NT / 2 - SD_MARGIN) << 16) | 0xFFFF);
+		int K = (st.t_next <= limit) ? (int)((uint32_t)(limit - st.t_next) / (uint32_t)st.period) + 1 : 0;
+		if (K > SD_ROUND_MAX) K = SD_ROUND_MAX;
+		const int64_t base = (n0 - BK_IT - SD_LH) << 16;
+		const uint32_t rel0 = (uint32_t)(st.t_next - base);
+		const float bias = st.bias;
+		uint32_t rel[G];
+#pragma unroll
+		for (int h = 0; h < G; h++) rel[h] = rel0 + __umul24((unsigned)(sd_hw_symbol(lane) + 64 * (G * wave + h)), (unsigned)st.period);
+		__syncthreads();
+		BK_STAMP_W(3 + 4 * t);
+		{
+			int Ei = 0, S1i = 0, S0i = 0, C1 = 0;
+			float y[G], m[G];
+#pragma unroll
+			for (int h = 0; h < G; h++) {
+				y[h] = interp<BK_NT>(A, s.taps, rel[h]);
+				m[h] = interp<BK_NT>(A, s.taps, rel[h] - ((uint32_t)st.period >> 1));
+			}
+#pragma unroll
+			for (int h = 0; h < G; h++) {
+				const int g = G * wave + h;
+				const bool act = sd_hw_symbol(lane) + 64 * g < K;
+				const float yy = act ? y[h] : 0.0f;
+				const float yprev = sd_hw_prev(yy, lane);
+				float e = (yprev - yy) * (m[h] - bias);
+				e = sd_clamp(e * 1024.0f, -1.0e6f, 1.0e6f);
+				Ei += (act && lane != 0) ? __float2int_rn(e) : 0;
+				const bool bit = act && (yy > bias);
+				const int Y = __float2int_rn(sd_clamp(yy, -8.0f, 8.0f) * 4096.0f);
+				S1i += bit ? Y : 0;
+				S0i += (act && !bit) ? Y : 0;
+				const unsigned long long bal = __ballot(sd_hw_unpermute(bit ? 1 : 0, lane) != 0);
+				C1 += __popcll(bal);
+				if (lane == 0) { s.chunk[1 + 2 * g] = (uint32_t)bal; s.chunk[2 + 2 * g] = (uint32_t)(bal >> 32); }
+			}
+			const int Ep = wave_sum(Ei), S1p = wave_sum(S1i), S0p = wave_sum(S0i);
+			if (lane == 0) { s.part[wave][0] = Ep; s.part[wave][1] = S1p; s.part[wave][2] = S0p; s.part[wave][3] = C1; }
+		}
+		BK_STAMP_W(4 + 4 * t);
+		__syncthreads();
+		BK_STAMP_W(5 + 4 * t);
+		int E = 0, S1 = 0, S0 = 0, C1 = 0;
+#pragma unroll
+		for (int j = 0; j < W; j++) { E += s.part[j][0]; S1 += s.part[j][1]; S0 += s.part[j][2]; C1 += s.part[j][3]; }
+		E = __builtin_amdgcn_readfirstlane(E); S1 = __builtin_amdgcn_readfirstlane(S1); S0 = __builtin_amdgcn_readfirstlane(S0); C1 = __builtin_amdgcn_readfirstlane(C1);
+		if (K > 0) {
+			if (wave == 0) {
+				if (lane < 9) {
+					const uint32_t sh = (uint32_t)wpos & 31u, w0 = (uint32_t)(wpos >> 5);
+					uint32_t vv = 0;
+					if ((uint32_t)(32 * lane) < sh + (uint32_t)K) {
+						const uint32_t lo = s.chunk[lane + 1], pvw = s.chunk[lane];
+						vv = sh ? ((lo << sh) | (pvw >> (32u - sh))) : lo;
+						if (lane == 0 && sh) vv |= partial & ((1u << sh) - 1u);
+						const uint32_t idx = (w0 + (uint32_t)lane) & ring_mask;
+						ring_g[idx] = vv;
+						s.mirror[idx & (SD_MIRROR_WORDS - 1)] = vv;
+					}
+					partial = vv;
+				}
+				partial = (uint32_t)__builtin_amdgcn_readlane((int)partial, (int)((((uint32_t)wpos & 31u) + (uint32_t)K) >> 5));
+			}
+			wpos += (uint64_t)K;
+			const int C0 = K - C1;
+			if (C1 > 0 && C0 > 0) {
+				const f32x2 cnt = {(float)C1, (float)C0};
+				const f32x2 rc = sd_recip2(cnt);
+				const float hi = ((float)S1 * rc.x) * (1.0f / 4096.0f);
+				const float lo = ((float)S0 * rc.y) * (1.0f / 4096.0f);
+				const float c = 0.5f * (hi + lo), a = 0.5f * (hi - lo);
+				if (st.nstat == 0) { st.bias = c; st.amp = a; }
+				else { st.bias = st.bias + 0.5f * (c - st.bias); st.amp = st.amp + 0.5f * (a - st.amp); }
+				if (!(st.amp >= 1.0e-3f)) st.amp = 1.0e-3f;
+				st.nstat = 1;
+			} else {
+				st.bias = ((float)(S1 + S0) * sd_recip((float)K)) * (1.0f / 4096.0f);
+			}
+			if (n0 <= 3 * (int64_t)BK_IT) st.bias = ((float)(S1 + S0) * sd_recip((float)K)) * (1.0f / 4096.0f);
+			const f32x2 den = {(float)K, st.amp * st.amp};
+			const f32x2 rd = sd_recip2(den);
+			float err = ((float)E * rd.x) * (1.0f / 1024.0f);
+			err = err * rd.y;
+			err = sd_clamp(err, -1.0f, 1.0f);
+			const int dphase = __float2int_rn(err * md.kp), dper = __float2int_rn(err * md.ki);
+			st.t_next += (int64_t)K * st.period + dphase;
+			st.period += dper;
+			if (st.period < md.pmin) st.period = md.pmin;
+			if (st.period > md.pmax) st.period = md.pmax;
+		}
+		if (wave == 0) {
+			An[lane] = A[BK_IT + lane];
+			if (t < 2) An[64 + lane] = A[BK_IT + 64 + lane];
+			if (t == 1) An[128 + lane] = A[BK_IT + 128 + lane];
+		}
+		constexpr int tn = (t + 1) % 3;
+		const int bn = t == 2 ? b + 1 : b;
+		if (bn < n_blocks) tile_passes(bn, tn, ph[tn], An);
+		if (t == 2 && framing && wave == 0) {
+			WAVE_SYNC();
+			SdFrameDesc *dch = (SdFrameDesc *)P.fo.descs + (size_t)ch * P.fo.max_frames;
+			const uint32_t mf = P.fo.max_frames;
+			if (is_rs41) sd_rs41_sync_step<true, 4, 12>(k4, wpos, s.mirror, lane, dch, mf, s.k4list);
+			else if (is_dfm) sd_fixed_sync_step<SONDE_DFM09, true>(k4, wpos, s.mirror, lane, dch, mf, s.k4list);
+			else if (is_ims) sd_fixed_sync_step<SONDE_IMS100, true>(k4, wpos, s.mirror, lane, dch, mf, s.k4list);
+			else sd_fixed_sync_step<SONDE_MRZN1, true>(k4, wpos, s.mirror, lane, dch, mf, s.k4list);
+		}
+		cur ^= 1;
+		BK_STAMP_W(6 + 4 * t);
+	};
+	for (int b = 0; b < n_blocks; b++) {
+		tile_step(b, std::integral_constant<int, 0>{});
+		tile_step(b, std::integral_constant<int, 1>{});
+		tile_step(b, std::integral_constant<int, 2>{});
+	}
+
+	if (wave == 0) {
+		WAVE_SYNC();
+		if (lane >= SD_HIST - 16) hist[(size_t)ch * SD_HIST + lane] = s.u.t.A[cur][lane];
+		if (lane < 8) {
+			const size_t n_ph = 2560 * (size_t)n_blocks;
+			reinterpret_cast<uint32_t *>(carry_rows + (size_t)ch * carry_stride)[lane] = row32[n_ph / 2 + lane];
+		}
+		if (lane == 0) {
+			st.n0 = n0;
+			st.wpos = wpos;
+			states[ch] = st;
+			if (framing) {
+				SdFramerState f1;
+				f1.rpos = k4.rpos; f1.fstart = k4.fstart; f1.collecting = k4.collecting; f1.inv = k4.inv; f1.flen = k4.flen; f1.pad = 0;
+				P.fo.fstates[ch] = f1;
+				P.fo.counts[ch] = k4.nout;
+			}
+			s.nout = k4.nout;
+		}
+	}
+	if (fec_here) {
+		__syncthreads();
+		const uint32_t max_frames = P.fo.max_frames;
+		const uint32_t nfr = min((uint32_t)__builtin_amdgcn_readfirstlane((int)s.nout), max_frames);
+		if (nfr) {
+			for (int i = tid; i < GF_EXP2 / 16 + 512 / 16 + RS_R * 8 * 4 / 16; i += 64 * W) {
+				if (i < GF_EXP2 / 16) reinterpret_cast<uint4 *>(s.et.tabs.exp2)[i] = reinterpret_cast<const uint4 *>(P.fo.gf_exp)[i];
+				else if (i < GF_EXP2 / 16 + 512 / 16) reinterpret_cast<uint4 *>(s.et.tabs.log2)[i - GF_EXP2 / 16] = reinterpret_cast<const uint4 *>(P.fo.gf_log)[i - GF_EXP2 / 16];
+				else reinterpret_cast<uint4 *>(s.et.swar)[i - (GF_EXP2 / 16 + 512 / 16)] = reinterpret_cast<const uint4 *>(P.fo.gf_swar)[i - (GF_EXP2 / 16 + 512 / 16)];
+			}
+			__syncthreads();
+			FramerLds &wl = s.u.fl[wave];
+			GfSwar swar;
+			const uint32_t *sw = s.et.swar + 8 * (lane % RS_R);
+			swar.a_lo = sw[0]; swar.a_hi = sw[1]; swar.b_lo = sw[2]; swar.b_hi = sw[3]; swar.c = sw[4];
+			const unsigned long long *dg = reinterpret_cast<const unsigned long long *>((const SdFrameDesc *)P.fo.descs + (size_t)ch * max_frames);
+			SondeFrame *fout = P.fo.frames + (size_t)ch * max_frames;
+			for (uint32_t k = (uint32_t)wave; k < nfr; k += W) {
+				unsigned long long d0, d1;
+				if (k < SD_K4_LIST) {
+					const unsigned long long *dl = reinterpret_cast<const unsigned long long *>(&s.k4list[k]);
+					d0 = dl[0]; d1 = dl[1];
+				} else {
+					d0 = __hip_atomic_load(dg + 2 * k, __ATOMIC_RELAXED, __HIP_MEMORY_SCOPE_AGENT);
+					d1 = __hip_atomic_load(dg + 2 * k + 1, __ATOMIC_RELAXED, __HIP_MEMORY_SCOPE_AGENT);
+				}
+				SdFrameDesc d;
+				d.fstart = sd_uniform64(d0);
+				d.flen = __builtin_amdgcn_readfirstlane((int)(uint32_t)d1);
+				d.inv = __builtin_amdgcn_readfirstlane((int)(d1 >> 32));
+				sd_rs41_decode_frame<true>(s.et.tabs, wl, swar, ring_g, ring_mask, d, fout + k, ch, lane);
+			}
+		}
+	}
+	BK_STAMP_W(15);
+}
+
+bool sd_bins_waves_known(int w) { return w == 0 || w == 1 || w == 2 || w == 4; }
+
 void sd_launch_bins(uint32_t n_channels, hipStream_t stream, const int16_t *phases, size_t row_stride, int n_blocks,
 	int16_t *carry_rows, size_t carry_stride, SdChanState *states, float *hist, uint32_t *bitring, uint32_t ring_words,
-	const float *taps_all, const SdModem *modems_host, const SdFramerOut *fo_host, const float *g_comp, int utype)
+	const float *taps_all, const SdModem *modems_host, const SdFramerOut *fo_host, const float *g_comp, int utype, int waves)
 {
-	int wpw = BK_WAVES;
+	int wpw = BK_WAVES, cus = 256;
 	{
 		static std::atomic<int> cus_of[64];
-		int dev = 0, cus = 256;
+		int dev = 0;
 		if (hipGetDevice(&dev) == hipSuccess && dev >= 0 && dev < 64) {
 			int known = cus_of[dev].load(std::memory_order_relaxed);
 			if (!known && hipDeviceGetAttribute(&known, hipDeviceAttributeMultiprocessorCount, dev) == hipSuccess && known > 0) cus_of[dev].store(known, std::memory_order_relaxed);
@@ -334,11 +656,20 @@
 		}
 		while (wpw > 1 && (n_channels + wpw - 1) / wpw < (uint32_t)cus) wpw >>= 1;
 	}
-	const dim3 g((n_channels + wpw - 1) / wpw), blk(64 * wpw);
+	if (waves == 0) waves = (uint64_t)n_channels * 4u <= 16u * (uint64_t)cus ? 4 : 1;
 	SdBinsParams P;
 	P.fo = *fo_host;
 	for (int t = 0; t < SONDE_NTYPES; t++) P.modems[t] = modems_host[t];
 	P.utype = utype;
-	hipLaunchKernelGGL(sd_bins_kernel, g, blk, 0, stream, phases, row_stride, n_blocks, carry_rows, carry_stride, states, hist, bitring,
-	                   ring_words, taps_all, g_comp, n_channels, P);
+	if (waves == 4)
+		hipLaunchKernelGGL(sd_bins_wide_kernel<4>, dim3(n_channels), dim3(256), 0, stream, phases, row_stride, n_blocks, carry_rows, carry_stride, states, hist, bitring,
+		                   ring_words, taps_all, g_comp, n_channels, P);
+	else if (waves == 2)
+		hipLaunchKernelGGL(sd_bins_wide_kernel<2>, dim3(n_channels), dim3(128), 0, stream, phases, row_stride, n_blocks, carry_rows, carry_stride, states, hist, bitring,
+		                   ring_words, taps_all, g_comp, n_channels, P);
+	else {
+		const dim3 g((n_channels + wpw - 1) / wpw), blk(64 * wpw);
+		hipLaunchKernelGGL(sd_bins_kernel, g, blk, 0, stream, phases, row_stride, n_blocks, carry_rows, carry_stride, states, hist, bitring,
+		                   ring_words, taps_all, g_comp, n_channels, P);
+	}
 }
diff --git a/sdrpp_radiosonde_amd/csrc/channelizer.hip b/sdrpp_radiosonde_amd/csrc/channelizer.hip
--- a/sdrpp_radiosonde_amd/csrc/channelizer.hip
+++ b/sdrpp_radiosonde_amd/csrc/channelizer.hip
@@ -327,6 +327,7 @@
 	hipEvent_t ev_xs = nullptr;
 	uint32_t xcd_map = 0;
 	bool overlap = false;
+	int bins_waves = 0;
 	hipStream_t s_pfb = nullptr, s_dec = nullptr;
 	hipEvent_t ev_in = nullptr, ev_pfb[2] = {}, ev_dec[2] = {};
 	int16_t *d_bins_b = nullptr;
@@ -514,6 +515,16 @@
 	return c->overlap ? 1 : 0;
 }
 
+extern "C" int sonde_chan_set_bins_waves(SondeChannelizer *c, int waves)
+{
+	if (!c) return -1;
+	if (waves < 0) return c->bins_waves;
+	if (c->n_blocks != 0) return sd_fail("sonde_chan_set_bins_waves: before the first submit only");
+	if (!sd_bins_waves_known(waves)) return sd_fail("sonde_chan_set_bins_waves: the bins decoder has 1, 2 or 4 waves per bin (0: its own choice)");
+	c->bins_waves = waves;
+	return c->bins_waves;
+}
+
 static bool chan_overlap_setup(SondeChannelizer *c)
 {
 	if (c->s_pfb) return true;
@@ -583,7 +594,7 @@
 		if (hipStreamWaitEvent(stream, c->ev_pfb[b], 0) != hipSuccess || hipStreamWaitEvent(c->s_dec, c->ev_pfb[b], 0) != hipSuccess) return -1;
 		if (hipGetLastError() != hipSuccess) return -1;
 		c->last_stream = stream;
-		const SdBinsArgs ba = { bins, (size_t)c->n_steps + PH_HEAD, bins_next, (size_t)c->n_steps + PH_HEAD, c->d_gc };
+		const SdBinsArgs ba = { bins, (size_t)c->n_steps + PH_HEAD, bins_next, (size_t)c->n_steps + PH_HEAD, c->d_gc, c->bins_waves };
 		if (sd_batch_submit_bins(c->batch, &ba, c->n_steps, (void *)c->s_dec) != 0) return -1;
 		return hipEventRecord(c->ev_dec[b], c->s_dec) == hipSuccess ? 0 : -1;
 	}
@@ -602,7 +613,7 @@
 	if (timed) { (void)hipEventRecord(c->ev[2], stream); c->ev_pending = true; }
 	if (hipGetLastError() != hipSuccess) return -1;
 	if (c->fused) {
-		const SdBinsArgs ba = { c->d_bins, (size_t)c->n_steps + PH_HEAD, c->d_bins, (size_t)c->n_steps + PH_HEAD, c->d_gc };
+		const SdBinsArgs ba = { c->d_bins, (size_t)c->n_steps + PH_HEAD, c->d_bins, (size_t)c->n_steps + PH_HEAD, c->d_gc, c->bins_waves };
 		return sd_batch_submit_bins(c->batch, &ba, c->n_steps, stream_);
 	}
 	return sonde_batch_submit(c->batch, c->d_out48, n_out, n_out, stream_);
diff --git a/sdrpp_radiosonde_amd/csrc/launch.h b/sdrpp_radiosonde_amd/csrc/launch.h
--- a/sdrpp_radiosonde_amd/csrc/launch.h
+++ b/sdrpp_radiosonde_amd/csrc/launch.h
@@ -31,11 +31,12 @@
 void sd_launch_demod_mixed(int in_kind, uint32_t n_a, const uint32_t *list_a, int utype_a, uint32_t n_b, const uint32_t *list_b, int utype_b, hipStream_t stream,
 	const float *in, size_t ch_stride, int n_tiles, SdChanState *states, float *hist, uint32_t *bitring, uint32_t ring_words,
 	const float *taps_all, const SdModem *modems, const SdFramerOut *fo );
-struct SdBinsArgs { const int16_t *phases; size_t row_stride; int16_t *carry_rows; size_t carry_stride; const float *g_comp ; };
+struct SdBinsArgs { const int16_t *phases; size_t row_stride; int16_t *carry_rows; size_t carry_stride; const float *g_comp ; int waves; };
+bool sd_bins_waves_known(int w);
 void sd_launch_bins(uint32_t n_channels, hipStream_t stream, const int16_t *phases, size_t row_stride, int n_blocks,
 	int16_t *carry_rows, size_t carry_stride, SdChanState *states, float *hist, uint32_t *bitring, uint32_t ring_words,
 	const float *taps_all, const SdModem *modems_host , const SdFramerOut *fo_host ,
-	const float *g_comp, int utype );
+	const float *g_comp, int utype , int waves );
 int sd_batch_submit_bins(SondeBatch *b, const SdBinsArgs *ba, size_t n_steps, void *stream);
 int sd_batch_bins_capable(const SondeBatch *b);
 
diff --git a/sdrpp_radiosonde_amd/csrc/sd_rs41.h b/sdrpp_radiosonde_amd/csrc/sd_rs41.h
--- a/sdrpp_radiosonde_amd/csrc/sd_rs41.h
+++ b/sdrpp_radiosonde_amd/csrc/sd_rs41.h
@@ -26,7 +26,7 @@
 	       (uint32_t)__builtin_amdgcn_readfirstlane((int)(uint32_t)v);
 }
 
-template <bool REG = false, int NCHUNK = (REG ? 4 : 1)>
+template <bool REG = false, int NCHUNK = (REG ? 4 : 1), int NSCAN = NCHUNK>
 __device__ __forceinline__ void sd_rs41_sync_step(SdSyncRun &lds_state, uint64_t wp, const uint32_t *mirror, int lane,
 	SdFrameDesc *__restrict__ descs_ch, uint32_t max_frames, SdFrameDesc *list = nullptr)
 {
@@ -41,11 +41,24 @@
 	if (REG && !fs.collecting) {
 		const uint32_t avail = (uint32_t)(wp - fs.rpos);
 		if (wp >= fs.rpos && avail < 64u) return;
-		if (wp >= fs.rpos && avail <= 64u * NCHUNK + 63u) {
+		if (wp >= fs.rpos && avail <= 64u * NSCAN + 63u) {
 			const uint32_t b0 = (uint32_t)fs.rpos;
 			unsigned long long any = 0;
+			if constexpr (NSCAN != NCHUNK) {
+				const uint32_t wi0 = (uint32_t)(fs.rpos >> 5) + ((((uint32_t)fs.rpos & 31u) + (uint32_t)lane) >> 5), sh = (b0 + (uint32_t)lane) & 31u;
+				uint32_t mw[2 * NSCAN + 1];
 #pragma unroll
-			for (int j = 0; j < NCHUNK; j++) {
+				for (int k = 0; k < 2 * NSCAN + 1; k++) mw[k] = mirror[(wi0 + (uint32_t)k) & (SD_MIRROR_WORDS - 1)];
+#pragma unroll
+				for (int j = 0; j < NSCAN; j++) {
+					const uint32_t lo = __builtin_amdgcn_alignbit(mw[2 * j + 1], mw[2 * j], sh), hi = __builtin_amdgcn_alignbit(mw[2 * j + 2], mw[2 * j + 1], sh);
+					const int hd = __popc(lo ^ RS41_SYNC_LO) + __popc(hi ^ RS41_SYNC_HI);
+					const bool hit = (uint32_t)(64 * j + lane) + 64u <= avail && (hd <= RS41_SYNC_THR || hd >= 64 - RS41_SYNC_THR);
+					any |= __ballot(hit);
+				}
+			} else
+#pragma unroll
+			for (int j = 0; j < NSCAN; j++) {
 				const uint32_t pb = b0 + (uint32_t)(64 * j + lane);
 				const uint32_t wi = (uint32_t)((fs.rpos + (uint64_t)(64 * j)) >> 5) + ((((uint32_t)fs.rpos & 31u) + (uint32_t)lane) >> 5), sh = pb & 31u;
 				const uint32_t w0 = mirror[wi & (SD_MIRROR_WORDS - 1)], w1 = mirror[(wi + 1) & (SD_MIRROR_WORDS - 1)],
```

Measured after the change: 766,500 Msamples/s. No clear change (-0.2%).
